# keya-dialog/LoCo-ASR

Hardware: AMD Instinct MI355X
Metric: audio frames/sec SpeechT5-base encoder, 30s×bs32 @1/2/4/8 GPU; embed L2 vs HF (higher is better)
Workload: dtype f16x3 (fp16 hi+lo operands, 3 MFMAs per product, fp32 accumulate); 1 GPU; SpeechT5-base speech encoder, synthetic 16 kHz 30 s clips, batch 32 per GPU (BASELINE.json configs[1]), random-init weights; batch_per_gpu=32, global_batch=32, frames_per_clip=1499, parallelism=dp1, collective=none

## Files before the change

### include/loco_asr.h

```cpp
#ifndef LOCO_ASR_H
#define LOCO_ASR_H

#include <stddef.h>
#include <stdint.h>

#ifdef __cplusplus
extern "C" {
#endif

#define LOCO_ABI_VERSION 1

enum {
    LOCO_OK = 0,
    LOCO_E_INVALID = -1,
    LOCO_E_STATE = -2,
    LOCO_E_WORKSPACE = -3,
    LOCO_E_HIP = -4,
    LOCO_E_RANGE = -5
};

typedef struct loco_config {
    int32_t struct_size;
    int32_t hidden;
    int32_t heads;
    int32_t ffn;
    int32_t layers;
    int32_t conv_dim;
    int32_t pos_conv_kernel;
    int32_t pos_conv_groups;
    int32_t rel_max;
    float ln_eps;
} loco_config;

typedef struct loco_encoder loco_encoder;

int loco_abi_version(void);
const char* loco_last_error(void);
void loco_default_config(loco_config* cfg);

loco_encoder* loco_create(const loco_config* cfg);
void loco_destroy(loco_encoder* enc);

int loco_set_weight(loco_encoder* enc, const char* key, const float* data, const int64_t* shape, int ndim);

int loco_missing_weights(const loco_encoder* enc, char* buf, size_t buflen);

int loco_finalize_weights(loco_encoder* enc, void* stream);

int64_t loco_output_frames(int64_t n_samples);

size_t loco_workspace_bytes(const loco_encoder* enc, int32_t B, int64_t L);

int loco_forward(loco_encoder* enc, const float* wav, const int32_t* attention_mask, int32_t B, int64_t L,
                 float* out, int32_t* out_frames, float* const* hidden_states, void* workspace,
                 size_t workspace_bytes, void* stream);

int loco_forward_status(loco_encoder* enc, char* buf, size_t buflen);
int loco_forward_range(const loco_encoder* enc, int32_t stage, float* amax, int32_t* layer, char* name, size_t namelen);
int loco_set_range_policy(loco_encoder* enc, int policy);
int loco_forward_checked(loco_encoder* enc, const float* wav, const int32_t* attention_mask, int32_t B, int64_t L,
                         float* out, int32_t* out_frames, float* const* hidden_states, void* workspace,
                         size_t workspace_bytes, void* stream, int32_t* used_fp32);

size_t loco_status_bytes(void);
int loco_forward_async(loco_encoder* enc, int precision, const float* wav, const int32_t* attention_mask, int32_t B, int64_t L,
                       float* out, int32_t* out_frames, float* const* hidden_states, void* workspace, size_t workspace_bytes,
                       void* stream, void* status);
int loco_status_check(const void* status, char* buf, size_t buflen);

int loco_max_pack_clips(void);
int loco_forward_packed(loco_encoder* enc, int precision, const float* wav, const int32_t* attention_mask, const int64_t* valid_len,
                        int32_t B, int64_t L, const int64_t* pad_len, float* out, int32_t* out_frames, float* const* hidden_states,
                        void* workspace, size_t workspace_bytes, void* stream, void* status);
int loco_status_range(const void* status, int32_t stage, float* amax, int32_t* layer, char* name, size_t namelen);

int loco_resample_design(int32_t sr_in, int32_t sr_out, int32_t* up, int32_t* down, int32_t* taps_per_phase, float* taps_host);
int64_t loco_resample_length(int64_t n_in, int32_t up, int32_t down);
int loco_op_resample(const float* x, int32_t B, int64_t n_in, int64_t x_stride, const float* taps_dev, int32_t up, int32_t down,
                     int32_t taps_per_phase, float* y, int64_t n_out, int64_t y_stride, void* stream);

const char* loco_flac_last_error(void);
int loco_flac_info(const void* data, size_t nbytes, int32_t* sample_rate, int32_t* channels, int32_t* bits_per_sample, int64_t* total_samples);
int loco_flac_decode(const void* data, size_t nbytes, float* mono, int32_t* pcm, int64_t capacity, int64_t* n_samples, int32_t verify_md5);

size_t loco_normalize_scratch_bytes(int32_t B);
int loco_op_normalize_waveform(const float* wav, const int32_t* attention_mask, int32_t B, int64_t L, float padding_value,
                               float* out, void* scratch, size_t scratch_bytes, void* stream);

size_t loco_text_workspace_bytes(const loco_encoder* enc, int32_t B, int32_t T);
int loco_text_max_positions(const loco_encoder* enc);
int loco_forward_text(loco_encoder* enc, const int32_t* input_ids, const int32_t* attention_mask, int32_t B, int32_t T,
                      float* out, int32_t* out_frames, float* const* hidden_states, void* workspace, size_t workspace_bytes,
                      void* stream);
int loco_forward_text_async(loco_encoder* enc, int precision, const int32_t* input_ids, const int32_t* attention_mask, int32_t B,
                            int32_t T, float* out, int32_t* out_frames, float* const* hidden_states, void* workspace,
                            size_t workspace_bytes, void* stream, void* status);

#define LOCO_PRECISION_MODES "0 f32, 1 f16x3, 2 f16x2"
const char* loco_precision_name(int mode);
int loco_set_precision(loco_encoder* enc, int mode);
int loco_get_precision(const loco_encoder* enc);

int loco_set_streams(loco_encoder* enc, int n);

int loco_set_taps(loco_encoder* enc, float* conv_stack, float* feature_projection, float* prenet);

int loco_set_attention_outputs(loco_encoder* enc, float* const* probs, int32_t n);

typedef struct loco_kernel_stat {
    char name[48];
    int64_t launches;
    double ms;
    double flops;
    double bytes;
} loco_kernel_stat;

int loco_set_profiling(loco_encoder* enc, int on);
int loco_set_profiling_filter(loco_encoder* enc, const char* bucket);
int loco_profile_reset(loco_encoder* enc);
int loco_profile_read(loco_encoder* enc, loco_kernel_stat* stats, int max_stats);


int loco_op_layernorm(const float* x, const float* gamma, const float* beta, float* y, int64_t rows, int32_t dim,
                      float eps, void* stream);

int loco_op_gemm(const float* A, int64_t lda, const float* W, int64_t ldw, const float* bias, const float* R, int64_t ldr,
                 float* C, int64_t ldc, int32_t M, int32_t N, int32_t K, int32_t epilogue, int32_t nb1, int32_t nb2,
                 int64_t sA1, int64_t sA2, int64_t sC1, int64_t sC2, void* stream);

size_t loco_conv0_scratch_bytes(int32_t B);
int loco_op_conv0_gn_gelu(const float* wav, int32_t B, int64_t L, const float* w, const float* gn_w, const float* gn_b,
                          float* out, void* scratch, void* stream);

int loco_op_frame_counts(const int32_t* mask, int32_t B, int64_t L, int32_t* frames, void* stream);

int loco_op_pos_conv(const float* h, const float* w_folded, const float* bias, const float* sin_table, const int32_t* frames,
                     float* out, int32_t B, int32_t T, void* stream);

int loco_op_attention(const float* qkv, const float* qp, const int32_t* frames, float* ctx, int32_t B, int32_t T,
                      void* stream);
int loco_op_attention_probs(const float* qkv, const float* qp, const int32_t* frames, float* probs, int32_t B, int32_t T,
                            void* stream);

int loco_op_split_f16(const float* x, void* hi, void* lo, int64_t n, void* stream);
int loco_op_gemm_f16x3(const void* Ahi, const void* Alo, int64_t lda, const void* Whi, const void* Wlo, int64_t ldw,
                       const float* bias, const float* R, int64_t ldr, float* C, void* Chi, void* Clo, int64_t ldc,
                       int32_t M, int32_t N, int32_t K, int32_t epilogue, int32_t nb1, int32_t nb2, int64_t sA1, int64_t sA2,
                       int64_t sC1, int64_t sC2, void* stream);

int loco_op_permute_conv_k(const float* w, float* out, int32_t N, int32_t taps, int32_t Cin, void* stream);
int loco_op_conv_gemm_f16x3(const void* Ahi, const void* Alo, int64_t lda, const void* Whi, const void* Wlo, float* C, void* Chi,
                            void* Clo, int32_t Tout, int32_t N, int32_t Cin, int32_t taps, int32_t epilogue, int32_t B, int64_t sA1,
                            void* stream);

size_t loco_gemm_splitk_bytes(void);
void loco_debug_reload_gemm_knobs(void);
int loco_op_gemm_f16x3_splitk(const void* Ahi, const void* Alo, int64_t lda, const void* Whi, const void* Wlo, int64_t ldw,
                              const float* bias, const float* R, int64_t ldr, float* C, void* Chi, void* Clo, int64_t ldc,
                              int32_t M, int32_t N, int32_t K, int32_t epilogue, void* splitk_ws, size_t splitk_bytes,
                              void* stream);

int loco_op_attention_f16x3(const void* qhi, const void* qlo, const void* khi, const void* klo, const void* vhi,
                            const void* vlo, const float* qp, const int32_t* frames, float* ctx, int32_t B, int32_t T,
                            void* stream);
int loco_op_attention_f16x3_pe(const void* qhi, const void* qlo, const void* khi, const void* klo, const void* vhi, const void* vlo,
                               const void* pe_hi, const void* pe_lo, float pe_scale, float* qp_scratch, const int32_t* frames,
                               float* ctx, int32_t B, int32_t T, void* stream);
int loco_op_attention_probs_f16x3(const void* qhi, const void* qlo, const void* khi, const void* klo, const float* qp,
                                  const int32_t* frames, float* probs, int32_t B, int32_t T, int32_t terms, void* stream);

typedef struct loco_head loco_head;
const char* loco_head_last_error(void);
loco_head* loco_head_create(int method);
void loco_head_destroy(loco_head* head);
int32_t loco_head_num_params(void);
int loco_head_set_params(loco_head* head, const float* flat);
int loco_head_get_params(const loco_head* head, float* flat);
size_t loco_head_workspace_bytes(int32_t B, int32_t T);
int loco_head_forward(loco_head* head, const float* x, int32_t B, int32_t T, float* logits, void* workspace,
                      size_t workspace_bytes, void* stream);
int loco_head_loss_grad(loco_head* head, const float* x, const float* target, int32_t B, int32_t T, float* loss,
                        float* logits, float* grads, void* workspace, size_t workspace_bytes, void* stream);
int loco_head_forward_ragged(loco_head* head, const float* store, const int64_t* offsets, const int32_t* lengths,
                             const int32_t* idx, int32_t B, int32_t T_pad, float* logits, void* workspace,
                             size_t workspace_bytes, void* stream);
int loco_head_loss_grad_ragged(loco_head* head, const float* store, const int64_t* offsets, const int32_t* lengths,
                               const float* targets, const int32_t* idx, int32_t B, int32_t T_pad, float* loss,
                               float* logits, float* grads, void* workspace, size_t workspace_bytes, void* stream);
int loco_head_adam_step(loco_head* head, const float* grads, float lr, float beta1, float beta2, float eps,
                        float weight_decay, void* stream);

int loco_has_decoder(const loco_encoder* enc);
int loco_decoder_max_batch(void);
size_t loco_decoder_workspace_bytes(const loco_encoder* enc, int32_t B, int32_t T_enc, int32_t S_max);
int loco_decoder_forward(loco_encoder* enc, const float* enc_out, const int32_t* enc_frames, int32_t B, int32_t T_enc,
                         const int32_t* decoder_input_ids, int32_t S, float* logits, float* const* hidden_states, void* workspace,
                         size_t workspace_bytes, void* stream);
int loco_decoder_begin(loco_encoder* enc, const float* enc_out, const int32_t* enc_frames, int32_t B, int32_t T_enc, int32_t S_max,
                       void* workspace, size_t workspace_bytes, void* stream);
int loco_decoder_step(loco_encoder* enc, int32_t B, int32_t T_enc, int32_t S_max, int32_t t, float* logits, void* workspace,
                      size_t workspace_bytes, void* stream);
int loco_decoder_read_tokens(const loco_encoder* enc, int32_t B, int32_t T_enc, int32_t S_max, int32_t* tokens, int32_t* lengths,
                             const void* workspace, size_t workspace_bytes, void* stream);
int loco_decoder_generate(loco_encoder* enc, const float* enc_out, const int32_t* enc_frames, int32_t B, int32_t T_enc, int32_t max_length,
                          int32_t* tokens_out, int32_t* lengths_out, int32_t* out_length, float* step_logits, void* workspace,
                          size_t workspace_bytes, void* stream);
int loco_op_skinny_gemm(const float* A, int64_t lda, const float* W, int64_t ldw, const float* bias, const float* R, int64_t ldr, float* C,
                        int64_t ldc, int32_t M, int32_t N, int32_t K, int32_t epilogue, void* stream);
size_t loco_decoder_attention_scratch_bytes(int32_t B, int32_t Sq, int32_t Tk);
int loco_op_decoder_attention(const float* q, const float* k, const float* v, const int32_t* key_counts, float* out, int32_t B, int32_t Sq,
                              int32_t Tk, int32_t causal, int32_t causal_offset, float scale, void* scratch, size_t scratch_bytes, void* stream);

#ifdef __cplusplus
}
#endif
#endif
```

### loco-asr_amd/_lib.py

```python
from __future__ import annotations

import ctypes as C
import os

_HERE = os.path.dirname(os.path.abspath(__file__))
LIB_PATH = os.environ.get("LOCO_ASR_LIB") or os.path.join(_HERE, "libloco_asr.so")
ABI_VERSION = 1


class LocoError(RuntimeError):
    """A C-ABI call returned a negative LOCO_E_* code."""


class LocoConfig(C.Structure):
    _fields_ = [("struct_size", C.c_int32), ("hidden", C.c_int32), ("heads", C.c_int32), ("ffn", C.c_int32),
                ("layers", C.c_int32), ("conv_dim", C.c_int32), ("pos_conv_kernel", C.c_int32),
                ("pos_conv_groups", C.c_int32), ("rel_max", C.c_int32), ("ln_eps", C.c_float)]


class KernelStat(C.Structure):
    _fields_ = [("name", C.c_char * 48), ("launches", C.c_int64), ("ms", C.c_double), ("flops", C.c_double),
                ("bytes", C.c_double)]


_vp, _i32, _i64, _sz, _f = C.c_void_p, C.c_int32, C.c_int64, C.c_size_t, C.c_float

SIGNATURES = {
    "loco_abi_version": (C.c_int, []),
    "loco_last_error": (C.c_char_p, []),
    "loco_default_config": (None, [C.POINTER(LocoConfig)]),
    "loco_create": (_vp, [C.POINTER(LocoConfig)]),
    "loco_destroy": (None, [_vp]),
    "loco_set_weight": (C.c_int, [_vp, C.c_char_p, _vp, C.POINTER(_i64), C.c_int]),
    "loco_missing_weights": (C.c_int, [_vp, C.c_char_p, _sz]),
    "loco_finalize_weights": (C.c_int, [_vp, _vp]),
    "loco_output_frames": (_i64, [_i64]),
    "loco_workspace_bytes": (_sz, [_vp, _i32, _i64]),
    "loco_forward": (C.c_int, [_vp, _vp, _vp, _i32, _i64, _vp, _vp, C.POINTER(_vp), _vp, _sz, _vp]),
    "loco_forward_status": (C.c_int, [_vp, C.c_char_p, _sz]),
    "loco_forward_range": (C.c_int, [_vp, _i32, C.POINTER(_f), C.POINTER(_i32), C.c_char_p, _sz]),
    "loco_set_range_policy": (C.c_int, [_vp, C.c_int]),
    "loco_forward_checked": (C.c_int, [_vp, _vp, _vp, _i32, _i64, _vp, _vp, C.POINTER(_vp), _vp, _sz, _vp, C.POINTER(_i32)]),
    "loco_status_bytes": (_sz, []),
    "loco_forward_async": (C.c_int, [_vp, C.c_int, _vp, _vp, _i32, _i64, _vp, _vp, C.POINTER(_vp), _vp, _sz, _vp, _vp]),
    "loco_max_pack_clips": (C.c_int, []),
    "loco_forward_packed": (C.c_int, [_vp, C.c_int, _vp, _vp, C.POINTER(_i64), _i32, _i64, C.POINTER(_i64), _vp, _vp, C.POINTER(_vp), _vp, _sz, _vp,
                                      _vp]),
    "loco_status_check": (C.c_int, [_vp, C.c_char_p, _sz]),
    "loco_status_range": (C.c_int, [_vp, _i32, C.POINTER(_f), C.POINTER(_i32), C.c_char_p, _sz]),
    "loco_flac_last_error": (C.c_char_p, []),
    "loco_flac_info": (C.c_int, [_vp, _sz, C.POINTER(_i32), C.POINTER(_i32), C.POINTER(_i32), C.POINTER(_i64)]),
    "loco_flac_decode": (C.c_int, [_vp, _sz, _vp, _vp, _i64, C.POINTER(_i64), _i32]),
    "loco_resample_design": (C.c_int, [_i32, _i32, C.POINTER(_i32), C.POINTER(_i32), C.POINTER(_i32), _vp]),
    "loco_resample_length": (_i64, [_i64, _i32, _i32]),
    "loco_op_resample": (C.c_int, [_vp, _i32, _i64, _i64, _vp, _i32, _i32, _i32, _vp, _i64, _i64, _vp]),
    "loco_normalize_scratch_bytes": (_sz, [_i32]),
    "loco_op_normalize_waveform": (C.c_int, [_vp, _vp, _i32, _i64, C.c_float, _vp, _vp, _sz, _vp]),
    "loco_text_workspace_bytes": (_sz, [_vp, _i32, _i32]),
    "loco_text_max_positions": (C.c_int, [_vp]),
    "loco_forward_text": (C.c_int, [_vp, _vp, _vp, _i32, _i32, _vp, _vp, C.POINTER(_vp), _vp, _sz, _vp]),
    "loco_precision_name": (C.c_char_p, [C.c_int]),
    "loco_forward_text_async": (C.c_int, [_vp, C.c_int, _vp, _vp, _i32, _i32, _vp, _vp, C.POINTER(_vp), _vp, _sz, _vp, _vp]),
    "loco_set_precision": (C.c_int, [_vp, C.c_int]),
    "loco_get_precision": (C.c_int, [_vp]),
    "loco_set_streams": (C.c_int, [_vp, C.c_int]),
    "loco_set_taps": (C.c_int, [_vp, _vp, _vp, _vp]),
    "loco_set_attention_outputs": (C.c_int, [_vp, _vp, _i32]),
    "loco_set_profiling": (C.c_int, [_vp, C.c_int]),
    "loco_set_profiling_filter": (C.c_int, [_vp, C.c_char_p]),
    "loco_profile_reset": (C.c_int, [_vp]),
    "loco_profile_read": (C.c_int, [_vp, C.POINTER(KernelStat), C.c_int]),
    "loco_op_layernorm": (C.c_int, [_vp, _vp, _vp, _vp, _i64, _i32, _f, _vp]),
    "loco_op_gemm": (C.c_int, [_vp, _i64, _vp, _i64, _vp, _vp, _i64, _vp, _i64, _i32, _i32, _i32, _i32, _i32, _i32,
                               _i64, _i64, _i64, _i64, _vp]),
    "loco_conv0_scratch_bytes": (_sz, [_i32]),
    "loco_op_conv0_gn_gelu": (C.c_int, [_vp, _i32, _i64, _vp, _vp, _vp, _vp, _vp, _vp]),
    "loco_op_frame_counts": (C.c_int, [_vp, _i32, _i64, _vp, _vp]),
    "loco_op_pos_conv": (C.c_int, [_vp, _vp, _vp, _vp, _vp, _vp, _i32, _i32, _vp]),
    "loco_op_attention": (C.c_int, [_vp, _vp, _vp, _vp, _i32, _i32, _vp]),
    "loco_op_attention_probs": (C.c_int, [_vp, _vp, _vp, _vp, _i32, _i32, _vp]),
    "loco_op_attention_probs_f16x3": (C.c_int, [_vp, _vp, _vp, _vp, _vp, _vp, _vp, _i32, _i32, _i32, _vp]),
    "loco_op_split_f16": (C.c_int, [_vp, _vp, _vp, _i64, _vp]),
    "loco_gemm_splitk_bytes": (_sz, []),
    "loco_debug_reload_gemm_knobs": (None, []),
    "loco_op_gemm_f16x3_splitk": (C.c_int, [_vp, _vp, _i64, _vp, _vp, _i64, _vp, _vp, _i64, _vp, _vp, _vp, _i64, _i32, _i32, _i32, _i32,
                                            _vp, _sz, _vp]),
    "loco_op_gemm_f16x3": (C.c_int, [_vp, _vp, _i64, _vp, _vp, _i64, _vp, _vp, _i64, _vp, _vp, _vp, _i64, _i32, _i32, _i32, _i32,
                                     _i32, _i32, _i64, _i64, _i64, _i64, _vp]),
    "loco_op_permute_conv_k": (C.c_int, [_vp, _vp, _i32, _i32, _i32, _vp]),
    "loco_op_conv_gemm_f16x3": (C.c_int, [_vp, _vp, _i64, _vp, _vp, _vp, _vp, _vp, _i32, _i32, _i32, _i32, _i32, _i32, _i64, _vp]),
    "loco_op_attention_f16x3": (C.c_int, [_vp, _vp, _vp, _vp, _vp, _vp, _vp, _vp, _vp, _i32, _i32, _vp]),
    "loco_op_attention_f16x3_pe": (C.c_int, [_vp, _vp, _vp, _vp, _vp, _vp, _vp, _vp, _f, _vp, _vp, _vp, _i32, _i32, _vp]),
    "loco_head_last_error": (C.c_char_p, []),
    "loco_head_create": (_vp, [C.c_int]),
    "loco_head_destroy": (None, [_vp]),
    "loco_head_num_params": (_i32, []),
    "loco_head_set_params": (C.c_int, [_vp, _vp]),
    "loco_head_get_params": (C.c_int, [_vp, _vp]),
    "loco_head_workspace_bytes": (_sz, [_i32, _i32]),
    "loco_head_forward": (C.c_int, [_vp, _vp, _i32, _i32, _vp, _vp, _sz, _vp]),
    "loco_head_loss_grad": (C.c_int, [_vp, _vp, _vp, _i32, _i32, _vp, _vp, _vp, _vp, _sz, _vp]),
    "loco_head_forward_ragged": (C.c_int, [_vp, _vp, _vp, _vp, _vp, _i32, _i32, _vp, _vp, _sz, _vp]),
    "loco_head_loss_grad_ragged": (C.c_int, [_vp, _vp, _vp, _vp, _vp, _vp, _i32, _i32, _vp, _vp, _vp, _vp, _sz, _vp]),
    "loco_head_adam_step": (C.c_int, [_vp, _vp, _f, _f, _f, _f, _f, _vp]),
    "loco_has_decoder": (C.c_int, [_vp]),
    "loco_decoder_max_batch": (C.c_int, []),
    "loco_decoder_workspace_bytes": (_sz, [_vp, _i32, _i32, _i32]),
    "loco_decoder_forward": (C.c_int, [_vp, _vp, _vp, _i32, _i32, _vp, _i32, _vp, C.POINTER(_vp), _vp, _sz, _vp]),
    "loco_decoder_begin": (C.c_int, [_vp, _vp, _vp, _i32, _i32, _i32, _vp, _sz, _vp]),
    "loco_decoder_step": (C.c_int, [_vp, _i32, _i32, _i32, _i32, _vp, _vp, _sz, _vp]),
    "loco_decoder_read_tokens": (C.c_int, [_vp, _i32, _i32, _i32, _vp, _vp, _vp, _sz, _vp]),
    "loco_decoder_generate": (C.c_int, [_vp, _vp, _vp, _i32, _i32, _i32, _vp, _vp, C.POINTER(_i32), _vp, _vp, _sz, _vp]),
    "loco_op_skinny_gemm": (C.c_int, [_vp, _i64, _vp, _i64, _vp, _vp, _i64, _vp, _i64, _i32, _i32, _i32, _i32, _vp]),
    "loco_decoder_attention_scratch_bytes": (_sz, [_i32, _i32, _i32]),
    "loco_op_decoder_attention": (C.c_int, [_vp, _vp, _vp, _vp, _vp, _i32, _i32, _i32, _i32, _i32, _f, _vp, _sz, _vp]),
}

_lib = None


def _check_foreign_build(path):
    import importlib.util
    spec = importlib.util.spec_from_file_location("loco_check_isa", os.path.join(_HERE, "csrc", "check_isa.py"))
    mod = importlib.util.module_from_spec(spec)
    spec.loader.exec_module(mod)
    try:
        _, _, bad = mod.check(path)
    except (OSError, RuntimeError) as e:
        import warnings
        warnings.warn(f"LOCO_ASR_LIB={path}: could not inspect the code objects ({e})")
        return
    if bad and os.environ.get("LOCO_ALLOW_BANNED_ISA") != "1":
        raise ImportError(f"LOCO_ASR_LIB={path}: {len(bad)} packed fp32 instructions cross-select their low lane (e.g. `{bad[0]}`): "
                          "results are unreliable beside the attention kernel (DESIGN.md 5); set LOCO_ALLOW_BANNED_ISA=1 only to "
                          "reproduce that hazard")


def load():
    global _lib
    if _lib is not None:
        return _lib
    if not os.path.exists(LIB_PATH):
        raise ImportError(
            f"{LIB_PATH} not found: the HIP library has not been built. Run `python -c 'import __graft_entry__ as g; "
            f"g.build()'` or `make -C {os.path.join(_HERE, 'csrc')}` (hipcc, --offload-arch=gfx950). There is no CPU fallback.")
    if os.environ.get("LOCO_ASR_LIB"):
        _check_foreign_build(LIB_PATH)
    lib = C.CDLL(LIB_PATH)
    for name, (res, args) in SIGNATURES.items():
        if os.environ.get("LOCO_ASR_LIB") and name.startswith("loco_op_") and not hasattr(lib, name):
            continue
        fn = getattr(lib, name)
        fn.restype = res
        fn.argtypes = args
    if lib.loco_abi_version() != ABI_VERSION:
        raise ImportError(f"{LIB_PATH}: ABI version {lib.loco_abi_version()} != {ABI_VERSION}; rebuild the library")
    _lib = lib
    return lib


def check(rc: int, what: str = ""):
    if rc < 0:
        msg = load().loco_last_error().decode(errors="replace")
        if rc == -1:
            raise ValueError(f"{what}: {msg}" if what else msg)
        raise LocoError(f"{what}: [{rc}] {msg}" if what else f"[{rc}] {msg}")
    return rc
```

### loco-asr_amd/csrc/gemm_f16x3.hip

```cpp
#include <cstdlib>

#include "loco_kernels.h"

#ifndef LOCO_GEMM_HACK
#define LOCO_GEMM_HACK 0
#endif

namespace loco {

typedef _Float16 h8 __attribute__((ext_vector_type(8)));
typedef _Float16 h4 __attribute__((ext_vector_type(4)));

template <int EPI, bool OUT_SPLIT>
__device__ __forceinline__ void split_gemm_store(const GemmSplitArgs& p, f32x4 v, long coff, int m, int n, float& amax, int z1 = 0,
                                                 int z2 = 0) {
    if (EPI == kEpiGelu) {
#pragma unroll
        for (int e = 0; e < 4; e += 2) { const f32x2_t g_ = gelu_erf2(f32x2_t{v[e], v[e + 1]}); v[e] = g_.x; v[e + 1] = g_.y; }
    }
    if (EPI == kEpiResidual) {
        const long ro = coff + (long)m * p.ldr + n;
        if (p.Rhi) {
            const h4 rh = *reinterpret_cast<const h4*>(p.Rhi + ro), rl = *reinterpret_cast<const h4*>(p.Rlo + ro);
#pragma unroll
            for (int e = 0; e < 4; ++e) v[e] += (float)rh[e] + (float)rl[e];
        } else {
            v += *reinterpret_cast<const f32x4*>(p.R + ro);
        }
    }
    if (EPI == kEpiPosConv) {
#pragma unroll
        for (int e = 0; e < 4; e += 2) { const f32x2_t g_ = gelu_erf2(f32x2_t{v[e], v[e + 1]}); v[e] = g_.x; v[e + 1] = g_.y; }
        int nvalid = p.frames ? p.frames[z1] : p.T;
        if (nvalid <= 0 || nvalid > p.T) nvalid = p.T;
        const int pos = m < nvalid ? m + 2 : 1;
        v += *reinterpret_cast<const f32x4*>(p.R + coff + (long)m * p.ldr + n);
        v += *reinterpret_cast<const f32x4*>(p.sin_table + (long)pos * kHidden + z2 * kPosCg + n);
        *reinterpret_cast<f32x4*>(p.C + coff + (long)m * p.ldc + n) = v;
        return;
    }
    if (!OUT_SPLIT && EPI != kEpiQkvScatter) {
        *reinterpret_cast<f32x4*>(p.C + coff + (long)m * p.ldc + n) = v;
        return;
    }
    typedef unsigned u32x2_t __attribute__((ext_vector_type(2)));
    amax = fmaxf(fmaxf(amax, fmaxf(fabsf(v[0]), fabsf(v[1]))), fmaxf(fabsf(v[2]), fabsf(v[3])));
    u32x2_t hu, lu;
    {
        unsigned h0, l0, h1, l1;
        split_f16_2pairs(v[0], v[1], v[2], v[3], h0, l0, h1, l1);
        hu = u32x2_t{h0, h1};
        lu = u32x2_t{l0, l1};
    }
    const h4 hi = __builtin_bit_cast(h4, hu), lo = __builtin_bit_cast(h4, lu);
    if (EPI == kEpiQkvScatter) {
        {
            const int third = n < kHidden ? 0 : (n < 2 * kHidden ? 1 : 2);
            const long o = third * p.qkv_stride + (long)m * kHidden + (n - third * kHidden);
            *reinterpret_cast<h4*>(p.Chi + o) = hi;
            *reinterpret_cast<h4*>(p.Clo + o) = lo;
        }
    } else {
        const long o = coff + (long)m * p.ldc + n;
        *reinterpret_cast<h4*>(p.Chi + o) = hi;
        *reinterpret_cast<h4*>(p.Clo + o) = lo;
    }
}

template <int EPI, bool OUT_SPLIT>
__device__ __forceinline__ void split_gemm_store16(const GemmSplitArgs& p, f32x4 (&v)[4], long coff, int m, int n, float& amax, int z1,
                                                   int z2) {
    constexpr bool wide_epi = EPI == kEpiNone || EPI == kEpiGelu || EPI == kEpiResidual || EPI == kEpiQkvScatter;
    if (!wide_epi || n + 16 > p.N) {
#pragma unroll
        for (int j = 0; j < 4; ++j)
            if (n + 4 * j < p.N) split_gemm_store<EPI, OUT_SPLIT>(p, v[j], coff, m, n + 4 * j, amax, z1, z2);
        return;
    }
    if (EPI == kEpiGelu) {
#pragma unroll
        for (int j = 0; j < 4; ++j)
#pragma unroll
            for (int e = 0; e < 4; e += 2) { const f32x2_t g_ = gelu_erf2(f32x2_t{v[j][e], v[j][e + 1]}); v[j][e] = g_.x; v[j][e + 1] = g_.y; }
    }
    if (EPI == kEpiResidual) {
        const long ro = coff + (long)m * p.ldr + n;
        if (p.Rhi) {
#pragma unroll
            for (int jj = 0; jj < 2; ++jj) {
                const h8 rh = *reinterpret_cast<const h8*>(p.Rhi + ro + 8 * jj), rl = *reinterpret_cast<const h8*>(p.Rlo + ro + 8 * jj);
#pragma unroll
                for (int e = 0; e < 8; ++e) v[2 * jj + (e >> 2)][e & 3] += (float)rh[e] + (float)rl[e];
            }
        } else {
#pragma unroll
            for (int j = 0; j < 4; ++j) v[j] += *reinterpret_cast<const f32x4*>(p.R + ro + 4 * j);
        }
    }
    if (!OUT_SPLIT && EPI != kEpiQkvScatter) {
        float* cp = p.C + coff + (long)m * p.ldc + n;
#pragma unroll
        for (int j = 0; j < 4; ++j)
            if (LOCO_GEMM_HACK != 4 || p.M <= 0) *reinterpret_cast<f32x4*>(cp + 4 * j) = v[j];
        return;
    }
    typedef unsigned u32x4_t __attribute__((ext_vector_type(4)));
    h8 hi[2], lo[2];
#pragma unroll
    for (int j = 0; j < 4; ++j) amax = fmaxf(fmaxf(amax, fmaxf(fabsf(v[j][0]), fabsf(v[j][1]))), fmaxf(fabsf(v[j][2]), fabsf(v[j][3])));
#pragma unroll
    for (int jj = 0; jj < 2; ++jj) {
        u32x4_t hu, lu;
        unsigned h0, l0, h1, l1;
        split_f16_2pairs(v[2 * jj][0], v[2 * jj][1], v[2 * jj][2], v[2 * jj][3], h0, l0, h1, l1);
        hu[0] = h0; hu[1] = h1; lu[0] = l0; lu[1] = l1;
        split_f16_2pairs(v[2 * jj + 1][0], v[2 * jj + 1][1], v[2 * jj + 1][2], v[2 * jj + 1][3], h0, l0, h1, l1);
        hu[2] = h0; hu[3] = h1; lu[2] = l0; lu[3] = l1;
        hi[jj] = __builtin_bit_cast(h8, hu);
        lo[jj] = __builtin_bit_cast(h8, lu);
    }
    _Float16 *dh, *dl;
    if (EPI == kEpiQkvScatter) {
        const int third = n < kHidden ? 0 : (n < 2 * kHidden ? 1 : 2);
        const long o = third * p.qkv_stride + (long)m * kHidden + (n - third * kHidden);
        dh = p.Chi + o;
        dl = p.Clo + o;
    } else {
        const long o = coff + (long)m * p.ldc + n;
        dh = p.Chi + o;
        dl = p.Clo + o;
    }
    if (LOCO_GEMM_HACK == 4 && p.M > 0) return;
    *reinterpret_cast<h8*>(dh) = hi[0];
    *reinterpret_cast<h8*>(dh + 8) = hi[1];
    *reinterpret_cast<h8*>(dl) = lo[0];
    *reinterpret_cast<h8*>(dl + 8) = lo[1];
}

constexpr int SBK = 32;

#ifdef LOCO_GEMM_STAMPS
__device__ unsigned long long* g_gemm_stamps = nullptr;
#define GEMM_STAMP(t) { __builtin_amdgcn_sched_barrier(0); asm volatile("s_memtime %0\n\ts_waitcnt lgkmcnt(0)" : "=s"(t) :: "memory"); __builtin_amdgcn_sched_barrier(0); }
#else
#define GEMM_STAMP(t) {}
#endif

typedef __attribute__((address_space(1))) const void* gptr_t;
typedef __attribute__((address_space(3))) void* lptr_t;
typedef __attribute__((address_space(3))) const h8* lds_h8p;

#if LOCO_GEMM_HACK == 1
#define DMA16(base_, voff_, ldsb_) asm volatile("" :: "s"(ldsb_), "v"(voff_), "s"(base_) : "memory")
#elif LOCO_GEMM_HACK == 6
#define DMA16(base_, voff_, ldsb_)                                                                                                  \
    if (wave < 4) asm volatile("s_mov_b32 m0, %0\n\ts_nop 0\n\tglobal_load_lds_dwordx4 %1, %2" :: "s"(ldsb_), "v"(voff_), "s"(base_) : "memory")
#else
#define DMA16(base_, voff_, ldsb_) \
    asm volatile("s_mov_b32 m0, %0\n\ts_nop 0\n\tglobal_load_lds_dwordx4 %1, %2" :: "s"(ldsb_), "v"(voff_), "s"(base_) : "memory")
#endif
#define VMCNT_LGKM0(n_)                                                                              \
    {                                                                                                \
        static_assert((n_) >= 0 && (n_) <= 63, "vmcnt is a 6-bit field");                            \
        asm volatile("s_waitcnt vmcnt(%0) lgkmcnt(0)" ::"n"(n_) : "memory");                         \
    }

template <int EPI, bool OUT_SPLIT, int WM, int WN, int AST, int WST, int NJ = 4, int WPS = 0, int TERMS = 3, bool PERSIST = false>
__global__ __launch_bounds__(64 * WM * WN, WPS ? WPS : (WM * WN) / 4) void gemm_f16x3_dma_kernel(GemmSplitArgs p, int tiles_m,
                                                                                                  int tiles_n, int nblk, int wg_step,
                                                                                                  int col_group) {
    constexpr int DBM = 64 * WM, DBN = 64 * WN, NW_ = WM * WN;
    constexpr int DPA = DBM * SBK, DPW = DBN * SBK;
    constexpr int ABUF = 2 * DPA, WBUF = 2 * DPW;
    constexpr int NDA = DBM / 16 / NW_;
    constexpr int NDW = (DBN / 16 + NW_ - 1) / NW_;
    constexpr int WPIECES = DBN / 16;
    constexpr int NA = 2 * NDA, NWP = (TERMS == 3 ? 2 : 1) * NDW;
    static_assert(NDA >= 1 && DBM % (16 * NW_) == 0, "tile too small for the wave count");
    static_assert((AST == WST && AST >= 2 && AST <= 5) || (AST == 3 && WST == 2), "ring depths: equal rings of 2-5 slots, or 3 A + 2 W");
    static_assert(WPIECES % NW_ == 0 || (WST == 2 && AST == 3) || AST == 2, "uneven W pieces: no wait may leave W DMAs in flight");
    static_assert(TERMS == 3 || TERMS == 2, "terms");
    static_assert((size_t)(AST * ABUF + WST * WBUF) * 2 <= 160 * 1024, "LDS");
    static_assert(2 * (DPA + 16 * 3 * SBK) < 65536 && 2 * (DPW + 16 * 3 * SBK) < 65536, "fragment offsets are ds_read immediates");
    constexpr bool PERMW = NJ == 4 && (OUT_SPLIT || EPI == kEpiQkvScatter);
    __shared__ __attribute__((aligned(16))) _Float16 lds[AST * ABUF + WST * WBUF];

    const int tid = threadIdx.x, lane = tid & 63;
    const int wave = __builtin_amdgcn_readfirstlane(tid >> 6);
    const int wm = wave / WN, wn = wave % WN;
    const int r16 = lane & 15, q4 = lane >> 4;
    const int drow = lane >> 2, dpos = lane & 3;
    const unsigned lds0 = (unsigned)(unsigned long)(lptr_t)lds;
    const int nk = p.K / SBK;

    const int xcd = blockIdx.x & 7;
    int tile_i = blockIdx.x >> 3;
    int run_start, run_len;
    {
        const int q = nblk >> 3, rr = nblk & 7;
        run_start = xcd < rr ? xcd * (q + 1) : rr * (q + 1) + (xcd - rr) * q;
        run_len = q + (xcd < rr ? 1 : 0);
    }
    struct Tile {
        const char *bAh, *bAl, *bWh, *bWl;
        unsigned va[NDA], vw[NDW];
        int m0, n0, z1, z2, kt0;
        long coff;
    };
    auto decode = [&](int i, Tile& t_) {
        const int t = run_start + i;
        const int per_z = tiles_m * tiles_n;
        const int z = t / per_z;
        const int tz = t - z * per_z;
        const int full = tiles_n / col_group;
        int g = tz / (tiles_m * col_group), rem, width;
        if (g < full) {
            rem = tz - g * tiles_m * col_group;
            width = col_group;
        } else {
            g = full;
            rem = tz - full * tiles_m * col_group;
            width = tiles_n - full * col_group;
        }
        const int mt = rem / width;
        const int nt = g * col_group + (rem - mt * width);
        t_.z1 = z / p.nb2;
        t_.z2 = z % p.nb2;
        t_.kt0 = t_.z2 * p.kt_per_z2;
        const int z1o = t_.z1 / p.z1_inner, z1i = t_.z1 - z1o * p.z1_inner;
        const long aoff = z1o * p.sA1 + z1i * p.sA1i + t_.z2 * p.sA2;
        const long woff = z1i * p.sW1i + t_.z2 * p.sW2;
        t_.coff = t_.z1 * p.sC1 + t_.z2 * p.sC2;
        t_.m0 = mt * DBM;
        t_.n0 = nt * DBN;
#pragma unroll
        for (int u = 0; u < NDA; ++u) {
            const int row = 16 * (NDA * wave + u) + drow;
            int ra = t_.m0 + row;
            ra = (ra < p.M ? ra : p.M - 1) - t_.m0;
            t_.va[u] = 2u * (unsigned)(ra * (int)p.lda + 8 * (dpos ^ (3 * ((row >> 2) & 1))));
        }
#pragma unroll
        for (int u = 0; u < NDW; ++u) {
            const int row = 16 * (NDW * wave + u) + drow;
            int rw = t_.n0 + row;
            rw = (rw < p.N ? rw : p.N - 1) - t_.n0;
            t_.vw[u] = 2u * (unsigned)(rw * (int)p.ldw + 8 * (dpos ^ (PERMW ? ((0x78 >> (2 * ((row >> 4) & 3))) & 3) : 3 * ((row >> 2) & 1))));
        }
        t_.bAh = reinterpret_cast<const char*>(p.Ahi + aoff + (long)t_.m0 * p.lda);
        t_.bAl = reinterpret_cast<const char*>(p.Alo + aoff + (long)t_.m0 * p.lda);
        t_.bWh = reinterpret_cast<const char*>(p.Whi + woff + (long)t_.n0 * p.ldw);
        t_.bWl = reinterpret_cast<const char*>(p.Wlo + woff + (long)t_.n0 * p.ldw);
    };
    Tile cur, nxt;
    decode(tile_i, cur);
    nxt = cur;

    const int ktaps = p.ktaps, kchan2 = 2 * (p.kchan ? p.kchan : p.K / (p.ktaps > 0 ? p.ktaps : 1));
    auto a_koff = [&](int t) -> long {
        const int q = t >> 1, half = t & 1;
        const int cbp = ktaps == 3 ? (int)(((unsigned)q * 0xAAABu) >> 17) : (ktaps == 2 ? q >> 1 : q);
        const int slot = q - cbp * ktaps;
        const int tap = ktaps == 3 ? ((0x18 >> (2 * slot)) & 3) : slot;
        const long off = (long)tap * kchan2 + (long)(2 * cbp + half) * (2 * SBK);
        return ktaps == 1 ? (long)t * (2 * SBK) : off;
    };
#define DMA_A(q_, T_, t_, sl_)                                                                                              \
    {                                                                                                                       \
        const int tt_ = (t_) < nk ? (t_) : nk - 1;                                                                          \
        const unsigned d_ = lds0 + 2u * (unsigned)((sl_) * ABUF + ((q_) & 1) * DPA + 16 * (NDA * wave + ((q_) >> 1)) * SBK); \
        DMA16((((q_) & 1) ? (T_).bAl : (T_).bAh) + a_koff((T_).kt0 + tt_), (T_).va[(q_) >> 1], d_);                         \
    }
#define DMA_W(q_, T_, t_, sl_)                                                                                              \
    {                                                                                                                       \
        const int tt_ = (t_) < nk ? (t_) : nk - 1;                                                                          \
        const int u_ = TERMS == 3 ? (q_) >> 1 : (q_);                                                                       \
        const int pl_ = TERMS == 3 ? (q_) & 1 : 0;                                                                          \
        if (WPIECES % NW_ == 0 || NDW * wave + u_ < WPIECES) {                                                              \
            const unsigned d_ = lds0 + 2u * (unsigned)(AST * ABUF + (sl_) * WBUF + pl_ * DPW + 16 * (NDW * wave + u_) * SBK); \
            DMA16((pl_ ? (T_).bWl : (T_).bWh) + (long)tt_ * (2 * SBK), (T_).vw[u_], d_);                                    \
        }                                                                                                                   \
    }

    [[maybe_unused]] unsigned long long st0 = 0, st1 = 0, st2 = 0, st3 = 0, st4 = 0, rt0 = 0, rt1 = 0;
#ifdef LOCO_GEMM_STAMPS
    asm volatile("s_memrealtime %0\n\ts_waitcnt lgkmcnt(0)" : "=s"(rt0) :: "memory");
#endif
    GEMM_STAMP(st0)

    const int swz = 3 * ((r16 >> 2) & 1);
    const int fa = (wm * 64 + r16) * SBK + 8 * (q4 ^ swz);
    const int fw = PERMW ? (wn * 64 + 16 * (r16 >> 2) + (r16 & 3)) * SBK + 8 * (q4 ^ ((0x78 >> (2 * (r16 >> 2))) & 3))
                         : (wn * 64 + r16) * SBK + 8 * (q4 ^ swz);
    unsigned a_ad = lds0 + 2u * (unsigned)fa;
    unsigned w_ad = lds0 + 2u * (unsigned)(AST * ABUF + fw);
#define LDS_H8(ad_, halves_) (*(lds_h8p)(unsigned long)((ad_) + 2u * (unsigned)(halves_)))
#define RD_A(i_, s_)                                                  \
    if (LOCO_GEMM_HACK != 2 || ((i_) & 1) == 0) {                     \
        ah[s_] = LDS_H8(a_ad, 16 * (i_) * SBK);                       \
        al[s_] = LDS_H8(a_ad, DPA + 16 * (i_) * SBK);                 \
    } else {                                                          \
        ah[s_] = ah[1 - (s_)];                                        \
        al[s_] = al[1 - (s_)];                                        \
    }
#define RD_W(j_)                                                                         \
    {                                                                                    \
        wh[j_] = LDS_H8(w_ad, (PERMW ? 4 : 16) * (j_) * SBK);                            \
        if (TERMS == 3) wl[j_] = LDS_H8(w_ad, DPW + (PERMW ? 4 : 16) * (j_) * SBK);      \
    }
#define MM(i_, s_, j_)                                                                                                    \
    {                                                                                                                     \
        if (TERMS == 3) acc16[i_][j_] = __builtin_amdgcn_mfma_f32_16x16x32_f16(wl[j_], ah[s_], acc16[i_][j_], 0, 0, 0);   \
        acc16[i_][j_] = __builtin_amdgcn_mfma_f32_16x16x32_f16(wh[j_], al[s_], acc16[i_][j_], 0, 0, 0);                   \
        acc16[i_][j_] = __builtin_amdgcn_mfma_f32_16x16x32_f16(wh[j_], ah[s_], acc16[i_][j_], 0, 0, 0);                   \
    }
#define SB() __builtin_amdgcn_sched_barrier(0);
    int sa = 0, sw = 0;
#define A_STEP() (unsigned)(sa + 1 == AST ? -(AST - 1) * 2 * ABUF : 2 * ABUF)
#define W_STEP() (unsigned)(sw + 1 == WST ? -(WST - 1) * 2 * WBUF : 2 * WBUF)

    constexpr int JH = (NJ + 1) / 2;
    constexpr int NG = (NJ + 1) / 2;
    constexpr int NBLK = 1 + NG;
    constexpr int NPC = NWP + NA;
    h8 ah[2], al[2], wh[NJ], wl[NJ];
    f32x4 acc16[4][NJ];
    constexpr int kPendLoop = AST == WST ? (AST - 2) * (NA + NWP) : NA;
    if (AST == WST) {
#pragma unroll
        for (int t = 0; t < AST; ++t) {
#pragma unroll
            for (int q = 0; q < NWP; ++q) DMA_W(q, cur, t, t)
#pragma unroll
            for (int q = 0; q < NA; ++q) DMA_A(q, cur, t, t)
        }
        VMCNT_LGKM0(WPIECES % NW_ == 0 ? (AST - 1) * (NA + NWP) : 0)
    } else {
#pragma unroll
        for (int t = 0; t < WST; ++t)
#pragma unroll
            for (int q = 0; q < NWP; ++q) DMA_W(q, cur, t, t)
#pragma unroll
        for (int t = 0; t < AST; ++t)
#pragma unroll
            for (int q = 0; q < NA; ++q) DMA_A(q, cur, t, t)
        VMCNT_LGKM0((AST - 1) * NA)
    }
    __builtin_amdgcn_s_barrier();
    GEMM_STAMP(st1)
#pragma unroll
    for (int j = 0; j < NJ; ++j) RD_W(j)
    RD_A(0, 0)
#define DMA_AFTER_BLOCK(b_)                                                                     \
    {                                                                                           \
        _Pragma("unroll") for (int q = 0; q < NPC; ++q)                                         \
            if (q * NBLK / NPC == (b_)) {                                                       \
                if (q < NWP) DMA_W(q < NWP ? q : 0, sel, tW, sw)                                \
                else DMA_A(q < NWP ? 0 : q - NWP, sel, tA, sa)                                  \
            }                                                                                   \
        SB()                                                                                    \
    }
    for (;;) {
        const bool has_next = PERSIST && wg_step > 0 && tile_i + wg_step < run_len;
        if (PERSIST && has_next) decode(tile_i + wg_step, nxt);
#pragma unroll
        for (int i = 0; i < 4; ++i)
#pragma unroll
            for (int j = 0; j < NJ; ++j) acc16[i][j] = f32x4{0.f, 0.f, 0.f, 0.f};
        for (int kt = 0; kt < nk; ++kt) {
            const unsigned a_step = A_STEP(), w_step = W_STEP();
            const bool a_cur = kt + AST < nk, w_cur = kt + WST < nk;
            const int tA = (a_cur || !PERSIST) ? kt + AST : kt + AST - nk, tW = (w_cur || !PERSIST) ? kt + WST : kt + WST - nk;
            Tile sel;
            if (PERSIST) {
                sel.kt0 = a_cur ? cur.kt0 : nxt.kt0;
                sel.bAh = a_cur ? cur.bAh : nxt.bAh;
                sel.bAl = a_cur ? cur.bAl : nxt.bAl;
                sel.bWh = w_cur ? cur.bWh : nxt.bWh;
                sel.bWl = w_cur ? cur.bWl : nxt.bWl;
#pragma unroll
                for (int u = 0; u < NDA; ++u) sel.va[u] = a_cur ? cur.va[u] : nxt.va[u];
#pragma unroll
                for (int u = 0; u < NDW; ++u) sel.vw[u] = w_cur ? cur.vw[u] : nxt.vw[u];
            } else {
                sel = cur;
            }
            SB()
            MM(0, 0, 0)
            if (NJ > 1) MM(0, 0, 1)
            asm volatile("" : "+v"(acc16[0][0]), "+v"(acc16[0][NJ > 1 ? 1 : 0]));
            SB()
            RD_A(1, 1)
            SB()
#pragma unroll
            for (int j = 2; j < NJ; ++j) MM(0, 0, j)
            SB()
            RD_A(2, 0)
            SB()
#pragma unroll
            for (int j = 0; j < NJ; ++j) MM(1, 1, j)
            SB()
            RD_A(3, 1)
            SB()
#pragma unroll
            for (int j = 0; j < JH; ++j) MM(2, 0, j)
            SB()
            VMCNT_LGKM0(kPendLoop)
            __builtin_amdgcn_s_barrier();
#pragma unroll
            for (int j = JH; j < NJ; ++j) MM(2, 0, j)
            SB()
            DMA_AFTER_BLOCK(0)
            a_ad += a_step;
            w_ad += w_step;
            RD_A(0, 0)
            SB()
#pragma unroll
            for (int g = 0; g < NG; ++g) {
#pragma unroll
                for (int j = 2 * g; j < 2 * g + 2 && j < NJ; ++j) MM(3, 1, j)
                SB()
                DMA_AFTER_BLOCK(1 + g)
#pragma unroll
                for (int j = 2 * g; j < 2 * g + 2 && j < NJ; ++j) RD_W(j)
                SB()
            }
            sa = sa + 1 == AST ? 0 : sa + 1;
            sw = sw + 1 == WST ? 0 : sw + 1;
            SB()
        }
        GEMM_STAMP(st2)

        {
            const int m0 = cur.m0, n0 = cur.n0, z1 = cur.z1, z2 = cur.z2;
            const long coff = cur.coff;
            const float osc = p.out_scale;
            float amax = 0.f;
            const unsigned seen = (OUT_SPLIT || EPI == kEpiQkvScatter) ? range_peek(p.range_slot) : 0u;
            if (PERMW) {
                const int n = n0 + wn * 64 + 16 * q4;
                if (n < p.N) {
#pragma unroll
                    for (int i = 0; i < 4; ++i) {
                        const int m = m0 + wm * 64 + 16 * i + r16;
                        if (m >= p.M) continue;
                        f32x4 v[4];
#pragma unroll
                        for (int j = 0; j < 4; ++j) {
                            v[j] = acc16[i][j < NJ ? j : 0] * osc;
                            if (p.bias && n + 4 * j < p.N) v[j] += *reinterpret_cast<const f32x4*>(p.bias + z2 * p.sBias2 + n + 4 * j);
                        }
                        split_gemm_store16<EPI, OUT_SPLIT>(p, v, coff, m, n, amax, z1, z2);
                    }
                }
                range_commit(p.range_slot, amax, seen);
            } else {
#pragma unroll
                for (int i = 0; i < 4; ++i) {
                    const int m = m0 + wm * 64 + 16 * i + r16;
                    if (m >= p.M) continue;
#pragma unroll
                    for (int j = 0; j < NJ; ++j) {
                        const int n = n0 + wn * 64 + 16 * j + 4 * q4;
                        if (n < p.N) {
                            f32x4 v = acc16[i][j] * osc;
                            if (p.bias) v += *reinterpret_cast<const f32x4*>(p.bias + z2 * p.sBias2 + n);
                            split_gemm_store<EPI, OUT_SPLIT>(p, v, coff, m, n, amax, z1, z2);
                        }
                    }
                }
                if (OUT_SPLIT || EPI == kEpiQkvScatter) range_commit(p.range_slot, amax, seen);
            }
        }
        if (!PERSIST || !has_next) break;
        cur = nxt;
        tile_i += wg_step;
    }
    asm volatile("s_waitcnt vmcnt(0)" ::: "memory");
#undef DMA_AFTER_BLOCK
#undef A_STEP
#undef W_STEP
#undef SB
#undef MM
#undef RD_W
#undef RD_A
#undef LDS_H8
#undef DMA_W
#undef DMA_A
#ifdef LOCO_GEMM_STAMPS
    {
        GEMM_STAMP(st3)
        asm volatile("s_waitcnt vmcnt(0)" ::: "memory");
        GEMM_STAMP(st4)
        asm volatile("s_memrealtime %0\n\ts_waitcnt lgkmcnt(0)" : "=s"(rt1) :: "memory");
        if (g_gemm_stamps && tid == 0) {
            unsigned hw;
            asm volatile("s_getreg_b32 %0, hwreg(HW_REG_XCC_ID)" : "=s"(hw));
            unsigned long long* o_ = g_gemm_stamps + 8l * blockIdx.x;
            o_[0] = st1 - st0; o_[1] = st2 - st1; o_[2] = 0; o_[3] = st3 - st2; o_[4] = st4 - st3; o_[5] = rt0; o_[6] = rt1;
            o_[7] = hw;
        }
    }
#endif
}
#undef VMCNT_LGKM0
#undef DMA16

constexpr int PCR_S = 24;
constexpr int PCR_WPL = kPosCg * SBK;
constexpr int PCR_WST = 3;
template <int NI> struct PcrGeom {
    static constexpr int BM = 8 * 16 * NI, ROWS = BM + kPosK;
    static constexpr int REG = ROWS * PCR_S, APL = 2 * REG;
    static_assert((REG * 2) % 256 == 0 && (ROWS * 3) % 64 == 0, "region = whole bank rows and whole DMA instructions");
    static_assert((2 * APL + PCR_WST * 2 * PCR_WPL) * 2 <= 160 * 1024, "LDS");
};
#define PCR_DMA16(base_, voff_, ldsb_) \
    asm volatile("s_mov_b32 m0, %0\n\ts_nop 0\n\tglobal_load_lds_dwordx4 %1, %2" :: "s"(ldsb_), "v"(voff_), "s"(base_) : "memory")

template <int TERMS, int NI>
__global__ __launch_bounds__(512, 2) void pos_conv_resident_kernel(GemmSplitArgs p) {
    constexpr int PCR_BM = PcrGeom<NI>::BM, PCR_ROWS = PcrGeom<NI>::ROWS, PCR_REG = PcrGeom<NI>::REG, PCR_APL = PcrGeom<NI>::APL;
    __shared__ __attribute__((aligned(16))) _Float16 lds[2 * PCR_APL + PCR_WST * 2 * PCR_WPL];
    const int tid = threadIdx.x, lane = tid & 63;
    const int wave = __builtin_amdgcn_readfirstlane(tid >> 6);
    const int r16 = lane & 15, q4 = lane >> 4;
    const int t0 = blockIdx.x * PCR_BM, g = blockIdx.y, b = blockIdx.z;
    const unsigned lds0 = (unsigned)(unsigned long)(lptr_t)lds;
    const int rows_total = p.M + kPosK;
    const char* const abase_h = reinterpret_cast<const char*>(p.Ahi + b * p.sA1 + g * p.sA2);
    const char* const abase_l = reinterpret_cast<const char*>(p.Alo + b * p.sA1 + g * p.sA2);
    const char* const wbase_h = reinterpret_cast<const char*>(p.Whi + g * p.sW2);
    const char* const wbase_l = reinterpret_cast<const char*>(p.Wlo + g * p.sW2);

    constexpr int kPiecesPerRegion = PCR_ROWS * 3, kInstrPerPlane = 2 * kPiecesPerRegion / 64;
    for (int n = wave; n < 2 * kInstrPerPlane; n += 8) {
        const int pl = n >= kInstrPerPlane, ni = pl ? n - kInstrPerPlane : n;
        const int P = 64 * ni + lane;
        const int par = P >= kPiecesPerRegion, Q = par ? P - kPiecesPerRegion : P;
        const int row = Q / 3, jj = Q - 3 * row;
        int grow = t0 + row;
        grow = grow < rows_total ? grow : rows_total - 1;
        const unsigned vo = (unsigned)grow * (2u * kPosCg) + 16u * (unsigned)(2 * jj + par);
        const unsigned d = lds0 + 2u * (unsigned)(pl * PCR_APL) + 1024u * (unsigned)ni;
        PCR_DMA16(pl ? abase_l : abase_h, vo, d);
    }
    const int wrow = 16 * (wave % 3) + (lane >> 2), wpos = lane & 3;
    const unsigned wvo = (unsigned)wrow * (unsigned)(2 * p.ldw) + 16u * (unsigned)(wpos ^ (3 * ((wrow >> 2) & 1)));
    const int nk = p.K / SBK;
#define PCR_DMA_W(kt_, slot_)                                                                                                   \
    if (wave < 6) {                                                                                                             \
        const int kk_ = (kt_) < nk ? (kt_) : nk - 1;                                                                            \
        const unsigned d_ = lds0 + 2u * (unsigned)(2 * PCR_APL + (slot_) * 2 * PCR_WPL + (wave / 3) * PCR_WPL + 16 * (wave % 3) * SBK); \
        PCR_DMA16((wave >= 3 ? wbase_l : wbase_h) + (long)kk_ * (2 * SBK), wvo, d_);                                             \
    }
    PCR_DMA_W(0, 0)
    PCR_DMA_W(1, 1)

    int aoff = (q4 & 1) * PCR_REG + (16 * NI * wave + r16) * PCR_S + 8 * (q4 >> 1);
    const int woff = r16 * SBK + 8 * (q4 ^ (3 * ((r16 >> 2) & 1)));
    f32x4 acc[NI][3];
#pragma unroll
    for (int i = 0; i < NI; ++i)
#pragma unroll
        for (int j = 0; j < 3; ++j) acc[i][j] = f32x4{0.f, 0.f, 0.f, 0.f};

    int slot = 0;
    for (int kt = 0; kt < nk; ++kt) {
        if (kt == 0 && wave >= 6) asm volatile("s_waitcnt vmcnt(0)" ::: "memory");
        else asm volatile("s_waitcnt vmcnt(1)" ::: "memory");
        __builtin_amdgcn_s_barrier();
        asm volatile("" ::: "memory");
        {
            const int s2 = slot + 2 >= PCR_WST ? slot + 2 - PCR_WST : slot + 2;
            PCR_DMA_W(kt + 2, s2)
        }
        const _Float16* wb = lds + 2 * PCR_APL + slot * 2 * PCR_WPL;
        h8 wh[3], wl[3];
#pragma unroll
        for (int j = 0; j < 3; ++j) {
            wh[j] = *reinterpret_cast<const h8*>(wb + 16 * j * SBK + woff);
            if (TERMS == 3) wl[j] = *reinterpret_cast<const h8*>(wb + PCR_WPL + 16 * j * SBK + woff);
        }
#pragma unroll
        for (int i = 0; i < NI; ++i) {
            const h8 ah = *reinterpret_cast<const h8*>(lds + aoff + 16 * i * PCR_S);
            const h8 al = *reinterpret_cast<const h8*>(lds + PCR_APL + aoff + 16 * i * PCR_S);
#pragma unroll
            for (int j = 0; j < 3; ++j) {
                if (TERMS == 3) acc[i][j] = __builtin_amdgcn_mfma_f32_16x16x32_f16(wl[j], ah, acc[i][j], 0, 0, 0);
                acc[i][j] = __builtin_amdgcn_mfma_f32_16x16x32_f16(wh[j], al, acc[i][j], 0, 0, 0);
                acc[i][j] = __builtin_amdgcn_mfma_f32_16x16x32_f16(wh[j], ah, acc[i][j], 0, 0, 0);
            }
        }
        aoff += 16;
        slot = slot + 1 == PCR_WST ? 0 : slot + 1;
    }
    asm volatile("s_waitcnt vmcnt(0)" ::: "memory");
#undef PCR_DMA_W

    const long coff = b * p.sC1 + g * p.sC2;
    float amax = 0.f;
#pragma unroll
    for (int i = 0; i < NI; ++i) {
        const int m = t0 + 16 * NI * wave + 16 * i + r16;
        if (m >= p.M) continue;
#pragma unroll
        for (int j = 0; j < 3; ++j) {
            const int n = 16 * j + 4 * q4;
            f32x4 v = acc[i][j] * p.out_scale;
            if (p.bias) v += *reinterpret_cast<const f32x4*>(p.bias + g * p.sBias2 + n);
            split_gemm_store<kEpiPosConv, false>(p, v, coff, m, n, amax, b, g);
        }
    }
}
#undef PCR_DMA16

template <int EPI, bool OUT_SPLIT>
__global__ __launch_bounds__(256) void splitk_reduce_kernel(GemmSplitArgs p, int ks) {
    const long n4 = (long)p.M * (p.N / 4);
    float amax = 0.f;
    const unsigned seen = (OUT_SPLIT || EPI == kEpiQkvScatter) ? range_peek(p.range_slot) : 0u;
    for (long i = (long)blockIdx.x * 256 + threadIdx.x; i < n4; i += (long)gridDim.x * 256) {
        const int m = (int)(i / (p.N / 4));
        const int n = 4 * (int)(i - (long)m * (p.N / 4));
        const float* part = p.splitk_ws + (long)m * p.N + n;
        f32x4 v = *reinterpret_cast<const f32x4*>(part);
        for (int k = 1; k < ks; ++k) v += *reinterpret_cast<const f32x4*>(part + (long)k * p.M * p.N);
        v *= p.out_scale;
        if (p.bias) v += *reinterpret_cast<const f32x4*>(p.bias + n);
        split_gemm_store<EPI, OUT_SPLIT>(p, v, 0, m, n, amax);
    }
    if (OUT_SPLIT || EPI == kEpiQkvScatter) range_commit_block(p.range_slot, amax, seen);
}

__global__ __launch_bounds__(256) void splitk_reduce_qkv_kernel(GemmSplitArgs p, int ks) {
    const int m0 = blockIdx.x * 64, n0 = blockIdx.y * 64;
    const int tid = threadIdx.x;
    const int c4 = tid & 15, r0 = tid >> 4;
    float amax = 0.f;
    const unsigned seen = range_peek(p.range_slot);
    const int n = n0 + 4 * c4;
    const f32x4 bias = p.bias ? *reinterpret_cast<const f32x4*>(p.bias + n) : f32x4{0.f, 0.f, 0.f, 0.f};
    const int third = n0 < kHidden ? 0 : (n0 < 2 * kHidden ? 1 : 2);
    _Float16* const dh = p.Chi + third * p.qkv_stride;
    _Float16* const dl = p.Clo + third * p.qkv_stride;
#pragma unroll
    for (int rr = 0; rr < 4; ++rr) {
        const int ml = r0 + 16 * rr, m = m0 + ml;
        if (m >= p.M) continue;
        const float* part = p.splitk_ws + (long)m * p.N + n;
        f32x4 v = *reinterpret_cast<const f32x4*>(part);
        for (int k = 1; k < ks; ++k) v += *reinterpret_cast<const f32x4*>(part + (long)k * p.M * p.N);
        v = v * p.out_scale + bias;
        amax = fmaxf(fmaxf(amax, fmaxf(fabsf(v[0]), fabsf(v[1]))), fmaxf(fabsf(v[2]), fabsf(v[3])));
        unsigned h0, l0, h1, l1;
        split_f16_2pairs(v[0], v[1], v[2], v[3], h0, l0, h1, l1);
        typedef unsigned u32x2_t __attribute__((ext_vector_type(2)));
        const long o = (long)m * kHidden + (n - third * kHidden);
        *reinterpret_cast<u32x2_t*>(dh + o) = u32x2_t{h0, h1};
        *reinterpret_cast<u32x2_t*>(dl + o) = u32x2_t{l0, l1};
    }
    range_commit_block(p.range_slot, amax, seen);
}

__global__ __launch_bounds__(256) void splitk_reduce_posconv_kernel(GemmSplitArgs p, int ks) {
    constexpr int n4s = kPosCg / 4;
    const long total = (long)p.nb1 * p.nb2 * p.M * n4s;
    float amax = 0.f;
    for (long i = (long)blockIdx.x * 256 + threadIdx.x; i < total; i += (long)gridDim.x * 256) {
        const int n = 4 * (int)(i % n4s);
        long rest = i / n4s;
        const int m = (int)(rest % p.M);
        rest /= p.M;
        const int g = (int)(rest % p.nb2), b = (int)(rest / p.nb2);
        const long gstride = (long)p.M * kPosCg, sstride = (long)p.nb2 * gstride;
        const float* part = p.splitk_ws + ((long)b * ks * p.nb2 + g) * gstride + (long)m * kPosCg + n;
        f32x4 v = *reinterpret_cast<const f32x4*>(part);
        for (int k = 1; k < ks; ++k) v += *reinterpret_cast<const f32x4*>(part + k * sstride);
        v *= p.out_scale;
        if (p.bias) v += *reinterpret_cast<const f32x4*>(p.bias + g * p.sBias2 + n);
        split_gemm_store<kEpiPosConv, false>(p, v, b * p.sC1 + g * p.sC2, m, n, amax, b, g);
    }
}

struct GemmKnobs {
    int tile = 0, narrow = 0;
    bool nopersist = false, nocolgroup = false, no192 = false, nosplitk = false, posconv_generic = false;
    int posconv_ni = 0;
};
static GemmKnobs read_gemm_knobs() {
    GemmKnobs k;
    const char* v;
    if ((v = getenv("LOCO_GEMM_TILE"))) k.tile = atoi(v);
    if ((v = getenv("LOCO_GEMM_TILE_NARROW"))) k.narrow = atoi(v);
    k.nopersist = getenv("LOCO_GEMM_NOPERSIST") != nullptr;
    k.nocolgroup = getenv("LOCO_GEMM_NOCOLGROUP") != nullptr;
    k.no192 = getenv("LOCO_GEMM_NO192") != nullptr;
    k.posconv_generic = getenv("LOCO_POSCONV_GENERIC") != nullptr;
    if ((v = getenv("LOCO_POSCONV_NI"))) k.posconv_ni = (atoi(v) == 2 || atoi(v) == 4) ? atoi(v) : 0;
    k.nosplitk = getenv("LOCO_GEMM_NOSPLITK") != nullptr;
    return k;
}
static GemmKnobs& gemm_knobs() {
    static GemmKnobs k = read_gemm_knobs();
    return k;
}
void reload_gemm_knobs() { gemm_knobs() = read_gemm_knobs(); }

template <int WM, int WN, int AST, int WST, int WPS, int TERMS = 3>
static hipError_t launch_tile(const GemmSplitArgs& a, hipStream_t s) {
    constexpr int bm = 64 * WM, bn = 64 * WN;
    const int tm = (a.M + bm - 1) / bm, tn = (a.N + bn - 1) / bn;
    const long nb = (long)tm * tn * a.nb1 * a.nb2;
    if (nb <= 0 || nb > 0x7fffffffL) return hipErrorInvalidValue;
    const bool sp = a.Chi != nullptr;
    constexpr bool kPersist = WM * WN <= 12;
    constexpr int slots = 256 * (WPS ? (4 * WPS) / (WM * WN) : 1);
    const bool persist = kPersist && nb > slots && a.K / SBK >= AST && !gemm_knobs().nopersist;
    const unsigned grid = persist ? (unsigned)slots : (unsigned)nb;
    const int wg_step = persist ? slots / 8 : 0;
    const int ngroups = (tn + 5) / 6;
    const int col_group = gemm_knobs().nocolgroup ? tn : (tn + ngroups - 1) / ngroups;
#define TILE_LAUNCH(EPI)                                                                                                              \
    if (sp) hipLaunchKernelGGL((gemm_f16x3_dma_kernel<EPI, true, WM, WN, AST, WST, 4, WPS, TERMS, kPersist>), dim3(grid), dim3(64 * WM * WN), 0, \
                               s, a, tm, tn, (int)nb, wg_step, col_group);                                                            \
    else hipLaunchKernelGGL((gemm_f16x3_dma_kernel<EPI, false, WM, WN, AST, WST, 4, WPS, TERMS, kPersist>), dim3(grid), dim3(64 * WM * WN), 0,  \
                            s, a, tm, tn, (int)nb, wg_step, col_group);
    switch (a.epilogue) {
        case kEpiNone: TILE_LAUNCH(kEpiNone) break;
        case kEpiGelu: TILE_LAUNCH(kEpiGelu) break;
        case kEpiResidual: TILE_LAUNCH(kEpiResidual) break;
        case kEpiQkvScatter: TILE_LAUNCH(kEpiQkvScatter) break;
        default: return hipErrorInvalidValue;
    }
#undef TILE_LAUNCH
    return hipGetLastError();
}

hipError_t launch_gemm_split(const GemmSplitArgs& a, hipStream_t s) {
    if (a.M <= 0 || a.N <= 0 || a.K <= 0 || a.K % SBK != 0) return hipErrorInvalidValue;
    if ((a.lda | a.ldw | a.sA1 | a.sA2) & 7) return hipErrorInvalidValue;
    if ((a.N | a.ldc | a.sC1 | a.sC2) & 3) return hipErrorInvalidValue;
    if (a.epilogue == kEpiResidual && ((!a.R && !(a.Rhi && a.Rlo)) || (a.ldr & (a.Rhi ? 7 : 3)))) return hipErrorInvalidValue;
    const bool split = a.Chi != nullptr;
    if (split ? (a.Clo == nullptr) : (a.C == nullptr)) return hipErrorInvalidValue;
    if (a.epilogue == kEpiQkvScatter &&
        (!split || a.N != kQkv || a.nb1 * a.nb2 != 1 || a.qkv_stride < (long)a.M * kHidden))
        return hipErrorInvalidValue;
    if (a.epilogue == kEpiPosConv) {
        if (a.N != kPosCg || !a.C || !a.R || !a.sin_table || a.T <= 0 || split) return hipErrorInvalidValue;
        const int tm = (a.M + 511) / 512;
        const long nb = (long)tm * a.nb1 * a.nb2;
        if (nb <= 0 || nb > 0x7fffffffL) return hipErrorInvalidValue;
        if (a.splitk_ws && nb <= 64 && a.z1_inner == 1 && !gemm_knobs().nosplitk) {
            const int ks = 8;
            if (a.K % (ks * SBK) == 0 && (size_t)ks * a.nb1 * a.nb2 * a.M * kPosCg * sizeof(float) <= kSplitKBytes) {
                GemmSplitArgs b = a;
                const int kslice = a.K / ks;
                b.splitk_ws = nullptr;
                b.bias = nullptr; b.R = nullptr; b.out_scale = 1.0f; b.sin_table = nullptr; b.frames = nullptr;
                b.C = a.splitk_ws; b.ldc = kPosCg;
                b.nb1 = a.nb1 * ks; b.z1_inner = ks;
                b.sA1i = kslice; b.sW1i = kslice;
                b.sC1 = (long)a.nb2 * a.M * kPosCg; b.sC2 = (long)a.M * kPosCg;
                b.K = kslice;
                b.epilogue = kEpiNone;
                const long nbp = (long)tm * b.nb1 * b.nb2;
                if (a.terms == 2)
                    hipLaunchKernelGGL((gemm_f16x3_dma_kernel<kEpiNone, false, 8, 1, 2, 2, 3, 0, 2>), dim3((unsigned)nbp), dim3(512), 0, s, b, tm, 1,
                                       (int)nbp, 0, 1);
                else
                    hipLaunchKernelGGL((gemm_f16x3_dma_kernel<kEpiNone, false, 8, 1, 2, 2, 3>), dim3((unsigned)nbp), dim3(512), 0, s, b, tm, 1,
                                       (int)nbp, 0, 1);
                hipError_t err = hipGetLastError();
                if (err != hipSuccess) return err;
                const long n4 = (long)a.nb1 * a.nb2 * a.M * (kPosCg / 4);
                const unsigned blocks = (unsigned)((n4 + 255) / 256 < 1024 ? (n4 + 255) / 256 : 1024);
                hipLaunchKernelGGL(splitk_reduce_posconv_kernel, dim3(blocks), dim3(256), 0, s, a, ks);
                return hipGetLastError();
            }
        }
        const bool resident = !gemm_knobs().posconv_generic && a.z1_inner == 1 && a.lda == kPosCg && a.K == kPosK * kPosCg && a.nb2 == kPosGroups &&
                              a.nb1 <= 65535 && a.sA2 == (long)(a.M + kPosK) * kPosCg && ((2 * a.ldw) & 15) == 0;
        if (resident) {
            constexpr double kSmallTile = 0.62;
            const int t512 = (a.M + 511) / 512, t256 = (a.M + 255) / 256;
            int ni = (t256 * kSmallTile < t512) ? 2 : 4;
            if (gemm_knobs().posconv_ni) ni = gemm_knobs().posconv_ni;
            const dim3 grid((unsigned)(ni == 2 ? t256 : t512), kPosGroups, (unsigned)a.nb1);
            if (ni == 2) {
                if (a.terms == 2) hipLaunchKernelGGL((pos_conv_resident_kernel<2, 2>), grid, dim3(512), 0, s, a);
                else hipLaunchKernelGGL((pos_conv_resident_kernel<3, 2>), grid, dim3(512), 0, s, a);
            } else {
                if (a.terms == 2) hipLaunchKernelGGL((pos_conv_resident_kernel<2, 4>), grid, dim3(512), 0, s, a);
                else hipLaunchKernelGGL((pos_conv_resident_kernel<3, 4>), grid, dim3(512), 0, s, a);
            }
            return hipGetLastError();
        }
        if (a.terms == 2)
            hipLaunchKernelGGL((gemm_f16x3_dma_kernel<kEpiPosConv, false, 8, 1, 2, 2, 3, 0, 2>), dim3((unsigned)nb), dim3(512), 0, s, a, tm, 1,
                               (int)nb, 0, 1);
        else
            hipLaunchKernelGGL((gemm_f16x3_dma_kernel<kEpiPosConv, false, 8, 1, 2, 2, 3>), dim3((unsigned)nb), dim3(512), 0, s, a, tm, 1,
                               (int)nb, 0, 1);
        return hipGetLastError();
    }
    if (a.ktaps < 1 || a.ktaps > 3 || (!a.kchan && a.ktaps > 1 && a.K % (a.ktaps * 2 * SBK) != 0) || a.K / SBK >= 32768) return hipErrorInvalidValue;
    if (a.splitk_ws && a.nb1 * a.nb2 == 1 && a.M <= kSplitKMaxM && !gemm_knobs().nosplitk) {
        const int bm = a.M >= 1024 ? 256 : 128;
        const int tm = (a.M + bm - 1) / bm, tn = (a.N + 127) / 128;
        int ks = 256 / (tm * tn);
        if (ks > a.K / 256) ks = a.K / 256;
        while (ks > 1 && a.K % (ks * SBK) != 0) --ks;
        if (ks >= 2) {
            GemmSplitArgs b = a;
            const int kslice = a.K / ks;
            b.splitk_ws = nullptr;
            b.bias = nullptr; b.R = nullptr; b.Chi = nullptr; b.Clo = nullptr; b.out_scale = 1.0f; b.range_slot = nullptr;
            b.C = a.splitk_ws; b.ldc = a.N;
            b.nb1 = 1; b.nb2 = ks; b.sA1 = 0; b.sC1 = 0;
            b.sA2 = kslice; b.sW2 = kslice; b.sC2 = (long)a.M * a.N; b.sBias2 = 0;
            if (a.ktaps > 1) {
                b.sA2 = 0;
                b.kt_per_z2 = kslice / SBK;
                b.kchan = a.kchan ? a.kchan : a.K / a.ktaps;
            }
            b.K = kslice;
            b.epilogue = kEpiNone;
            hipError_t err = launch_gemm_split(b, s);
            if (err != hipSuccess) return err;
            const long n4 = (long)a.M * (a.N / 4);
            const unsigned blocks = (unsigned)((n4 + 255) / 256 < 1024 ? (n4 + 255) / 256 : 1024);
#define RED_LAUNCH(EPI)                                                                                                  \
            if (split || EPI == kEpiQkvScatter) hipLaunchKernelGGL((splitk_reduce_kernel<EPI, true>), dim3(blocks), dim3(256), 0, s, a, ks); \
            else hipLaunchKernelGGL((splitk_reduce_kernel<EPI, false>), dim3(blocks), dim3(256), 0, s, a, ks);
            switch (a.epilogue) {
                case kEpiNone: RED_LAUNCH(kEpiNone) break;
                case kEpiGelu: RED_LAUNCH(kEpiGelu) break;
                case kEpiResidual: RED_LAUNCH(kEpiResidual) break;
                case kEpiQkvScatter:
                    hipLaunchKernelGGL(splitk_reduce_qkv_kernel, dim3((unsigned)((a.M + 63) / 64), kQkv / 64), dim3(256), 0, s, a, ks);
                    break;
                default: return hipErrorInvalidValue;
            }
#undef RED_LAUNCH
            return hipGetLastError();
        }
    }
    int tile = gemm_knobs().tile;
    if (tile == 0) {
        const long rows_total = (long)a.M * a.nb1 * a.nb2;
        if (rows_total >= 1024 && a.K <= 128) {
            tile = 4;
        } else if (rows_total >= 1024) {
            struct Form { int id, bm, bn; double eff; bool n256; };
            static const Form kForms[] = {{1, 256, 256, 1.00, true}, {6, 192, 256, 0.91, true}, {2, 256, 128, 0.80, false}, {5, 128, 128, 0.55, false}};
            double best = 0.0;
            for (const Form& f : kForms) {
                if (f.n256 && a.N % 256 != 0) continue;
                if (f.id == 6 && gemm_knobs().no192) continue;
                const double tiles = (double)((a.M + f.bm - 1) / f.bm) * ((a.N + f.bn - 1) / f.bn) * a.nb1 * a.nb2;
                const double rounds = a.co_scheduled ? tiles / 256.0 : (double)(((long)tiles + 255) / 256);
                const double cost = rounds * f.bm * f.bn / f.eff;
                if (tile == 0 || cost < best) { tile = f.id; best = cost; }
            }
            if (tile == 2 && gemm_knobs().narrow) tile = gemm_knobs().narrow;
        } else {
            tile = 5;
        }
    }
    if (a.terms == 2) {
        switch (tile) {
            case 1: return launch_tile<4, 4, 3, 2, 0, 2>(a, s);
            case 2: return launch_tile<4, 2, 3, 3, 0, 2>(a, s);
            case 4: return launch_tile<2, 2, 2, 2, 2, 2>(a, s);
            case 6: return launch_tile<3, 4, 3, 2, 0, 2>(a, s);
            case 3:
            case 5: return launch_tile<2, 2, 3, 3, 0, 2>(a, s);
            default: return hipErrorInvalidValue;
        }
    }
    switch (tile) {
        case 1: return launch_tile<4, 4, 3, 2, 0>(a, s);
        case 2: return launch_tile<4, 2, 3, 3, 0>(a, s);
        case 3: return launch_tile<3, 2, 2, 2, 3>(a, s);
        case 4: return launch_tile<2, 2, 2, 2, 2>(a, s);
        case 5: return launch_tile<2, 2, 3, 3, 0>(a, s);
        case 8: return launch_tile<2, 2, 5, 5, 0>(a, s);
        case 6: return launch_tile<3, 4, 3, 2, 0>(a, s);
        case 7: return launch_tile<4, 4, 2, 2, 0>(a, s);
        default: return hipErrorInvalidValue;
    }
}

__global__ void split_f16_kernel(const float* __restrict__ x, _Float16* __restrict__ hi, _Float16* __restrict__ lo, long n4, float scale) {
    for (long i = (long)blockIdx.x * blockDim.x + threadIdx.x; i < n4; i += (long)gridDim.x * blockDim.x) {
        const f32x4 v = reinterpret_cast<const f32x4*>(x)[i] * scale;
        h4 a, b;
#pragma unroll
        for (int e = 0; e < 4; ++e) {
            a[e] = (_Float16)v[e];
            b[e] = (_Float16)(v[e] - (float)a[e]);
        }
        reinterpret_cast<h4*>(hi)[i] = a;
        reinterpret_cast<h4*>(lo)[i] = b;
    }
}

__global__ void group_major_split_kernel(const float* __restrict__ x, _Float16* __restrict__ hi, _Float16* __restrict__ lo, int T,
                                         long total4, float* __restrict__ range_slot, const int32_t* __restrict__ rows_clip) {
    const int rows = T + kPosK;
    float amax = 0.f;
    const unsigned seen = range_peek(range_slot);
    for (long i = (long)blockIdx.x * blockDim.x + threadIdx.x; i < total4; i += (long)gridDim.x * blockDim.x) {
        const int c4 = (int)(i % (kPosCg / 4));
        long rest = i / (kPosCg / 4);
        const int row = (int)(rest % rows);
        rest /= rows;
        const int g = (int)(rest % kPosGroups);
        const int b = (int)(rest / kPosGroups);
        const int t = row - kPosK / 2;
        f32x4 v = {0.f, 0.f, 0.f, 0.f};
        if (t >= 0 && t < (rows_clip ? rows_clip[b] : T)) v = *reinterpret_cast<const f32x4*>(x + ((long)b * T + t) * kHidden + g * kPosCg + 4 * c4);
        h4 a, c;
#pragma unroll
        for (int e = 0; e < 4; ++e) {
            amax = fmaxf(amax, fabsf(v[e]));
            a[e] = (_Float16)v[e];
            c[e] = (_Float16)(v[e] - (float)a[e]);
        }
        reinterpret_cast<h4*>(hi)[i] = a;
        reinterpret_cast<h4*>(lo)[i] = c;
    }
    range_commit_block(range_slot, amax, seen);
}

hipError_t launch_group_major_split(const float* x, void* hi, void* lo, int B, int T, hipStream_t s, float* range_slot,
                                    const int32_t* rows_clip) {
    if (B <= 0 || T <= 0) return hipErrorInvalidValue;
    const long total4 = (long)B * kPosGroups * (T + kPosK) * (kPosCg / 4);
    hipLaunchKernelGGL(group_major_split_kernel, dim3(2048), dim3(256), 0, s, x, (_Float16*)hi, (_Float16*)lo, T, total4, range_slot, rows_clip);
    return hipGetLastError();
}

__global__ void pos_w_for_gemm_kernel(const float* __restrict__ wf, float* __restrict__ out) {
    const long total = (long)kHidden * kPosCg * kPosK;
    for (long idx = (long)blockIdx.x * blockDim.x + threadIdx.x; idx < total; idx += (long)gridDim.x * blockDim.x) {
        const int i = (int)(idx % kPosCg);
        long rest = idx / kPosCg;
        const int tap = (int)(rest % kPosK);
        rest /= kPosK;
        const int o = (int)(rest % kPosCg);
        const int g = (int)(rest / kPosCg);
        out[idx] = wf[(((long)g * kPosK + tap) * kPosCg + o) * kPosCg + i];
    }
}

hipError_t launch_pos_w_for_gemm(const float* wf, float* out, hipStream_t s) {
    hipLaunchKernelGGL(pos_w_for_gemm_kernel, dim3(1024), dim3(256), 0, s, wf, out);
    return hipGetLastError();
}

hipError_t launch_split_f16(const float* x, void* hi, void* lo, long n, hipStream_t s, float scale) {
    if (n <= 0 || (n & 3)) return hipErrorInvalidValue;
    hipLaunchKernelGGL(split_f16_kernel, dim3(2048), dim3(256), 0, s, x, (_Float16*)hi, (_Float16*)lo, n / 4, scale);
    return hipGetLastError();
}

}

#ifdef LOCO_GEMM_STAMPS
extern "C" int loco_debug_set_gemm_stamps(void* buf) {
    return (int)hipMemcpyToSymbol(HIP_SYMBOL(loco::g_gemm_stamps), &buf, sizeof(buf));
}
#endif
```

### loco-asr_amd/csrc/loco_api.hip

```cpp
#include <hip/hip_runtime.h>

#include <atomic>
#include <cmath>
#include <cstdarg>
#include <cstdio>
#include <cstring>
#include <map>
#include <mutex>
#include <string>
#include <utility>
#include <vector>

#include "../../include/loco_asr.h"
#include "loco_kernels.h"

using namespace loco;

namespace {

thread_local std::string g_err;

int fail(int code, const char* fmt, ...) {
    char buf[512];
    va_list ap;
// ... 268 lines not shown
std::string canonical_key(const char* key) {
    std::string k(key);
    const std::string a = "pos_conv_embed.conv.weight_g", b = "pos_conv_embed.conv.weight_v";
    size_t pos;
    if ((pos = k.find(a)) != std::string::npos && pos + a.size() == k.size())
        k.replace(pos, a.size(), "pos_conv_embed.conv.parametrizations.weight.original0");
    else if ((pos = k.find(b)) != std::string::npos && pos + b.size() == k.size())
        k.replace(pos, b.size(), "pos_conv_embed.conv.parametrizations.weight.original1");
    return k;
}

const float* W(const loco_encoder* e, const std::string& k) { return e->raw.at(k); }
WB weight_bias(const loco_encoder* e, const std::string& prefix) { return {W(e, prefix + "weight"), W(e, prefix + "bias")}; }

size_t align_up(size_t n) { return (n + 255) & ~size_t(255); }

struct Plan {
    int B;
    long L;
    long Tc[7];
    long T, M;
    size_t off_frames, off_clip, off_c0scratch, off_a, off_b, off_x0, off_x1, off_tmp, off_ctx, off_qkv, off_qp, off_ffn, off_xs0, off_xs1,
        off_splitk, total;
    bool splitk;
};

void carve_plan(const loco_encoder* e, Plan& p);

bool make_plan(const loco_encoder* e, int B, long L, Plan& p) {
    p.B = B;
    p.L = L;
    long n = L;
    for (int i = 0; i < 7; ++i) {
        n = conv_out_len(n, kConvK[i], kConvS[i]);
        p.Tc[i] = n;
    }
    if (B <= 0 || n <= 0) return false;
    p.T = n;
    p.M = (long)B * n;
    carve_plan(e, p);
    return true;
}

bool make_plan_tokens(const loco_encoder* e, int B, long T, Plan& p) {
    p.B = B;
    p.L = 0;
    for (int i = 0; i < 7; ++i) p.Tc[i] = 0;
    if (B <= 0 || T <= 0) return false;
    p.T = T;
    p.M = (long)B * T;
    carve_plan(e, p);
    return true;
}

void carve_plan(const loco_encoder* e, Plan& p) {
    const int B = p.B;
    const size_t f = sizeof(float);
    size_t o = 0;
    auto take = [&](size_t bytes) {
        size_t at = o;
        o += align_up(bytes);
        return at;
    };
    p.off_frames = take((size_t)B * sizeof(int32_t));
    p.off_clip = take((size_t)3 * B * sizeof(int32_t));
    p.off_c0scratch = take(conv0_scratch_bytes(B));
    p.off_a = take((size_t)B * p.Tc[0] * kConvDim * f);
    p.off_b = take((size_t)B * p.Tc[1] * kConvDim * f);
    p.off_x0 = take((size_t)p.M * kHidden * f);
    p.off_x1 = take((size_t)p.M * kHidden * f);
    p.off_tmp = take((size_t)p.M * kHidden * f);
    p.off_ctx = take((size_t)p.M * kHidden * f);
    p.off_qkv = take((size_t)3 * p.M * kHidden * f);
    p.off_qp = take((size_t)p.M * kHeads * kRelN * f);
    const size_t ffn_elems = (size_t)p.M * e->cfg.ffn, posg_elems = (size_t)B * (p.T + kPosK) * kHidden;
    p.off_ffn = take((ffn_elems > posg_elems ? ffn_elems : posg_elems) * f);
    p.off_xs0 = take((size_t)p.M * kHidden * f);
    p.off_xs1 = take((size_t)p.M * kHidden * f);
    p.splitk = p.M <= kSplitKMaxM;
    p.off_splitk = take(p.splitk ? kSplitKBytes : 0);
    p.total = o;
}

struct Bracket {
    loco_encoder* e;
    hipStream_t s;
    ProfRec* rec = nullptr;
    Bracket(loco_encoder* enc, hipStream_t st, int kid, double flops, double bytes) : e(enc), s(st) {
        if (!e->profiling || (e->profile_only >= 0 && e->profile_only != kid)) return;
        if (e->recs_used == e->recs.size()) {
            ProfRec r{};
            if (hipEventCreate(&r.a) != hipSuccess || hipEventCreate(&r.b) != hipSuccess) return;
            e->recs.push_back(r);
        }
        rec = &e->recs[e->recs_used++];
        rec->kid = kid;
        rec->flops = flops;
        rec->bytes = bytes;
        (void)hipEventRecord(rec->a, s);
    }
    ~Bracket() {
        if (rec) (void)hipEventRecord(rec->b, s);
    }
};

double gemm_flops(int M, int N, int K, int nb1, int nb2) { return 2.0 * M * (double)N * K * ((double)nb1 * nb2); }
double gemm_bytes(int M, int N, int K, int nb1, int nb2, int epi) {
    const double nb = (double)nb1 * nb2;
    return 4.0 * (nb * ((double)M * K + (double)M * N * (epi == kEpiResidual ? 2 : 1)) + (double)N * K);
}

int run_gemm(loco_encoder* e, hipStream_t s, const float* A, long lda, const float* Wt, long ldw, const float* bias,
             const float* R, long ldr, float* C, long ldc, int M, int N, int K, int epi, int nb1 = 1, int nb2 = 1,
             long sA1 = 0, long sA2 = 0, long sC1 = 0, long sC2 = 0) {
    GemmArgs a{A, Wt, bias, R, C, M, N, K, lda, ldw, ldc, ldr, nb1, nb2, sA1, sA2, sC1, sC2, epi};
    Bracket br(e, s, K_GEMM, gemm_flops(M, N, K, nb1, nb2), gemm_bytes(M, N, K, nb1, nb2, epi));
    HIP_TRY(launch_gemm(a, s));
    return LOCO_OK;
}

int run_ln(loco_encoder* e, hipStream_t s, const float* x, const float* g, const float* b, float* y, long rows, int dim,
           _Float16* yhi = nullptr, _Float16* ylo = nullptr, float* nonfinite_slot = nullptr) {
    Bracket br(e, s, K_LN, 8.0 * rows * dim, (y && yhi ? 12.0 : 8.0) * rows * dim);
    HIP_TRY(launch_layernorm(x, g, b, y, rows, dim, e->cfg.ln_eps, s, yhi, ylo, nonfinite_slot));
    return LOCO_OK;
}

GemmSplitArgs split_args(int M, int N, int K, int epilogue) {
    GemmSplitArgs a{};
    a.M = M; a.N = N; a.K = K;
    a.lda = a.ldw = K;
    a.ldc = N;
    a.epilogue = epilogue;
    a.nb1 = a.nb2 = 1;
    return a;
}

int run_gemm_split(loco_encoder* e, const Call& c, hipStream_t s, GemmSplitArgs a, const SplitW& w, int kid, double flops, double bytes) {
    a.Whi = w.hi;
    a.Wlo = w.lo;
    a.out_scale = w.inv_scale;
    a.terms = c.precision == 2 ? 2 : 3;
    a.co_scheduled = c.dual && a.epilogue != kEpiPosConv;
    a.splitk_ws = c.splitk;
    Bracket br(e, s, kid, flops, bytes);
    HIP_TRY(launch_gemm_split(a, s));
    return LOCO_OK;
}
int run_gemm_split(loco_encoder* e, const Call& c, hipStream_t s, const GemmSplitArgs& a, const SplitW& w) {
    return run_gemm_split(e, c, s, a, w, K_GEMM_SPLIT, gemm_flops(a.M, a.N, a.K, a.nb1, a.nb2),
                          gemm_bytes(a.M, a.N, a.K, a.nb1, a.nb2, a.epilogue));
}

int absmax_host(loco_encoder* e, const float* src, size_t n, hipStream_t s, float& out) {
    HIP_TRY(hipMemsetAsync(e->absmax_dev, 0, sizeof(float), s));
    HIP_TRY(launch_absmax(src, (long)n, e->absmax_dev, s));
    HIP_TRY(hipMemcpyAsync(&out, e->absmax_dev, sizeof(float), hipMemcpyDeviceToHost, s));
    HIP_TRY(hipStreamSynchronize(s));
    return LOCO_OK;
}

int make_split(loco_encoder* e, SplitW& w, const float* src, size_t n, hipStream_t s) {
    if (!w.hi) HIP_TRY(hipMalloc(&w.hi, n * sizeof(_Float16)));
    if (!w.lo) HIP_TRY(hipMalloc(&w.lo, n * sizeof(_Float16)));
    float amax = 0.f;
    if (int rc = absmax_host(e, src, n, s, amax)) return rc;
    int k = 0;
    if (amax > 0.f && amax < INFINITY) {
        int ex = 0;
        (void)frexpf(amax, &ex);
        k = 14 - ex;
        k = k > 100 ? 100 : (k < -100 ? -100 : k);
    }
    w.inv_scale = ldexpf(1.0f, -k);
    HIP_TRY(launch_split_f16(src, w.hi, w.lo, (long)n, s, ldexpf(1.0f, k)));
    return LOCO_OK;
}

constexpr float kRangeHi = 65504.0f;
constexpr float kRangeLo = 0.015625f;

int static_range_check(loco_encoder* e, const std::string& ln_prefix, int dim, hipStream_t s) {
    float g = 0.f, b = 0.f;
    int rc = absmax_host(e, W(e, ln_prefix + "weight"), (size_t)dim, s, g);
    if (!rc) rc = absmax_host(e, W(e, ln_prefix + "bias"), (size_t)dim, s, b);
    if (rc) return rc;
    const float hi = sqrtf((float)dim) * g + b, lo = fmaxf(g, b);
    if (e->range_static.empty() && (!(hi < kRangeHi) || lo < kRangeLo)) {
        char msg[320];
        snprintf(msg, sizeof msg, "activation range: the output of '%s*' (max|weight| = %.6g, max|bias| = %.6g) is %s the range precision mode "
                 "f16x3 represents to fp32 class (%g <= max|x| < %g)", ln_prefix.c_str(), (double)g, (double)b,
                 !(hi < kRangeHi) ? "not bounded inside" : "below", (double)kRangeLo, (double)kRangeHi);
        e->range_static = msg;
    }
    return LOCO_OK;
}

int dbg_check(loco_encoder* e, hipStream_t s, const char* stage, int layer, const void* p, size_t n, bool half, long row_len) {
    if (!e->debug_nonfinite || !p) return LOCO_OK;
    unsigned long long h[2] = {0, ~0ull};
    HIP_TRY(hipMemcpyAsync(e->debug_counter, h, sizeof h, hipMemcpyHostToDevice, s));
    HIP_TRY(launch_count_nonfinite(p, (long)n, half, e->debug_counter, s));
    HIP_TRY(hipMemcpyAsync(h, e->debug_counter, sizeof h, hipMemcpyDeviceToHost, s));
    HIP_TRY(hipStreamSynchronize(s));
    if (h[0])
        fprintf(stderr, "[loco debug] non-finite values: %llu of %zu elements written by '%s' (layer %d); first at element %llu = row %llu, column %llu\n",
                h[0], n, stage, layer, h[1], row_len ? h[1] / row_len : 0ull, row_len ? h[1] % row_len : 0ull);
    return LOCO_OK;
}
void dbg_planes(loco_encoder* e, hipStream_t s, const char* stage, int layer, const _Float16* hi, const _Float16* lo, size_t n,
                long row_len) {
    if (!e->debug_nonfinite) return;
    char name[96];
    snprintf(name, sizeof name, stage, "hi");
    dbg_check(e, s, name, layer, hi, n, true, row_len);
    snprintf(name, sizeof name, stage, "lo");
    dbg_check(e, s, name, layer, lo, n, true, row_len);
}

int run_copy(loco_encoder* e, hipStream_t s, float* dst, const float* src, size_t n) {
    Bracket br(e, s, K_COPY, 0.0, 8.0 * n);
    HIP_TRY(hipMemcpyAsync(dst, src, n * sizeof(float), hipMemcpyDeviceToDevice, s));
    return LOCO_OK;
}

int ensure_sin_rows(loco_encoder* e, int rows, hipStream_t s, const float** tab) {
    if (e->sin_rows.load(std::memory_order_acquire) >= rows) {
        *tab = e->sin_tab.load(std::memory_order_acquire);
        return LOCO_OK;
    }
    std::lock_guard<std::mutex> lock(e->sin_mu);
    if (e->sin_rows.load(std::memory_order_relaxed) >= rows) {
        *tab = e->sin_tab.load(std::memory_order_relaxed);
        return LOCO_OK;
    }
    int want = rows < 4002 ? 4002 : rows + 2;
    float* nt = nullptr;
    HIP_TRY(hipMalloc(&nt, (size_t)want * kHidden * sizeof(float)));
    hipError_t err = launch_sinusoid_table(nt, want, s);
    if (err == hipSuccess) err = hipStreamSynchronize(s);
    if (err != hipSuccess) {
        (void)hipFree(nt);
        return fail(LOCO_E_HIP, "sinusoid table: %s", hipGetErrorString(err));
    }
    if (float* old = e->sin_tab.load(std::memory_order_relaxed)) e->retired.push_back(old);
    e->sin_tab.store(nt, std::memory_order_release);
    e->sin_rows.store(want, std::memory_order_release);
    *tab = nt;
    e->sin_user = false;
    return LOCO_OK;
}


struct Bufs {
    int32_t* frames;
    const int32_t* frames_or_null;
    float *bufA, *bufB, *x0, *x1, *tmp, *ctx, *qkv, *qp, *ffn;
    _Float16 *xs0, *xs1;
    char* c0scratch;
    const int32_t* t0_clip = nullptr;
    const int32_t* rows_clip = nullptr;
    const float* sin_tab = nullptr;
};

Bufs carve_bufs(Call& c, const Plan& p, char* ws, int32_t* out_frames) {
    auto f32 = [ws](size_t off) { return reinterpret_cast<float*>(ws + off); };
    c.splitk = p.splitk ? f32(p.off_splitk) : nullptr;
    c.nslot = 0;
    return {out_frames ? out_frames : reinterpret_cast<int32_t*>(ws + p.off_frames), nullptr, f32(p.off_a), f32(p.off_b), f32(p.off_x0),
            f32(p.off_x1), f32(p.off_tmp), f32(p.off_ctx), f32(p.off_qkv), f32(p.off_qp), f32(p.off_ffn),
            reinterpret_cast<_Float16*>(ws + p.off_xs0), reinterpret_cast<_Float16*>(ws + p.off_xs1), ws + p.off_c0scratch};
}

int run_conv0(loco_encoder* e, hipStream_t s, const Plan& p, const float* wav, const Bufs& bf, float* y, _Float16* yhi, _Float16* ylo,
              float* range_slot) {
    const double outb = 4.0 * p.B * (double)p.Tc[0] * kConvDim;
    Bracket br(e, s, K_CONV0, 2.0 * 10 * p.B * (double)p.Tc[0] * kConvDim, outb + 8.0 * p.B * (double)p.L);
    HIP_TRY(launch_conv0_gn_gelu(wav, p.B, p.L, e->conv_w[0], e->stem.conv0_norm.w, e->stem.conv0_norm.b, y, bf.c0scratch, e->cfg.ln_eps, s,
                                 yhi, ylo, range_slot, bf.t0_clip));
    return LOCO_OK;
}

void planes(float* base, size_t n, _Float16*& hi, _Float16*& lo) {
    hi = reinterpret_cast<_Float16*>(base);
    lo = hi + n;
}

int prenet_f32(loco_encoder* e, const Plan& p, const float* wav, const Bufs& bf, hipStream_t s) {
    const int B = p.B;
    const long M = p.M;
    const StemW& sw = e->stem;
    int rc;
    if ((rc = run_conv0(e, s, p, wav, bf, bf.bufA, nullptr, nullptr, nullptr))) return rc;
    float* cin = bf.bufA;
    float* cout = bf.bufB;
    for (int i = 1; i < 7; ++i) {
        const long Tin = p.Tc[i - 1], Tout = p.Tc[i];
        rc = run_gemm(e, s, cin, (long)kConvS[i] * kConvDim, e->conv_w[i], (long)kConvK[i] * kConvDim, nullptr, nullptr, 0,
                      cout, kConvDim, (int)Tout, kConvDim, kConvK[i] * kConvDim, kEpiGelu, B, 1, Tin * kConvDim, 0,
                      Tout * kConvDim, 0);
        if (rc) return rc;
        std::swap(cin, cout);
    }
    float* feats = cin;
    if (e->tap_conv && (rc = run_copy(e, s, e->tap_conv, feats, (size_t)M * kConvDim))) return rc;

// ... 17 lines not shown
    const double tt = (double)B * kHeads * T * (double)T;
    Bracket br(e, s, K_ATTN_PROBS, 2.0 * 2.0 * tt * kHeadDim, 4.0 * tt);
    HIP_TRY(launch_attention_probs(qkv, qhi, qlo, khi, klo, qp, frames, e->attn_probs[l], B, T, 3, s));
    return LOCO_OK;
}

int encoder_f32(loco_encoder* e, const Plan& p, float* out, float* const* hidden_states, const Bufs& bf, hipStream_t s) {
    const int B = p.B;
    const int T = (int)p.T;
    const long M = p.M;
    int rc;
    float *x0 = bf.x0, *x1 = bf.x1, *tmp = bf.tmp, *ctx = bf.ctx, *qkv = bf.qkv, *qp = bf.qp, *ffn = bf.ffn;
    if ((rc = run_ln(e, s, x0, e->stem.layer_norm.w, e->stem.layer_norm.b, x0, M, kHidden))) return rc;
    const int nl = e->cfg.layers;
    for (int l = 0; l < nl; ++l) {
        if (hidden_states && hidden_states[l] && (rc = run_copy(e, s, hidden_states[l], x0, (size_t)M * kHidden))) return rc;
        const LayerW& lw = e->layers[l];
        if ((rc = run_gemm(e, s, x0, kHidden, lw.wqkv, kHidden, lw.bqkv, nullptr, 0, qkv, kQkv, (int)M, kQkv, kHidden, kEpiNone)))
            return rc;
        if ((rc = run_gemm(e, s, qkv, kQkv, e->stem.pe_k, kHeadDim, nullptr, nullptr, 0, qp, kRelN, T, kRelN, kHeadDim, kEpiNone, B,
                           kHeads, (long)T * kQkv, kHeadDim, (long)kHeads * T * kRelN, (long)T * kRelN)))
            return rc;
        {
            const double tt = (double)T * T;
            Bracket br(e, s, K_ATTN, 4.0 * B * kHeads * tt * kHeadDim, 4.0 * (M * (double)(kQkv + kHidden) + M * (double)kHeads * kRelN));
            HIP_TRY(launch_attention(qkv, qp, bf.frames_or_null, ctx, B, T, s));
        }
        if ((rc = run_attention_probs(e, s, qkv, nullptr, nullptr, nullptr, nullptr, qp, bf.frames_or_null, l, B, T))) return rc;
        if ((rc = run_gemm(e, s, ctx, kHidden, lw.out_proj.w, kHidden, lw.out_proj.b, x0, kHidden, tmp, kHidden, (int)M, kHidden, kHidden,
                           kEpiResidual)))
            return rc;
        if ((rc = run_ln(e, s, tmp, lw.layer_norm.w, lw.layer_norm.b, x1, M, kHidden))) return rc;
        if ((rc = run_gemm(e, s, x1, kHidden, lw.ffn_in.w, kHidden, lw.ffn_in.b, nullptr, 0, ffn, e->cfg.ffn, (int)M, e->cfg.ffn, kHidden,
                           kEpiGelu)))
            return rc;
        if ((rc = run_gemm(e, s, ffn, e->cfg.ffn, lw.ffn_out.w, e->cfg.ffn, lw.ffn_out.b, x1, kHidden, tmp, kHidden, (int)M, kHidden,
                           e->cfg.ffn, kEpiResidual)))
            return rc;
        float* dst = (l == nl - 1) ? out : x0;
        if ((rc = run_ln(e, s, tmp, lw.final_layer_norm.w, lw.final_layer_norm.b, dst, M, kHidden))) return rc;
    }
    if (nl == 0 && (rc = run_copy(e, s, out, x0, (size_t)M * kHidden))) return rc;
    if (hidden_states && hidden_states[nl] && (rc = run_copy(e, s, hidden_states[nl], out, (size_t)M * kHidden))) return rc;
    return LOCO_OK;
}

int prenet_f16x3(loco_encoder* e, Call& c, const Plan& p, const float* wav, const Bufs& bf, hipStream_t s) {
    const int B = p.B;
    const int T = (int)p.T;
    const long M = p.M;
    const StemW& sw = e->stem;
    int rc;
    static const char* const kConvNames[7] = {"feature_encoder.conv_layers.0 (GroupNorm + GELU)", "feature_encoder.conv_layers.1",
                                              "feature_encoder.conv_layers.2", "feature_encoder.conv_layers.3",
                                              "feature_encoder.conv_layers.4", "feature_encoder.conv_layers.5",
                                              "feature_encoder.conv_layers.6"};
    _Float16 *ihi, *ilo, *ohi, *olo;
    planes(bf.bufA, (size_t)B * p.Tc[0] * kConvDim, ihi, ilo);
    if ((rc = run_conv0(e, s, p, wav, bf, nullptr, ihi, ilo, c.slot(kConvNames[0])))) return rc;
    float* cin = bf.bufA;
    float* cout = bf.bufB;
    for (int i = 1; i < 7; ++i) {
        const long Tin = p.Tc[i - 1], Tout = p.Tc[i];
        planes(cin, (size_t)B * Tin * kConvDim, ihi, ilo);
        planes(cout, (size_t)B * Tout * kConvDim, ohi, olo);
        GemmSplitArgs a = split_args(Tout, kConvDim, kConvK[i] * kConvDim, kEpiGelu);
        a.Ahi = ihi; a.Alo = ilo; a.lda = (long)kConvS[i] * kConvDim; a.ktaps = kConvK[i];
        a.nb1 = B; a.sA1 = Tin * kConvDim; a.sC1 = Tout * kConvDim;
        if (i == 6) {
            a.C = cout;
        } else {
            a.Chi = ohi; a.Clo = olo;
            a.range_slot = c.slot(kConvNames[i]);
        }
        if ((rc = run_gemm_split(e, c, s, a, e->conv_s[i]))) return rc;
        std::swap(cin, cout);
    }
    float* feats = cin;
    if (e->tap_conv && (rc = run_copy(e, s, e->tap_conv, feats, (size_t)M * kConvDim))) return rc;

    planes(cout, (size_t)M * kConvDim, ohi, olo);
    if ((rc = run_ln(e, s, feats, sw.proj_norm.w, sw.proj_norm.b, nullptr, M, kConvDim, ohi, olo))) return rc;
    GemmSplitArgs a = split_args(M, kHidden, kConvDim, kEpiNone);
    a.Ahi = ohi; a.Alo = olo; a.bias = sw.proj.b; a.C = bf.x1;
    if ((rc = run_gemm_split(e, c, s, a, e->proj_s))) return rc;
    if (e->tap_proj && (rc = run_copy(e, s, e->tap_proj, bf.x1, (size_t)M * kHidden))) return rc;

    _Float16* ghi = reinterpret_cast<_Float16*>(bf.ffn);
    _Float16* glo = ghi + (size_t)B * kPosGroups * (T + kPosK) * kPosCg;
    {
        Bracket br(e, s, K_COPY, 0.0, 8.0 * M * kHidden);
        HIP_TRY(launch_group_major_split(bf.x1, ghi, glo, B, T, s, c.slot("feature_projection (input of pos_conv_embed)"), bf.rows_clip));
    }
    a = split_args(T, kPosCg, kPosK * kPosCg, kEpiPosConv);
    a.Ahi = ghi; a.Alo = glo; a.bias = sw.pos_b; a.R = bf.x1; a.C = bf.x0;
    a.lda = kPosCg; a.ldc = kHidden; a.ldr = kHidden;
    a.nb1 = B; a.nb2 = kPosGroups;
    a.sA1 = (long)kPosGroups * (T + kPosK) * kPosCg; a.sA2 = (long)(T + kPosK) * kPosCg;
    a.sC1 = (long)T * kHidden; a.sC2 = kPosCg;
    a.sW2 = (long)kPosCg * kPosK * kPosCg; a.sBias2 = kPosCg;
    a.sin_table = bf.sin_tab; a.frames = bf.frames_or_null; a.T = T;
    if ((rc = run_gemm_split(e, c, s, a, e->posg_s, K_POSCONV_SPLIT, 2.0 * M * (double)kHidden * kPosCg * kPosK, 8.0 * M * kHidden)))
        return rc;
    if (e->tap_prenet && (rc = run_copy(e, s, e->tap_prenet, bf.x0, (size_t)M * kHidden))) return rc;
    return LOCO_OK;
}

int encoder_f16x3(loco_encoder* e, Call& c, const Plan& p, float* out, float* const* hidden_states, const Bufs& bf, hipStream_t s) {
    const int B = p.B;
    const int T = (int)p.T;
    const long M = p.M;
    const int F = e->cfg.ffn;
    const size_t MH = (size_t)M * kHidden;
    int rc;
    float *x0 = bf.x0, *tmp = bf.tmp;
    _Float16* qshi = reinterpret_cast<_Float16*>(bf.qkv);
    _Float16* qslo = qshi + MH;
    _Float16* const kshi = qslo + MH;
    _Float16* const kslo = kshi + MH;
    _Float16* const vshi = kslo + MH;
    _Float16* const vslo = vshi + MH;
    _Float16 *x0hi = bf.xs0, *x0lo = bf.xs0 + MH;
    _Float16 *x1hi = bf.xs1, *x1lo = bf.xs1 + MH;
    _Float16 *chi, *clo, *fhi, *flo;
    planes(bf.ctx, MH, chi, clo);
    planes(bf.ffn, (size_t)M * F, fhi, flo);
    const int nl = e->cfg.layers;
    float* x0f = (hidden_states || nl == 0) ? x0 : nullptr;
    if ((rc = run_ln(e, s, x0, e->stem.layer_norm.w, e->stem.layer_norm.b, x0f, M, kHidden, x0hi, x0lo))) return rc;
    for (int l = 0; l < nl; ++l) {
        if (hidden_states && hidden_states[l] && (rc = run_copy(e, s, hidden_states[l], x0, MH))) return rc;
        const LayerW& lw = e->layers[l];
        GemmSplitArgs a = split_args(M, kQkv, kHidden, kEpiQkvScatter);
        a.Ahi = x0hi; a.Alo = x0lo; a.bias = lw.bqkv;
        a.Chi = qshi; a.Clo = qslo; a.ldc = kHidden; a.qkv_stride = (long)2 * M * kHidden; a.T = T;
        a.range_slot = c.slot("attention q|k|v projections", l);
        if ((rc = run_gemm_split(e, c, s, a, lw.sqkv))) return rc;
        dbg_planes(e, s, "x0 planes %s (layer input)", l, x0hi, x0lo, MH, kHidden);
        dbg_planes(e, s, "q planes %s", l, qshi, qslo, MH, kHidden);
        dbg_planes(e, s, "k planes %s", l, kshi, kslo, MH, kHidden);
        dbg_planes(e, s, "v planes %s", l, vshi, vslo, MH, kHidden);
        {
            const double tt = (double)T * T;
            Bracket br(e, s, K_ATTN_SPLIT, 4.0 * B * kHeads * tt * kHeadDim + 2.0 * M * (double)kHeads * kRelN * kHeadDim,
                       4.0 * (M * (double)(kQkv + kHidden)));
            HIP_TRY(launch_attention_f16x3(qshi, qslo, kshi, kslo, vshi, vslo, bf.qp, bf.frames_or_null, chi, clo, nullptr, B, T,
                                           s, e->pe_s.hi, e->pe_s.lo, e->pe_s.inv_scale));
        }
        if ((rc = run_attention_probs(e, s, nullptr, qshi, qslo, kshi, kslo, bf.qp, bf.frames_or_null, l, B, T))) return rc;
        dbg_planes(e, s, "attention context planes %s", l, chi, clo, MH, kHidden);
        a = split_args(M, kHidden, kHidden, kEpiResidual);
        a.Ahi = chi; a.Alo = clo; a.bias = lw.out_proj.b;
        a.Rhi = x0hi; a.Rlo = x0lo; a.ldr = kHidden; a.C = tmp;
        if ((rc = run_gemm_split(e, c, s, a, lw.so))) return rc;
        dbg_check(e, s, "out_proj + residual (fp32)", l, tmp, MH, false, kHidden);
        if ((rc = run_ln(e, s, tmp, lw.layer_norm.w, lw.layer_norm.b, nullptr, M, kHidden, x1hi, x1lo))) return rc;
        dbg_planes(e, s, "layer_norm planes %s", l, x1hi, x1lo, MH, kHidden);
        a = split_args(M, F, kHidden, kEpiGelu);
        a.Ahi = x1hi; a.Alo = x1lo; a.bias = lw.ffn_in.b;
        a.Chi = fhi; a.Clo = flo; a.range_slot = c.slot("feed_forward intermediate (GELU)", l);
        if ((rc = run_gemm_split(e, c, s, a, lw.s1))) return rc;
        dbg_planes(e, s, "feed_forward intermediate planes %s", l, fhi, flo, (size_t)M * F, F);
        a = split_args(M, kHidden, F, kEpiResidual);
        a.Ahi = fhi; a.Alo = flo; a.bias = lw.ffn_out.b;
        a.Rhi = x1hi; a.Rlo = x1lo; a.ldr = kHidden; a.C = tmp;
        if ((rc = run_gemm_split(e, c, s, a, lw.s2))) return rc;
        dbg_check(e, s, "feed_forward output + residual (fp32)", l, tmp, MH, false, kHidden);
        const bool last = l == nl - 1;
        if ((rc = run_ln(e, s, tmp, lw.final_layer_norm.w, lw.final_layer_norm.b, last ? out : (hidden_states ? x0 : nullptr), M, kHidden,
                         last ? nullptr : x0hi, last ? nullptr : x0lo,
                         last && c.range_dev ? c.range_dev + (size_t)kRangeShards * kFiniteStage : nullptr)))
            return rc;
    }
    if (nl == 0 && (rc = run_copy(e, s, out, x0, MH))) return rc;
    if (hidden_states && hidden_states[nl] && (rc = run_copy(e, s, hidden_states[nl], out, MH))) return rc;
    if (c.st) c.st->used = c.nslot;
    return LOCO_OK;
}

int encoder_stack(loco_encoder* e, Call& c, const Plan& p, float* out, float* const* hidden_states, const Bufs& bf, hipStream_t s) {
    return c.precision >= 1 ? encoder_f16x3(e, c, p, out, hidden_states, bf, s) : encoder_f32(e, p, out, hidden_states, bf, s);
}

int range_begin(loco_encoder* e, Call& c, hipStream_t s) {
    StatusBlock* st = c.st;
    st->magic = kStatusMagic;
    st->precision = c.precision;
    st->used = 0;
    st->msg[0] = 0;
    if (c.precision >= 1 && !e->range_static.empty()) snprintf(st->msg, sizeof st->msg, "%s", e->range_static.c_str());
    if (c.precision >= 1) HIP_TRY(hipMemsetAsync(c.range_dev, 0, sizeof(float) * kRangeMaxStages * kRangeShards, s));
    return LOCO_OK;
}
int range_end(const Call& c, hipStream_t s) {
    if (c.precision >= 1 && c.st->used > 0)
        HIP_TRY(hipMemcpyAsync(c.st->words, c.range_dev, sizeof(float) * kRangeShards * kRangeMaxStages, hipMemcpyDeviceToHost, s));
    return LOCO_OK;
}

template <class Half>
int enqueue(loco_encoder* e, int precision, StatusBlock* st, void* workspace, hipStream_t s, bool dual, const Half& half) {
    Call c;
    c.precision = precision;
    c.st = st;
    c.range_dev = reinterpret_cast<float*>(workspace);
    char* ws = reinterpret_cast<char*>(workspace) + kStatusDevBytes;
    int rc = range_begin(e, c, s);
    if (rc) return rc;
    if (!dual) {
        rc = half(c, 0, ws, s);
        return rc ? rc : range_end(c, s);
    }

    std::lock_guard<std::mutex> lock(e->side_mu);
    if (!e->side) {
        HIP_TRY(hipStreamCreateWithFlags(&e->side, hipStreamNonBlocking));
        HIP_TRY(hipEventCreateWithFlags(&e->ev_fork, hipEventDisableTiming));
        HIP_TRY(hipEventCreateWithFlags(&e->ev_join, hipEventDisableTiming));
    }
    HIP_TRY(hipEventRecord(e->ev_fork, s));
    HIP_TRY(hipStreamWaitEvent(e->side, e->ev_fork, 0));
    c.dual = true;
    rc = half(c, 0, ws, s);
    if (!rc) rc = half(c, 1, ws, e->side);
    c.dual = false;
    const hipError_t j1 = hipEventRecord(e->ev_join, e->side);
    const hipError_t j2 = j1 == hipSuccess ? hipStreamWaitEvent(s, e->ev_join, 0) : j1;
    if (j2 != hipSuccess) {
        (void)hipStreamSynchronize(e->side);
        if (!rc) return fail(LOCO_E_HIP, "loco_forward: joining the second stream failed: %s", hipGetErrorString(j2));
    }
    return rc ? rc : range_end(c, s);
}

template <class Run>
int with_status(const loco_encoder* e, const char* fn, int precision, void* status, const Run& run) {
    if (precision != -1 && !loco_precision_name(precision))
        return fail(LOCO_E_INVALID, "%s: precision must be -1 (the handle's mode) or one of " LOCO_PRECISION_MODES, fn);
    if (reinterpret_cast<uintptr_t>(status) & 7) return fail(LOCO_E_INVALID, "%s: the status block must be 8-byte aligned", fn);
    StatusBlock* st = reinterpret_cast<StatusBlock*>(status);
    st->magic = 0;
    const int rc = run(precision < 0 ? e->precision : precision, st);
    if (rc) st->magic = 0;
    return rc;
}

}

extern "C" {

int loco_abi_version(void) { return LOCO_ABI_VERSION; }

const char* loco_last_error(void) { return g_err.c_str(); }

void loco_default_config(loco_config* c) {
    if (!c) return;
    c->struct_size = (int32_t)sizeof(loco_config);
    c->hidden = kHidden;
    c->heads = kHeads;
    c->ffn = kFfn;
    c->layers = 12;
    c->conv_dim = kConvDim;
    c->pos_conv_kernel = kPosK;
    c->pos_conv_groups = kPosGroups;
    c->rel_max = kRelMax;
    c->ln_eps = 1e-5f;
}

loco_encoder* loco_create(const loco_config* cfg) {
    loco_config c;
    loco_default_config(&c);
    if (cfg) {
        if (cfg->struct_size != (int32_t)sizeof(loco_config)) {
            fail(LOCO_E_INVALID, "loco_config.struct_size %d != %zu", cfg->struct_size, sizeof(loco_config));
            return nullptr;
        }
        c = *cfg;
    }
    if (c.hidden != kHidden || c.heads != kHeads || c.ffn != kFfn || c.conv_dim != kConvDim ||
        c.pos_conv_kernel != kPosK || c.pos_conv_groups != kPosGroups || c.rel_max != kRelMax || c.layers < 0 ||
        c.layers > 64) {
        fail(LOCO_E_INVALID, "unsupported configuration: kernels are specialised for SpeechT5-base (768/12/3072/512/128/16/160)");
        return nullptr;
    }
    int dev = 0;
    if (hipGetDevice(&dev) != hipSuccess) {
        fail(LOCO_E_HIP, "hipGetDevice failed: no usable HIP device");
        return nullptr;
    }
    loco_encoder* e = new loco_encoder();
    e->cfg = c;
    e->device = dev;
    if (hipHostMalloc(reinterpret_cast<void**>(&e->own), sizeof(StatusBlock), hipHostMallocDefault) != hipSuccess ||
        hipMalloc(&e->absmax_dev, sizeof(float)) != hipSuccess) {
        fail(LOCO_E_HIP, "loco_create: could not allocate the range-status block");
        if (e->own) (void)hipHostFree(e->own);
        delete e;
        return nullptr;
    }
    memset(e->own, 0, sizeof(StatusBlock));
    e->own->magic = kStatusMagic;
    if (const char* dbg = getenv("LOCO_DEBUG_NONFINITE")) {
        e->debug_nonfinite = dbg[0] == '1' && hipMalloc(&e->debug_counter, 2 * sizeof(unsigned long long)) == hipSuccess;
    }
    e->layers.resize(c.layers);
    build_expected(e);
    for (int i = 0; i < K_COUNT; ++i) {
        memset(&e->stats[i], 0, sizeof(loco_kernel_stat));
        snprintf(e->stats[i].name, sizeof e->stats[i].name, "%s", kKernelNames[i]);
    }
    return e;
}

void loco_destroy(loco_encoder* e) {
    if (!e) return;
    for (auto& kv : e->raw) (void)hipFree(kv.second);
    for (int i = 1; i < 7; ++i) (void)hipFree(e->conv_w[i]);
    (void)hipFree(e->pos_w);
    auto free_split = [](SplitW& w) {
        (void)hipFree(w.hi);
        (void)hipFree(w.lo);
    };
    for (int i = 1; i < 7; ++i) free_split(e->conv_s[i]);
    free_split(e->proj_s);
// ... 661 lines not shown

static int drain_records(loco_encoder* e) {
    for (size_t i = 0; i < e->recs_used; ++i) {
        ProfRec& r = e->recs[i];
        HIP_TRY(hipEventSynchronize(r.b));
        float ms = 0.f;
        HIP_TRY(hipEventElapsedTime(&ms, r.a, r.b));
        loco_kernel_stat& st = e->stats[r.kid];
        st.launches += 1;
        st.ms += ms;
        st.flops += r.flops;
        st.bytes += r.bytes;
    }
    e->recs_used = 0;
    return LOCO_OK;
}

int loco_profile_reset(loco_encoder* e) {
    if (!e) return fail(LOCO_E_INVALID, "null encoder");
    int rc = drain_records(e);
    if (rc) return rc;
    for (int i = 0; i < K_COUNT; ++i) {
        e->stats[i].launches = 0;
        e->stats[i].ms = e->stats[i].flops = e->stats[i].bytes = 0.0;
    }
    return LOCO_OK;
}

int loco_profile_read(loco_encoder* e, loco_kernel_stat* stats, int max_stats) {
    if (!e || !stats) return fail(LOCO_E_INVALID, "null argument");
    int rc = drain_records(e);
    if (rc) return rc;
    int n = 0;
    for (int i = 0; i < K_COUNT && n < max_stats; ++i)
        if (e->stats[i].launches) stats[n++] = e->stats[i];
    return n;
}

int loco_op_layernorm(const float* x, const float* gamma, const float* beta, float* y, int64_t rows, int32_t dim, float eps,
                      void* stream) {
    if (!x || !gamma || !beta || !y) return fail(LOCO_E_INVALID, "loco_op_layernorm: null argument");
    if (dim != 512 && dim != 768) return fail(LOCO_E_INVALID, "loco_op_layernorm: dim %d not in {512,768}", dim);
    HIP_TRY(launch_layernorm(x, gamma, beta, y, rows, dim, eps, (hipStream_t)stream));
    return LOCO_OK;
}

int loco_op_gemm(const float* A, int64_t lda, const float* Wt, int64_t ldw, const float* bias, const float* R, int64_t ldr,
                 float* C, int64_t ldc, int32_t M, int32_t N, int32_t K, int32_t epilogue, int32_t nb1, int32_t nb2,
                 int64_t sA1, int64_t sA2, int64_t sC1, int64_t sC2, void* stream) {
    if (!A || !Wt || !C) return fail(LOCO_E_INVALID, "loco_op_gemm: null argument");
    if (K % 32 || (lda | ldw) & 3) return fail(LOCO_E_INVALID, "loco_op_gemm: K %% 32 and lda/ldw %% 4 must be 0");
    if (nb1 < 1 || nb2 < 1) return fail(LOCO_E_INVALID, "loco_op_gemm: batch counts must be >= 1");
    GemmArgs a{A, Wt, bias, R, C, M, N, K, lda, ldw, ldc, ldr, nb1, nb2, sA1, sA2, sC1, sC2, epilogue};
    HIP_TRY(launch_gemm(a, (hipStream_t)stream));
    return LOCO_OK;
}

size_t loco_conv0_scratch_bytes(int32_t B) { return conv0_scratch_bytes(B); }

int loco_op_conv0_gn_gelu(const float* wav, int32_t B, int64_t L, const float* w, const float* gn_w, const float* gn_b,
                          float* out, void* scratch, void* stream) {
    if (!wav || !w || !gn_w || !gn_b || !out || !scratch) return fail(LOCO_E_INVALID, "loco_op_conv0_gn_gelu: null argument");
    if (L < 10) return fail(LOCO_E_INVALID, "loco_op_conv0_gn_gelu: L < 10");
    HIP_TRY(launch_conv0_gn_gelu(wav, B, L, w, gn_w, gn_b, out, scratch, 1e-5f, (hipStream_t)stream));
    return LOCO_OK;
}

int loco_op_frame_counts(const int32_t* mask, int32_t B, int64_t L, int32_t* frames, void* stream) {
    if (!frames || B <= 0) return fail(LOCO_E_INVALID, "loco_op_frame_counts: invalid argument");
    HIP_TRY(launch_frame_counts(mask, B, L, frames, (hipStream_t)stream));
    return LOCO_OK;
}

int loco_op_pos_conv(const float* h, const float* w_folded, const float* bias, const float* sin_table, const int32_t* frames,
                     float* out, int32_t B, int32_t T, void* stream) {
    if (!h || !w_folded || !bias || !sin_table || !out) return fail(LOCO_E_INVALID, "loco_op_pos_conv: null argument");
    HIP_TRY(launch_pos_conv(h, w_folded, bias, sin_table, frames, out, B, T, (hipStream_t)stream));
    return LOCO_OK;
}


size_t loco_normalize_scratch_bytes(int32_t B) { return B > 0 ? normalize_scratch_bytes(B) : 0; }

int loco_op_normalize_waveform(const float* wav, const int32_t* attention_mask, int32_t B, int64_t L, float padding_value, float* out,
                               void* scratch, size_t scratch_bytes, void* stream) {
    if (!wav || !out || !scratch || B <= 0 || L <= 0) return fail(LOCO_E_INVALID, "loco_op_normalize_waveform: null/invalid argument");
    if (scratch_bytes < normalize_scratch_bytes(B) || (reinterpret_cast<uintptr_t>(scratch) & 7))
        return fail(LOCO_E_WORKSPACE, "loco_op_normalize_waveform: scratch %zu < %zu bytes (or not 8-byte aligned)", scratch_bytes,
                    normalize_scratch_bytes(B));
    HIP_TRY(launch_normalize_waveform(wav, attention_mask, B, L, padding_value, out, scratch, (hipStream_t)stream));
    return LOCO_OK;
}

int loco_resample_design(int32_t sr_in, int32_t sr_out, int32_t* up, int32_t* down, int32_t* taps_per_phase, float* taps_host) {
    if (!up || !down || !taps_per_phase) return fail(LOCO_E_INVALID, "loco_resample_design: null argument");
    int L = 0, M = 0, K = 0;
    const int rc = resample_design(sr_in, sr_out, &L, &M, &K, taps_host);
    if (rc) return fail(LOCO_E_INVALID, "loco_resample_design: unsupported rates %d -> %d Hz", sr_in, sr_out);
    *up = L; *down = M; *taps_per_phase = K;
    return LOCO_OK;
}

int64_t loco_resample_length(int64_t n_in, int32_t up, int32_t down) {
    if (n_in <= 0 || up <= 0 || down <= 0) return 0;
    return (n_in * up + down - 1) / down;
}

int loco_op_resample(const float* x, int32_t B, int64_t n_in, int64_t x_stride, const float* taps_dev, int32_t up, int32_t down,
                     int32_t taps_per_phase, float* y, int64_t n_out, int64_t y_stride, void* stream) {
    if (!x || !taps_dev || !y) return fail(LOCO_E_INVALID, "loco_op_resample: null argument");
    if (B <= 0 || n_in <= 0 || n_out <= 0 || n_out > loco_resample_length(n_in, up, down) || x_stride < n_in || y_stride < n_out ||
        (reinterpret_cast<uintptr_t>(taps_dev) & 15))
        return fail(LOCO_E_INVALID, "loco_op_resample: invalid shape (n_out must be <= ceil(n_in * up / down); taps 16-byte aligned)");
    HIP_TRY(launch_resample(x, B, n_in, x_stride, taps_dev, up, down, taps_per_phase, y, n_out, y_stride, (hipStream_t)stream));
    return LOCO_OK;
}

int loco_op_split_f16(const float* x, void* hi, void* lo, int64_t n, void* stream) {
    if (!x || !hi || !lo || n <= 0 || (n & 3)) return fail(LOCO_E_INVALID, "loco_op_split_f16: invalid argument");
    HIP_TRY(launch_split_f16(x, hi, lo, n, (hipStream_t)stream));
    return LOCO_OK;
}

int loco_op_gemm_f16x3(const void* Ahi, const void* Alo, int64_t lda, const void* Whi, const void* Wlo, int64_t ldw,
                       const float* bias, const float* R, int64_t ldr, float* C, void* Chi, void* Clo, int64_t ldc, int32_t M,
                       int32_t N, int32_t K, int32_t epilogue, int32_t nb1, int32_t nb2, int64_t sA1, int64_t sA2, int64_t sC1,
                       int64_t sC2, void* stream) {
    if (!Ahi || !Alo || !Whi || !Wlo || (!C && !Chi)) return fail(LOCO_E_INVALID, "loco_op_gemm_f16x3: null argument");
    if (K % 32 || (lda | ldw) & 7) return fail(LOCO_E_INVALID, "loco_op_gemm_f16x3: K %% 32 and lda/ldw %% 8 must be 0");
    GemmSplitArgs a{(const _Float16*)Ahi, (const _Float16*)Alo, (const _Float16*)Whi, (const _Float16*)Wlo, bias, R, C,
                    (_Float16*)Chi, (_Float16*)Clo, M, N, K, lda, ldw, ldc, ldr, nb1, nb2, sA1, sA2, sC1, sC2, epilogue};
    HIP_TRY(launch_gemm_split(a, (hipStream_t)stream));
    return LOCO_OK;
}

int loco_op_permute_conv_k(const float* w, float* out, int32_t N, int32_t taps, int32_t C, void* stream) {
    if (!w || !out) return fail(LOCO_E_INVALID, "loco_op_permute_conv_k: null argument");
    HIP_TRY(launch_permute_conv_k(w, out, N, taps, C, (hipStream_t)stream));
    return LOCO_OK;
}

int loco_op_conv_gemm_f16x3(const void* Ahi, const void* Alo, int64_t lda, const void* Whi, const void* Wlo, float* C, void* Chi, void* Clo,
                            int32_t Tout, int32_t N, int32_t Cin, int32_t taps, int32_t epilogue, int32_t B, int64_t sA1, void* stream) {
    if (!Ahi || !Alo || !Whi || !Wlo || (!C && !Chi)) return fail(LOCO_E_INVALID, "loco_op_conv_gemm_f16x3: null argument");
    if (taps < 1 || taps > 3 || Cin % 64 || lda & 7) return fail(LOCO_E_INVALID, "loco_op_conv_gemm_f16x3: taps in 1..3, Cin %% 64 and lda %% 8");
    const int K = taps * Cin;
    GemmSplitArgs a{(const _Float16*)Ahi, (const _Float16*)Alo, (const _Float16*)Whi, (const _Float16*)Wlo, nullptr, nullptr, C,
                    (_Float16*)Chi, (_Float16*)Clo, Tout, N, K, lda, K, N, 0, B, 1, sA1, 0, (int64_t)Tout * N, 0, epilogue};
    a.ktaps = taps;
    HIP_TRY(launch_gemm_split(a, (hipStream_t)stream));
    return LOCO_OK;
}

size_t loco_gemm_splitk_bytes(void) { return kSplitKBytes; }

void loco_debug_reload_gemm_knobs(void) {
    reload_gemm_knobs();
    reload_attention_knobs();
}

int loco_op_gemm_f16x3_splitk(const void* Ahi, const void* Alo, int64_t lda, const void* Whi, const void* Wlo, int64_t ldw,
                              const float* bias, const float* R, int64_t ldr, float* C, void* Chi, void* Clo, int64_t ldc, int32_t M,
                              int32_t N, int32_t K, int32_t epilogue, void* splitk_ws, size_t splitk_bytes, void* stream) {
    if (!Ahi || !Alo || !Whi || !Wlo || (!C && !Chi) || !splitk_ws) return fail(LOCO_E_INVALID, "loco_op_gemm_f16x3_splitk: null argument");
    if (K % 32 || (lda | ldw) & 7) return fail(LOCO_E_INVALID, "loco_op_gemm_f16x3_splitk: K %% 32 and lda/ldw %% 8 must be 0");
    if (splitk_bytes < kSplitKBytes) return fail(LOCO_E_WORKSPACE, "loco_op_gemm_f16x3_splitk: workspace %zu < %zu bytes", splitk_bytes, kSplitKBytes);
    GemmSplitArgs a{(const _Float16*)Ahi, (const _Float16*)Alo, (const _Float16*)Whi, (const _Float16*)Wlo, bias, R, C,
                    (_Float16*)Chi, (_Float16*)Clo, M, N, K, lda, ldw, ldc, ldr, 1, 1, 0, 0, 0, 0, epilogue};
    a.splitk_ws = reinterpret_cast<float*>(splitk_ws);
    HIP_TRY(launch_gemm_split(a, (hipStream_t)stream));
    return LOCO_OK;
}

int loco_op_attention_f16x3(const void* qhi, const void* qlo, const void* khi, const void* klo, const void* vhi, const void* vlo,
                            const float* qp, const int32_t* frames, float* ctx, int32_t B, int32_t T, void* stream) {
    if (!qhi || !qlo || !khi || !klo || !vhi || !vlo || !qp || !ctx) return fail(LOCO_E_INVALID, "loco_op_attention_f16x3: null argument");
    HIP_TRY(launch_attention_f16x3((const _Float16*)qhi, (const _Float16*)qlo, (const _Float16*)khi, (const _Float16*)klo,
                                   (const _Float16*)vhi, (const _Float16*)vlo, qp, frames, nullptr, nullptr, ctx, B, T,
                                   (hipStream_t)stream));
    return LOCO_OK;
}

int loco_op_attention_f16x3_pe(const void* qhi, const void* qlo, const void* khi, const void* klo, const void* vhi, const void* vlo,
                               const void* pe_hi, const void* pe_lo, float pe_scale, float* qp_scratch, const int32_t* frames, float* ctx,
                               int32_t B, int32_t T, void* stream) {
    if (!qhi || !qlo || !khi || !klo || !vhi || !vlo || !pe_hi || !pe_lo || !qp_scratch || !ctx)
        return fail(LOCO_E_INVALID, "loco_op_attention_f16x3_pe: null argument");
    HIP_TRY(launch_attention_f16x3((const _Float16*)qhi, (const _Float16*)qlo, (const _Float16*)khi, (const _Float16*)klo,
                                   (const _Float16*)vhi, (const _Float16*)vlo, qp_scratch, frames, nullptr, nullptr, ctx, B, T,
                                   (hipStream_t)stream, (const _Float16*)pe_hi, (const _Float16*)pe_lo, pe_scale));
    return LOCO_OK;
}

int loco_op_attention_probs(const float* qkv, const float* qp, const int32_t* frames, float* probs, int32_t B, int32_t T, void* stream) {
    if (!qkv || !qp || !probs) return fail(LOCO_E_INVALID, "loco_op_attention_probs: null argument");
    HIP_TRY(launch_attention_probs(qkv, nullptr, nullptr, nullptr, nullptr, qp, frames, probs, B, T, 3, (hipStream_t)stream));
    return LOCO_OK;
}

int loco_op_attention_probs_f16x3(const void* qhi, const void* qlo, const void* khi, const void* klo, const float* qp, const int32_t* frames,
                                  float* probs, int32_t B, int32_t T, int32_t terms, void* stream) {
    if (!qhi || !qlo || !khi || !klo || !qp || !probs) return fail(LOCO_E_INVALID, "loco_op_attention_probs_f16x3: null argument");
    if (terms != 2 && terms != 3) return fail(LOCO_E_INVALID, "loco_op_attention_probs_f16x3: terms must be 2 or 3");
    HIP_TRY(launch_attention_probs(nullptr, (const _Float16*)qhi, (const _Float16*)qlo, (const _Float16*)khi, (const _Float16*)klo, qp,
                                   frames, probs, B, T, terms, (hipStream_t)stream));
    return LOCO_OK;
}

int loco_op_attention(const float* qkv, const float* qp, const int32_t* frames, float* ctx, int32_t B, int32_t T, void* stream) {
    if (!qkv || !qp || !ctx) return fail(LOCO_E_INVALID, "loco_op_attention: null argument");
    HIP_TRY(launch_attention(qkv, qp, frames, ctx, B, T, (hipStream_t)stream));
    return LOCO_OK;
}

}

namespace {

struct DecPlan {
    int B, T, S, L;
    size_t off_state, off_lengths, off_frames, off_tokens, off_nonpad, off_finished, off_cross, off_self, off_x0, off_x1, off_tmp, off_q,
        off_ctx, off_ffn, off_logits, off_attn, total;
};

void make_dec_plan(int layers, int B, int T, int S, DecPlan& p) {
    p.B = B, p.T = T, p.S = S, p.L = layers;
    const size_t f = sizeof(float), rows = (size_t)B * S;
    size_t o = 0;
    auto take = [&](size_t bytes) {
        size_t at = o;
        o += align_up(bytes);
        return at;
    };
    p.off_state = take(4 * sizeof(int32_t));
    p.off_lengths = take((size_t)B * sizeof(int32_t));
    p.off_frames = take((size_t)B * sizeof(int32_t));
    p.off_tokens = take(rows * sizeof(int32_t));
    p.off_nonpad = take(rows * sizeof(int32_t));
    p.off_finished = take(rows * sizeof(int32_t));
    p.off_cross = take((size_t)B * T * p.L * 2 * kHidden * f);
    p.off_self = take((size_t)p.L * rows * 2 * kHidden * f);
    p.off_x0 = take(rows * kHidden * f);
    p.off_x1 = take(rows * kHidden * f);
    p.off_tmp = take(rows * kHidden * f);
    p.off_q = take(rows * kHidden * f);
    p.off_ctx = take(rows * kHidden * f);
    p.off_ffn = take(rows * kFfn * f);
    p.off_logits = take((size_t)B * 128 * f);
    size_t attn = dec_attention_scratch_bytes(B, S, T);
    for (size_t v : {dec_attention_scratch_bytes(B, S, S), dec_attention_scratch_bytes(B, 1, T), dec_attention_scratch_bytes(B, 1, S)})
        attn = v > attn ? v : attn;
    p.off_attn = take(attn);
    p.total = o;
}

int dec_check(const loco_encoder* e, const char* fn, int B, int T, int S, const void* ws, size_t bytes, DecPlan& p) {
    if (!e) return fail(LOCO_E_INVALID, "%s: null encoder", fn);
    if (!e->finalized || !e->dec.ready)
        return fail(LOCO_E_STATE, "%s: the handle has no decoder weights (decoder.prenet.*, decoder.wrapped_decoder.*, text_decoder_postnet.*) or "
                                  "loco_finalize_weights has not run", fn);
    if (B <= 0 || T <= 0 || S <= 0) return fail(LOCO_E_INVALID, "%s: B, T_enc and the sequence length must be positive", fn);
    if (S > kDecMaxPositions) return fail(LOCO_E_INVALID, "%s: %d positions exceed max_text_positions = %d", fn, S, kDecMaxPositions);
    if (!ws) return fail(LOCO_E_INVALID, "%s: null workspace", fn);
    make_dec_plan(e->dec.layers, B, T, S, p);
    if (bytes < p.total) return fail(LOCO_E_WORKSPACE, "%s: workspace %zu < %zu bytes", fn, bytes, p.total);
    return LOCO_OK;
}

int run_skinny(hipStream_t s, const float* A, const WB& w, const float* R, float* C, int M, int N, int K, int epi) {
    HIP_TRY(launch_skinny_gemm(A, K, w.w, K, w.b, R, N, C, N, nullptr, 0, N, M, N, K, epi, s));
    return LOCO_OK;
}

int dec_cross_kv(loco_encoder* e, const DecPlan& p, char* ws, const float* enc_out, hipStream_t s) {
    const int N = p.L * 2 * kHidden;
    return run_gemm(e, s, enc_out, kHidden, e->dec.wckv, kHidden, e->dec.bckv, nullptr, 0, reinterpret_cast<float*>(ws + p.off_cross), N,
                    p.B * p.T, N, kHidden, kEpiNone);
}

int dec_attention(hipStream_t s, const float* q, long ldq, long sq, const float* kv, long ldk, long sk, const int32_t* kcount, float* out,
                  int B, int Sq, int Tk, int causal, float* scratch) {
    HIP_TRY(launch_dec_attention(q, ldq, sq, kv, ldk, sk, kv + kHidden, ldk, sk, kcount, out, kHidden, (long)Sq * kHidden, B, Sq, Tk, causal, 0,
                                 1.0f, scratch, s));
    return LOCO_OK;
}

#define DEC_TRY(expr)           \
    do {                        \
        const int rc_ = (expr); \
        if (rc_) return rc_;    \
    } while (0)

int dec_step(loco_encoder* e, const DecPlan& p, char* ws, int t, float* logits_out, hipStream_t s) {
    const DecoderW& d = e->dec;
    const int B = p.B;
    auto F = [&](size_t off) { return reinterpret_cast<float*>(ws + off); };
    auto I = [&](size_t off) { return reinterpret_cast<int32_t*>(ws + off); };
    float *x0 = F(p.off_x0), *x1 = F(p.off_x1), *tmp = F(p.off_tmp), *q = F(p.off_q), *ctx = F(p.off_ctx), *ffn = F(p.off_ffn), *scr = F(p.off_attn);
    float* logits = logits_out ? logits_out : F(p.off_logits);
    const long ld_cross = (long)p.L * 2 * kHidden, ld_self = 2 * kHidden;
    HIP_TRY(launch_dec_embed_step(I(p.off_tokens), p.S, t, d.embed, d.vocab, d.pos_tab, d.pos_rows, I(p.off_nonpad), x0, B, s));
    for (int l = 0; l < p.L; ++l) {
        const DecLayerW& lw = d.L[l];
        float* cache = F(p.off_self) + (size_t)l * B * p.S * ld_self;
        HIP_TRY(launch_skinny_gemm(x0, kHidden, lw.wqkv, kHidden, lw.bqkv, nullptr, 0, q, kHidden, cache + (size_t)t * ld_self, (long)p.S * ld_self,
                                   kHidden, B, kQkv, kHidden, kEpiNone, s));
// ... 174 lines not shown
```

### loco-asr_amd/csrc/loco_kernels.h

```cpp
#pragma once
#include <hip/hip_runtime.h>
#include <stdint.h>

namespace loco {

typedef float f32x4 __attribute__((ext_vector_type(4)));
typedef float f32x16 __attribute__((ext_vector_type(16)));

constexpr int kHidden = 768;
constexpr int kHeads = 12;
constexpr int kHeadDim = 64;
constexpr int kFfn = 3072;
constexpr int kConvDim = 512;
constexpr int kPosK = 128;
constexpr int kPosGroups = 16;
constexpr int kPosCg = 48;
constexpr int kRelMax = 160;
constexpr int kRelN = 320;
constexpr int kQkv = 3 * kHidden;

constexpr size_t kSplitKBytes = (size_t)256 * 256 * 128 * sizeof(float);
constexpr int kSplitKMaxM = 8192;

enum Epilogue { kEpiNone = 0, kEpiGelu = 1, kEpiResidual = 2, kEpiQkvScatter = 3, kEpiPosConv = 4 };

struct GemmArgs {
    const float* A;
    const float* W;
    const float* bias;
    const float* R;
    float* C;
    int M, N, K;
    long lda, ldw, ldc, ldr;
    int nb1, nb2;
    long sA1, sA2, sC1, sC2;
    int epilogue;
};

struct GemmSplitArgs {
    const _Float16* Ahi;
    const _Float16* Alo;
    const _Float16* Whi;
    const _Float16* Wlo;
    const float* bias;
    const float* R;
    float* C;
    _Float16* Chi;
    _Float16* Clo;
    int M, N, K;
    long lda, ldw, ldc, ldr;
    int nb1, nb2;
    long sA1, sA2, sC1, sC2;
    int epilogue;
    const _Float16* Rhi = nullptr;
    const _Float16* Rlo = nullptr;
    float* splitk_ws = nullptr;
    long qkv_stride = 0;
    int T = 0;
    float out_scale = 1.0f;
    int terms = 3;
    bool co_scheduled = false;
    int ktaps = 1;
    int kchan = 0;
    int kt_per_z2 = 0;
    float* range_slot = nullptr;
    long sW2 = 0;
    int z1_inner = 1;
    long sA1i = 0, sW1i = 0;
    long sBias2 = 0;
    const float* sin_table = nullptr;
    const int32_t* frames = nullptr;
};
hipError_t launch_group_major_split(const float* x, void* hi, void* lo, int B, int T, hipStream_t s, float* range_slot = nullptr,
                                    const int32_t* rows_clip = nullptr);
hipError_t launch_pos_w_for_gemm(const float* wf, float* out, hipStream_t s);
hipError_t launch_attention_f16x3(const _Float16* qhi, const _Float16* qlo, const _Float16* khi, const _Float16* klo,
                                  const _Float16* vhi, const _Float16* vlo, const float* qp, const int32_t* frames,
                                  _Float16* ctx_hi, _Float16* ctx_lo, float* ctx, int B, int T, hipStream_t s,
                                  const _Float16* pe_hi = nullptr, const _Float16* pe_lo = nullptr, float pe_scale = 1.0f);
hipError_t launch_gemm_split(const GemmSplitArgs& a, hipStream_t s);
void reload_gemm_knobs();
void reload_attention_knobs();
hipError_t launch_split_f16(const float* x, void* hi, void* lo, long n, hipStream_t s, float scale = 1.0f);
hipError_t launch_absmax(const float* x, long n, float* out, hipStream_t s);

hipError_t launch_count_nonfinite(const void* x, long n, bool half, unsigned long long* out, hipStream_t s);

constexpr int kRangeShards = 8;
constexpr int kRangeMaxStages = 96;
constexpr int kFiniteStage = kRangeMaxStages - 1;
__device__ __forceinline__ unsigned range_peek(const float* slot) {
    if (!slot) return 0xffffffffu;
    return __hip_atomic_load(reinterpret_cast<const unsigned*>(slot) + (blockIdx.x & (kRangeShards - 1)), __ATOMIC_RELAXED,
                             __HIP_MEMORY_SCOPE_AGENT);
}
__device__ __forceinline__ float wave_max_nonneg(float v) {
#define LOCO_DPP_MAX(ctrl) \
    v = fmaxf(v, __builtin_bit_cast(float, __builtin_amdgcn_update_dpp(0, __builtin_bit_cast(int, v), ctrl, 0xf, 0xf, true)))
    LOCO_DPP_MAX(0xB1);
    LOCO_DPP_MAX(0x4E);
    LOCO_DPP_MAX(0x141);
    LOCO_DPP_MAX(0x140);
#undef LOCO_DPP_MAX
    const int b = __builtin_bit_cast(int, v);
    const float r0 = __builtin_bit_cast(float, __builtin_amdgcn_readlane(b, 0)), r1 = __builtin_bit_cast(float, __builtin_amdgcn_readlane(b, 16));
    const float r2 = __builtin_bit_cast(float, __builtin_amdgcn_readlane(b, 32)), r3 = __builtin_bit_cast(float, __builtin_amdgcn_readlane(b, 48));
    return fmaxf(fmaxf(r0, r1), fmaxf(r2, r3));
}
__device__ __forceinline__ void range_commit(float* slot, float amax, unsigned seen) {
    if (!slot) return;
    const unsigned bits = __float_as_uint(wave_max_nonneg(amax));
    if ((threadIdx.x & 63) == 0 && bits > seen)
        atomicMax(reinterpret_cast<unsigned*>(slot) + (blockIdx.x & (kRangeShards - 1)), bits);
}

__device__ __forceinline__ void range_commit_block(float* slot, float amax, unsigned seen) {
    if (!slot) return;
    __shared__ float wmax[16];
    const float w = wave_max_nonneg(amax);
    if ((threadIdx.x & 63) == 0) wmax[threadIdx.x >> 6] = w;
    __syncthreads();
    if (threadIdx.x == 0) {
        float m = wmax[0];
        for (unsigned i = 1; i < (blockDim.x + 63) / 64; ++i) m = fmaxf(m, wmax[i]);
        const unsigned bits = __float_as_uint(m);
        if (bits > seen) atomicMax(reinterpret_cast<unsigned*>(slot) + (blockIdx.x & (kRangeShards - 1)), bits);
    }
}


__device__ __forceinline__ float gelu_erf(float x) {
    constexpr float kSMax = 5.79827547f;
    const float s = fminf(fabsf(x), kSMax);
    float q = 2.171883651e-08f;
    q = fmaf(q, s, -6.759613029e-07f);
    q = fmaf(q, s, 9.013814633e-06f);
    q = fmaf(q, s, -6.522983313e-05f);
    q = fmaf(q, s, 2.421164681e-04f);
    q = fmaf(q, s, 7.379760791e-05f);
    q = fmaf(q, s, -7.028903347e-03f);
    q = fmaf(q, s, 5.248807371e-02f);
    q = fmaf(q, s, 4.592096508e-01f);
    q = fmaf(q, s, 1.151104808e+00f);
    const float h = 0.5f * __builtin_amdgcn_exp2f(-(q * s));
    return x >= 0.f ? x * (1.0f - h) : (x < -kSMax ? -kSMax : x) * h;
}

__device__ __forceinline__ void split_f16_2pairs(float a0, float a1, float b0, float b1, unsigned& hia, unsigned& loa, unsigned& hib,
                                                 unsigned& lob) {
    typedef _Float16 h2_ __attribute__((ext_vector_type(2)));
    asm volatile("" : "+v"(a0), "+v"(a1), "+v"(b0), "+v"(b1));
    const h2_ ha = {(_Float16)a0, (_Float16)a1}, hb = {(_Float16)b0, (_Float16)b1};
    hia = __builtin_bit_cast(unsigned, ha);
    hib = __builtin_bit_cast(unsigned, hb);
    asm("v_fma_mixlo_f16 %0, %2, 1.0, -%6 op_sel_hi:[0,0,1]\n\t"
        "v_fma_mixlo_f16 %1, %4, 1.0, -%7 op_sel_hi:[0,0,1]\n\t"
        "v_fma_mixhi_f16 %0, %3, 1.0, -%6 op_sel:[0,0,1] op_sel_hi:[0,0,1]\n\t"
        "v_fma_mixhi_f16 %1, %5, 1.0, -%7 op_sel:[0,0,1] op_sel_hi:[0,0,1]"
        : "=&v"(loa), "=&v"(lob)
        : "v"(a0), "v"(a1), "v"(b0), "v"(b1), "v"(hia), "v"(hib));
}

typedef float f32x2_t __attribute__((ext_vector_type(2)));
__device__ __forceinline__ f32x2_t gelu_erf2(f32x2_t x) {
    constexpr float kSMax = 5.79827547f;
    const f32x2_t s = {fminf(fabsf(x.x), kSMax), fminf(fabsf(x.y), kSMax)};
#define LOCO_Q2(c) (f32x2_t){(c), (c)}
    f32x2_t q = LOCO_Q2(2.171883651e-08f);
    q = __builtin_elementwise_fma(q, s, LOCO_Q2(-6.759613029e-07f));
    q = __builtin_elementwise_fma(q, s, LOCO_Q2(9.013814633e-06f));
    q = __builtin_elementwise_fma(q, s, LOCO_Q2(-6.522983313e-05f));
    q = __builtin_elementwise_fma(q, s, LOCO_Q2(2.421164681e-04f));
    q = __builtin_elementwise_fma(q, s, LOCO_Q2(7.379760791e-05f));
    q = __builtin_elementwise_fma(q, s, LOCO_Q2(-7.028903347e-03f));
    q = __builtin_elementwise_fma(q, s, LOCO_Q2(5.248807371e-02f));
    q = __builtin_elementwise_fma(q, s, LOCO_Q2(4.592096508e-01f));
    q = __builtin_elementwise_fma(q, s, LOCO_Q2(1.151104808e+00f));
#undef LOCO_Q2
    const f32x2_t u = q * s;
    const f32x2_t h = {0.5f * __builtin_amdgcn_exp2f(-u.x), 0.5f * __builtin_amdgcn_exp2f(-u.y)};
    f32x2_t r;
    r.x = x.x >= 0.f ? x.x * (1.0f - h.x) : (x.x < -kSMax ? -kSMax : x.x) * h.x;
    r.y = x.y >= 0.f ? x.y * (1.0f - h.y) : (x.y < -kSMax ? -kSMax : x.y) * h.y;
    return r;
}

hipError_t launch_gemm(const GemmArgs& a, hipStream_t s);
hipError_t launch_layernorm(const float* x, const float* g, const float* b, float* y, long rows, int dim, float eps,
                            hipStream_t s, void* yhi = nullptr, void* ylo = nullptr, float* nonfinite_slot = nullptr);

constexpr int kConv0Parts = 64;
constexpr int kConv0Moments = 65;
size_t conv0_scratch_bytes(int B);
hipError_t launch_conv0_gn_gelu(const float* wav, int B, long L, const float* w, const float* gn_w, const float* gn_b,
                                float* out, void* scratch, float eps, hipStream_t s, void* out_hi = nullptr,
                                void* out_lo = nullptr, float* range_slot = nullptr, const int32_t* t0_clip = nullptr);
hipError_t launch_frame_counts(const int32_t* mask, int B, long L, int32_t* frames, hipStream_t s);
size_t normalize_scratch_bytes(int B);
hipError_t launch_normalize_waveform(const float* wav, const int32_t* mask, int B, long L, float pad, float* out, void* scratch,
                                     hipStream_t s);
hipError_t launch_token_counts(const int32_t* mask, int B, int T, int32_t* frames, hipStream_t s);
hipError_t launch_text_prenet(const int32_t* ids, const float* embed, int vocab, const float* alpha, const float* pe, int B, int T,
                              float* out, hipStream_t s);
hipError_t launch_text_pe_table(float* pe, int rows, hipStream_t s);
hipError_t launch_pos_conv(const float* h, const float* wf, const float* bias, const float* sin_table,
                           const int32_t* frames, float* out, int B, int T, hipStream_t s, const int32_t* rows_clip = nullptr);
hipError_t launch_attention(const float* qkv, const float* qp, const int32_t* frames, float* ctx, int B, int T,
                            hipStream_t s, void* ctx_hi = nullptr, void* ctx_lo = nullptr);
hipError_t launch_attention_probs(const float* qkv, const _Float16* qhi, const _Float16* qlo, const _Float16* khi, const _Float16* klo,
                                  const float* qp, const int32_t* frames, float* probs, int B, int T, int terms, hipStream_t s);

hipError_t launch_relayout_conv_weight(const float* w, float* out, int N, int C, int k, hipStream_t s);
hipError_t launch_fold_pos_conv(const float* g, const float* v, float* out, hipStream_t s);
hipError_t launch_scale_copy(const float* src, float* dst, long n, float scale, hipStream_t s);
hipError_t launch_permute_conv_k(const float* src, float* dst, int N, int taps, int C, hipStream_t s);
hipError_t launch_sinusoid_table(float* tab, int rows, hipStream_t s);

int resample_design(int sr_in, int sr_out, int* L_out, int* M_out, int* K_out, float* taps);
hipError_t launch_resample(const float* x, int B, long n_in, long x_stride, const float* taps, int L, int M, int K, float* y, long n_out,
                           long y_stride, hipStream_t s);

constexpr int kSkinnyMaxM = 64;
constexpr int kDecAttnMaxSplit = 64;
hipError_t launch_skinny_gemm(const float* A, long lda, const float* W, long ldw, const float* bias, const float* R, long ldr, float* C,
                              long ldc, float* C2, long ldc2, int nsplit, int M, int N, int K, int epilogue, hipStream_t s);
int skinny_gemm_slices(int N, int K);
int dec_attention_splits(int B, int Sq, int Tk);
size_t dec_attention_scratch_bytes(int B, int Sq, int Tk);
hipError_t launch_dec_attention(const float* q, long ldq, long sq, const float* k, long ldk, long sk, const float* v, long ldv, long sv,
                                const int32_t* kcount, float* out, long ldo, long so, int B, int Sq, int Tk, int causal, int causal_offset,
                                float scale, float* scratch, hipStream_t s);
hipError_t launch_dec_embed(const int32_t* ids, long ld_ids, const float* embed, int vocab, const float* table, int table_rows, float* x,
                            int B, int S, int32_t* positions, hipStream_t s);
hipError_t launch_dec_embed_step(const int32_t* tokens, int S_max, int t, const float* embed, int vocab, const float* table, int table_rows,
                                 int32_t* nonpad, float* x, int B, hipStream_t s);
hipError_t launch_dec_select(const float* logits, int vocab, int B, int32_t* tokens, int S_max, int t, int32_t* finished, int32_t* lengths,
                             int32_t* state, int eos, int pad, hipStream_t s);
hipError_t launch_dec_begin(int32_t* tokens, int B, int S_max, int start, int pad, int32_t* lengths, int32_t* state, hipStream_t s);

inline long conv_out_len(long n, int k, int s) { return n < k ? 0 : (n - k) / s + 1; }

}
```

### loco-asr_amd/csrc/norm_misc.hip

```cpp
#include "loco_kernels.h"

namespace loco {

__device__ __forceinline__ float wave_sum(float v) {
#pragma unroll
    for (int o = 32; o > 0; o >>= 1) v += __shfl_xor(v, o, 64);
    return v;
}

typedef _Float16 h4_t __attribute__((ext_vector_type(4)));

template <int NV4, bool SPLIT>
__global__ __launch_bounds__(256) void layernorm_kernel(const float* __restrict__ x, const float* __restrict__ g,
                                                        const float* __restrict__ b, float* __restrict__ y,
                                                        _Float16* __restrict__ yhi, _Float16* __restrict__ ylo, long rows,
                                                        float eps, float* __restrict__ nonfinite_slot) {
    constexpr int D = NV4 * 256;
    const int lane = threadIdx.x & 63;
    const long row = (long)blockIdx.x * 4 + (threadIdx.x >> 6);
    if (row >= rows) return;
    const float4* xr = reinterpret_cast<const float4*>(x + row * D);
    float4 v[NV4];
    float s = 0.f;
#pragma unroll
    for (int i = 0; i < NV4; ++i) {
        v[i] = xr[lane + 64 * i];
        s += (v[i].x + v[i].y) + (v[i].z + v[i].w);
    }
    const float mean = wave_sum(s) * (1.0f / D);
    float q = 0.f;
#pragma unroll
    for (int i = 0; i < NV4; ++i) {
        v[i].x -= mean; v[i].y -= mean; v[i].z -= mean; v[i].w -= mean;
        q += (v[i].x * v[i].x + v[i].y * v[i].y) + (v[i].z * v[i].z + v[i].w * v[i].w);
    }
    const float rstd = 1.0f / sqrtf(wave_sum(q) * (1.0f / D) + eps);
    if (nonfinite_slot && lane == 0 && !(rstd > 0.f)) atomicMax(reinterpret_cast<unsigned*>(nonfinite_slot) + (blockIdx.x & 7), 0x7f800000u);
#pragma unroll
    for (int i = 0; i < NV4; ++i) {
        const float4 gg = reinterpret_cast<const float4*>(g)[lane + 64 * i];
        const float4 bb = reinterpret_cast<const float4*>(b)[lane + 64 * i];
        float o[4];
        o[0] = v[i].x * rstd * gg.x + bb.x;
        o[1] = v[i].y * rstd * gg.y + bb.y;
        o[2] = v[i].z * rstd * gg.z + bb.z;
        o[3] = v[i].w * rstd * gg.w + bb.w;
        if (y) reinterpret_cast<float4*>(y + row * D)[lane + 64 * i] = make_float4(o[0], o[1], o[2], o[3]);
        if (SPLIT) {
            typedef unsigned u32x2_t __attribute__((ext_vector_type(2)));
            unsigned h0, l0, h1, l1;
            split_f16_2pairs(o[0], o[1], o[2], o[3], h0, l0, h1, l1);
            reinterpret_cast<u32x2_t*>(yhi + row * D)[lane + 64 * i] = u32x2_t{h0, h1};
            reinterpret_cast<u32x2_t*>(ylo + row * D)[lane + 64 * i] = u32x2_t{l0, l1};
        }
    }
}

hipError_t launch_layernorm(const float* x, const float* g, const float* b, float* y, long rows, int dim, float eps,
                            hipStream_t s, void* yhi, void* ylo, float* nonfinite_slot) {
    if (rows <= 0 || (!y && !yhi) || ((yhi == nullptr) != (ylo == nullptr))) return hipErrorInvalidValue;
    const unsigned grid = (unsigned)((rows + 3) / 4);
    _Float16* hi = (_Float16*)yhi;
    _Float16* lo = (_Float16*)ylo;
    if (dim == 768 && !hi)
        hipLaunchKernelGGL((layernorm_kernel<3, false>), dim3(grid), dim3(256), 0, s, x, g, b, y, hi, lo, rows, eps, nonfinite_slot);
    else if (dim == 768)
        hipLaunchKernelGGL((layernorm_kernel<3, true>), dim3(grid), dim3(256), 0, s, x, g, b, y, hi, lo, rows, eps, nonfinite_slot);
    else if (dim == 512 && !hi)
        hipLaunchKernelGGL((layernorm_kernel<2, false>), dim3(grid), dim3(256), 0, s, x, g, b, y, hi, lo, rows, eps, nonfinite_slot);
    else if (dim == 512)
        hipLaunchKernelGGL((layernorm_kernel<2, true>), dim3(grid), dim3(256), 0, s, x, g, b, y, hi, lo, rows, eps, nonfinite_slot);
    else
        return hipErrorInvalidValue;
    return hipGetLastError();
}

__global__ __launch_bounds__(256) void mask_count_kernel(const int32_t* __restrict__ mask, long L, int32_t* __restrict__ frames) {
    __shared__ int part[4];
    const int b = blockIdx.y;
    const int32_t* m = mask + (long)b * L;
    const long per = (((L + gridDim.x - 1) / gridDim.x) + 3) & ~3L;
    const long i0 = (long)blockIdx.x * per;
    long i1 = i0 + per;
    i1 = i1 < L ? i1 : L;
    i1 = i1 < i0 ? i0 : i1;
    int n = 0;
    if ((reinterpret_cast<uintptr_t>(m) & 15) == 0) {
        const long v1 = i0 + ((i1 - i0) & ~3L);
        for (long i = i0 + 4 * threadIdx.x; i < v1; i += 1024) {
            const int4 v = *reinterpret_cast<const int4*>(m + i);
            n += (v.x + v.y) + (v.z + v.w);
        }
        for (long i = v1 + threadIdx.x; i < i1; i += 256) n += m[i];
    } else {
        for (long i = i0 + threadIdx.x; i < i1; i += 256) n += m[i];
    }
#pragma unroll
    for (int o = 32; o > 0; o >>= 1) n += __shfl_xor(n, o, 64);
    if ((threadIdx.x & 63) == 0) part[threadIdx.x >> 6] = n;
    __syncthreads();
    if (threadIdx.x == 0) atomicAdd(&frames[b], (part[0] + part[1]) + (part[2] + part[3]));
}

__global__ void frames_from_counts_kernel(int32_t* __restrict__ frames, int B, long L, int have_mask) {
    const int b = blockIdx.x * blockDim.x + threadIdx.x;
    if (b >= B) return;
    long n = have_mask ? (long)frames[b] : L;
    const int ks[7] = {10, 3, 3, 3, 3, 2, 2}, ss[7] = {5, 2, 2, 2, 2, 2, 2};
    for (int i = 0; i < 7; ++i) {
        const long d = n - ks[i];
        n = (d >= 0 ? d / ss[i] : -((-d + ss[i] - 1) / ss[i])) + 1;
    }
    frames[b] = (int32_t)n;
}

hipError_t launch_frame_counts(const int32_t* mask, int B, long L, int32_t* frames, hipStream_t s) {
    if (B <= 0 || B > 65535) return hipErrorInvalidValue;
    if (mask) {
        hipError_t e = hipMemsetAsync(frames, 0, (size_t)B * sizeof(int32_t), s);
        if (e != hipSuccess) return e;
        long parts = (L + 65535) / 65536;
        parts = parts < 1 ? 1 : (parts > 256 ? 256 : parts);
        hipLaunchKernelGGL(mask_count_kernel, dim3((unsigned)parts, B), dim3(256), 0, s, mask, L, frames);
    }
    hipLaunchKernelGGL(frames_from_counts_kernel, dim3((B + 63) / 64), dim3(64), 0, s, frames, B, L, mask ? 1 : 0);
    return hipGetLastError();
}

constexpr int kNormParts = 128;

__global__ __launch_bounds__(256) void wav_moments_kernel(const float* __restrict__ x, long L, const int32_t* __restrict__ counts,
                                                          double* __restrict__ part) {
    const int b = blockIdx.y;
    const long n = counts ? counts[b] : L;
    const long chunk = ((n + kNormParts - 1) / kNormParts + 3) & ~3L;
    long i0 = (long)blockIdx.x * chunk, i1 = i0 + chunk;
    i1 = i1 < n ? i1 : n;
    const float* xb = x + (long)b * L;
    double s = 0.0, q = 0.0;
    for (long i = i0 + threadIdx.x; i < i1; i += 256) {
        const double v = xb[i];
        s += v;
        q += v * v;
    }
    __shared__ double sh[2][256];
    sh[0][threadIdx.x] = s;
    sh[1][threadIdx.x] = q;
    __syncthreads();
    for (int w = 128; w > 0; w >>= 1) {
        if ((int)threadIdx.x < w) {
            sh[0][threadIdx.x] += sh[0][threadIdx.x + w];
            sh[1][threadIdx.x] += sh[1][threadIdx.x + w];
        }
        __syncthreads();
    }
    if (threadIdx.x == 0) {
        part[((long)b * kNormParts + blockIdx.x) * 2] = sh[0][0];
        part[((long)b * kNormParts + blockIdx.x) * 2 + 1] = sh[1][0];
    }
}

__global__ void wav_norm_coeffs_kernel(const double* __restrict__ part, const int32_t* __restrict__ counts, long L, int B,
                                       float* __restrict__ coef) {
    const int b = blockIdx.x * blockDim.x + threadIdx.x;
    if (b >= B) return;
    const long n = counts ? counts[b] : L;
    double s = 0.0, q = 0.0;
    for (int p = 0; p < kNormParts; ++p) {
        s += part[((long)b * kNormParts + p) * 2];
        q += part[((long)b * kNormParts + p) * 2 + 1];
    }
    const double mean = n > 0 ? s / (double)n : 0.0;
    double var = n > 0 ? q / (double)n - mean * mean : 0.0;
    var = var > 0.0 ? var : 0.0;
    coef[2 * b] = (float)mean;
    coef[2 * b + 1] = (float)(1.0 / sqrt(var + 1e-7));
}

__global__ __launch_bounds__(256) void wav_norm_apply_kernel(const float* __restrict__ x, long L, const int32_t* __restrict__ counts,
                                                             const float* __restrict__ coef, float pad, float* __restrict__ out) {
    const int b = blockIdx.y;
    const long n = counts ? counts[b] : L;
    const float mean = coef[2 * b], rstd = coef[2 * b + 1];
    const float* xb = x + (long)b * L;
    float* ob = out + (long)b * L;
    for (long i = (long)blockIdx.x * 256 + threadIdx.x; i < L; i += (long)gridDim.x * 256)
        ob[i] = i < n ? (xb[i] - mean) * rstd : pad;
}

size_t normalize_scratch_bytes(int B) { return ((size_t)B * (kNormParts * 2 * sizeof(double) + 2 * sizeof(float) + sizeof(int32_t)) + 255) & ~size_t(255); }

hipError_t launch_normalize_waveform(const float* wav, const int32_t* mask, int B, long L, float pad, float* out, void* scratch,
                                     hipStream_t s) {
    if (B <= 0 || B > 65535 || L <= 0) return hipErrorInvalidValue;
    double* part = reinterpret_cast<double*>(scratch);
    float* coef = reinterpret_cast<float*>(part + (size_t)B * kNormParts * 2);
    int32_t* counts = nullptr;
    if (mask) {
        counts = reinterpret_cast<int32_t*>(coef + (size_t)2 * B);
        hipError_t e = hipMemsetAsync(counts, 0, (size_t)B * sizeof(int32_t), s);
        if (e != hipSuccess) return e;
        long parts = (L + 65535) / 65536;
        parts = parts < 1 ? 1 : (parts > 256 ? 256 : parts);
        hipLaunchKernelGGL(mask_count_kernel, dim3((unsigned)parts, B), dim3(256), 0, s, mask, L, counts);
    }
    hipLaunchKernelGGL(wav_moments_kernel, dim3(kNormParts, B), dim3(256), 0, s, wav, L, counts, part);
    hipLaunchKernelGGL(wav_norm_coeffs_kernel, dim3((B + 63) / 64), dim3(64), 0, s, part, counts, L, B, coef);
    long blocks = (L + 255) / 256;
// ... 199 lines not shown
```

Before: 975,300 frames/s.

## Fuse post-residual LayerNorm into the persistent GEMM via row-block walk

Adds an LNTAIL mode to the persistent f16x3 GEMM. Each workgroup owns a row block and walks every column tile of the 768-wide output, then runs LayerNorm on those completed rows in-kernel, writing the fp32 output and/or the fp16 hi/lo split. This removes the separate LayerNorm launch and its re-read of C after residual GEMMs. In exchange, the tile scheduling becomes row-major per workgroup, which may hurt load balance and L2 reuse of weights. The tile-cost model gains a form 9 that is chosen only when enough row blocks exist.

```diff
diff --git a/include/loco_asr.h b/include/loco_asr.h
--- a/include/loco_asr.h
+++ b/include/loco_asr.h
@@ -147,6 +147,11 @@
                        const float* bias, const float* R, int64_t ldr, float* C, void* Chi, void* Clo, int64_t ldc,
                        int32_t M, int32_t N, int32_t K, int32_t epilogue, int32_t nb1, int32_t nb2, int64_t sA1, int64_t sA2,
                        int64_t sC1, int64_t sC2, void* stream);
+
+int loco_op_gemm_f16x3_ln(const void* Ahi, const void* Alo, const void* Whi, const void* Wlo, const float* bias, const void* Rhi,
+                          const void* Rlo, float* C, const float* gamma, const float* beta, float eps, float* y, void* yhi, void* ylo,
+                          int32_t M, int32_t K, int32_t* fused, void* stream);
+int loco_debug_gemm_tile_form(int32_t M, int32_t N, int32_t K, int32_t epilogue, int32_t with_layernorm, int32_t co_scheduled);
 
 int loco_op_permute_conv_k(const float* w, float* out, int32_t N, int32_t taps, int32_t Cin, void* stream);
 int loco_op_conv_gemm_f16x3(const void* Ahi, const void* Alo, int64_t lda, const void* Whi, const void* Wlo, float* C, void* Chi,
diff --git a/loco-asr_amd/_lib.py b/loco-asr_amd/_lib.py
--- a/loco-asr_amd/_lib.py
+++ b/loco-asr_amd/_lib.py
@@ -87,6 +87,8 @@
                                             _vp, _sz, _vp]),
     "loco_op_gemm_f16x3": (C.c_int, [_vp, _vp, _i64, _vp, _vp, _i64, _vp, _vp, _i64, _vp, _vp, _vp, _i64, _i32, _i32, _i32, _i32,
                                      _i32, _i32, _i64, _i64, _i64, _i64, _vp]),
+    "loco_op_gemm_f16x3_ln": (C.c_int, [_vp, _vp, _vp, _vp, _vp, _vp, _vp, _vp, _vp, _vp, _f, _vp, _vp, _vp, _i32, _i32, _vp, _vp]),
+    "loco_debug_gemm_tile_form": (C.c_int, [_i32, _i32, _i32, _i32, _i32, _i32]),
     "loco_op_permute_conv_k": (C.c_int, [_vp, _vp, _i32, _i32, _i32, _vp]),
     "loco_op_conv_gemm_f16x3": (C.c_int, [_vp, _vp, _i64, _vp, _vp, _vp, _vp, _vp, _i32, _i32, _i32, _i32, _i32, _i32, _i64, _vp]),
     "loco_op_attention_f16x3": (C.c_int, [_vp, _vp, _vp, _vp, _vp, _vp, _vp, _vp, _vp, _i32, _i32, _vp]),
diff --git a/loco-asr_amd/csrc/gemm_f16x3.hip b/loco-asr_amd/csrc/gemm_f16x3.hip
--- a/loco-asr_amd/csrc/gemm_f16x3.hip
+++ b/loco-asr_amd/csrc/gemm_f16x3.hip
@@ -165,7 +165,8 @@
         asm volatile("s_waitcnt vmcnt(%0) lgkmcnt(0)" ::"n"(n_) : "memory");                         \
     }
 
-template <int EPI, bool OUT_SPLIT, int WM, int WN, int AST, int WST, int NJ = 4, int WPS = 0, int TERMS = 3, bool PERSIST = false>
+template <int EPI, bool OUT_SPLIT, int WM, int WN, int AST, int WST, int NJ = 4, int WPS = 0, int TERMS = 3, bool PERSIST = false,
+          bool LNTAIL = false>
 __global__ __launch_bounds__(64 * WM * WN, WPS ? WPS : (WM * WN) / 4) void gemm_f16x3_dma_kernel(GemmSplitArgs p, int tiles_m,
                                                                                                   int tiles_n, int nblk, int wg_step,
                                                                                                   int col_group) {
@@ -175,6 +176,7 @@
     constexpr int NDA = DBM / 16 / NW_;
     constexpr int NDW = (DBN / 16 + NW_ - 1) / NW_;
     constexpr int WPIECES = DBN / 16;
+    static_assert(!LNTAIL || (PERSIST && EPI == kEpiResidual && !OUT_SPLIT && NJ == 4), "the LayerNorm tail belongs to the persistent residual form");
     constexpr int NA = 2 * NDA, NWP = (TERMS == 3 ? 2 : 1) * NDW;
     static_assert(NDA >= 1 && DBM % (16 * NW_) == 0, "tile too small for the wave count");
     static_assert((AST == WST && AST >= 2 && AST <= 5) || (AST == 3 && WST == 2), "ring depths: equal rings of 2-5 slots, or 3 A + 2 W");
@@ -201,29 +203,38 @@
         run_start = xcd < rr ? xcd * (q + 1) : rr * (q + 1) + (xcd - rr) * q;
         run_len = q + (xcd < rr ? 1 : 0);
     }
+    if (LNTAIL && tile_i >= run_len) return;
+    int nt_cur = 0;
     struct Tile {
         const char *bAh, *bAl, *bWh, *bWl;
         unsigned va[NDA], vw[NDW];
         int m0, n0, z1, z2, kt0;
         long coff;
     };
-    auto decode = [&](int i, Tile& t_) {
-        const int t = run_start + i;
-        const int per_z = tiles_m * tiles_n;
-        const int z = t / per_z;
-        const int tz = t - z * per_z;
-        const int full = tiles_n / col_group;
-        int g = tz / (tiles_m * col_group), rem, width;
-        if (g < full) {
-            rem = tz - g * tiles_m * col_group;
-            width = col_group;
+    auto decode = [&](int i, int ntw, Tile& t_) {
+        int z, mt, nt;
+        if (LNTAIL) {
+            z = 0;
+            mt = run_start + i;
+            nt = ntw;
         } else {
-            g = full;
-            rem = tz - full * tiles_m * col_group;
-            width = tiles_n - full * col_group;
-        }
-        const int mt = rem / width;
-        const int nt = g * col_group + (rem - mt * width);
+            const int t = run_start + i;
+            const int per_z = tiles_m * tiles_n;
+            z = t / per_z;
+            const int tz = t - z * per_z;
+            const int full = tiles_n / col_group;
+            int g = tz / (tiles_m * col_group), rem, width;
+            if (g < full) {
+                rem = tz - g * tiles_m * col_group;
+                width = col_group;
+            } else {
+                g = full;
+                rem = tz - full * tiles_m * col_group;
+                width = tiles_n - full * col_group;
+            }
+            mt = rem / width;
+            nt = g * col_group + (rem - mt * width);
+        }
         t_.z1 = z / p.nb2;
         t_.z2 = z % p.nb2;
         t_.kt0 = t_.z2 * p.kt_per_z2;
@@ -253,7 +264,7 @@
         t_.bWl = reinterpret_cast<const char*>(p.Wlo + woff + (long)t_.n0 * p.ldw);
     };
     Tile cur, nxt;
-    decode(tile_i, cur);
+    decode(tile_i, 0, cur);
     nxt = cur;
 
     const int ktaps = p.ktaps, kchan2 = 2 * (p.kchan ? p.kchan : p.K / (p.ktaps > 0 ? p.ktaps : 1));
@@ -361,8 +372,9 @@
         SB()                                                                                    \
     }
     for (;;) {
-        const bool has_next = PERSIST && wg_step > 0 && tile_i + wg_step < run_len;
-        if (PERSIST && has_next) decode(tile_i + wg_step, nxt);
+        const bool more_cols = LNTAIL && nt_cur + 1 < tiles_n;
+        const bool has_next = PERSIST && wg_step > 0 && (more_cols || tile_i + wg_step < run_len);
+        if (PERSIST && has_next) decode(more_cols ? tile_i : tile_i + wg_step, more_cols ? nt_cur + 1 : 0, nxt);
 #pragma unroll
         for (int i = 0; i < 4; ++i)
 #pragma unroll
@@ -472,9 +484,25 @@
                 if (OUT_SPLIT || EPI == kEpiQkvScatter) range_commit(p.range_slot, amax, seen);
             }
         }
+        if (LNTAIL && !more_cols) {
+            asm volatile("s_waitcnt vmcnt(0)" ::: "memory");
+            __threadfence_block();
+            __builtin_amdgcn_s_barrier();
+            const int nrows = p.M - cur.m0 < DBM ? p.M - cur.m0 : DBM;
+            const float* x = p.C + cur.coff;
+            for (int r = wave; r < nrows; r += NW_) {
+                if (p.ln_hi) layernorm_row<kHidden / 256, true>(x, p.ln_gamma, p.ln_beta, p.ln_y, p.ln_hi, p.ln_lo, (long)cur.m0 + r, lane, p.ln_eps, p.ln_nonfinite);
+                else layernorm_row<kHidden / 256, false>(x, p.ln_gamma, p.ln_beta, p.ln_y, nullptr, nullptr, (long)cur.m0 + r, lane, p.ln_eps, p.ln_nonfinite);
+            }
+        }
         if (!PERSIST || !has_next) break;
         cur = nxt;
-        tile_i += wg_step;
+        if (LNTAIL && more_cols) {
+            ++nt_cur;
+        } else {
+            nt_cur = 0;
+            tile_i += wg_step;
+        }
     }
     asm volatile("s_waitcnt vmcnt(0)" ::: "memory");
 #undef DMA_AFTER_BLOCK
@@ -686,7 +714,7 @@
 
 struct GemmKnobs {
     int tile = 0, narrow = 0;
-    bool nopersist = false, nocolgroup = false, no192 = false, nosplitk = false, posconv_generic = false;
+    bool nopersist = false, nocolgroup = false, no192 = false, nosplitk = false, posconv_generic = false, nolnfuse = false;
     int posconv_ni = 0;
 };
 static GemmKnobs read_gemm_knobs() {
@@ -697,6 +725,7 @@
     k.nopersist = getenv("LOCO_GEMM_NOPERSIST") != nullptr;
     k.nocolgroup = getenv("LOCO_GEMM_NOCOLGROUP") != nullptr;
     k.no192 = getenv("LOCO_GEMM_NO192") != nullptr;
+    k.nolnfuse = getenv("LOCO_GEMM_NOLNFUSE") != nullptr;
     k.posconv_generic = getenv("LOCO_POSCONV_GENERIC") != nullptr;
     if ((v = getenv("LOCO_POSCONV_NI"))) k.posconv_ni = (atoi(v) == 2 || atoi(v) == 4) ? atoi(v) : 0;
     k.nosplitk = getenv("LOCO_GEMM_NOSPLITK") != nullptr;
@@ -708,7 +737,7 @@
 }
 void reload_gemm_knobs() { gemm_knobs() = read_gemm_knobs(); }
 
-template <int WM, int WN, int AST, int WST, int WPS, int TERMS = 3>
+template <int WM, int WN, int AST, int WST, int WPS, int TERMS = 3, bool LNT = false>
 static hipError_t launch_tile(const GemmSplitArgs& a, hipStream_t s) {
     constexpr int bm = 64 * WM, bn = 64 * WN;
     const int tm = (a.M + bm - 1) / bm, tn = (a.N + bn - 1) / bn;
@@ -722,6 +751,13 @@
     const int wg_step = persist ? slots / 8 : 0;
     const int ngroups = (tn + 5) / 6;
     const int col_group = gemm_knobs().nocolgroup ? tn : (tn + ngroups - 1) / ngroups;
+    if constexpr (LNT) {
+        static_assert(kPersist && WPS == 0, "the row-block walk is a mode of the one-per-CU persistent form");
+        if (a.epilogue != kEpiResidual || sp || a.nb1 * a.nb2 != 1 || tn * bn != a.N || a.K / SBK < AST) return hipErrorInvalidValue;
+        hipLaunchKernelGGL((gemm_f16x3_dma_kernel<kEpiResidual, false, WM, WN, AST, WST, 4, WPS, TERMS, true, true>), dim3(slots),
+                           dim3(64 * WM * WN), 0, s, a, tm, tn, tm, slots / 8, tn);
+        return hipGetLastError();
+    }
 #define TILE_LAUNCH(EPI)                                                                                                              \
     if (sp) hipLaunchKernelGGL((gemm_f16x3_dma_kernel<EPI, true, WM, WN, AST, WST, 4, WPS, TERMS, kPersist>), dim3(grid), dim3(64 * WM * WN), 0, \
                                s, a, tm, tn, (int)nb, wg_step, col_group);                                                            \
@@ -738,7 +774,46 @@
     return hipGetLastError();
 }
 
-hipError_t launch_gemm_split(const GemmSplitArgs& a, hipStream_t s) {
+static bool ln_fusable(const GemmSplitArgs& a) {
+    if (!a.ln_gamma || !a.ln_beta || (!a.ln_y && !a.ln_hi) || ((a.ln_hi == nullptr) != (a.ln_lo == nullptr))) return false;
+    if (a.epilogue != kEpiResidual || a.Chi || !a.C || a.N != kHidden || a.ldc != kHidden || a.nb1 * a.nb2 != 1 || a.ktaps != 1) return false;
+    if (a.co_scheduled || gemm_knobs().nolnfuse || gemm_knobs().nopersist || a.K / SBK < 3) return false;
+    return (long)((a.M + 191) / 192) * (kHidden / 256) > 256;
+}
+constexpr double kEffLnFused = 0.92;
+
+static int choose_tile(const GemmSplitArgs& a) {
+    int tile = gemm_knobs().tile;
+    if (tile == 9 && !ln_fusable(a)) tile = 6;
+    if (tile == 0) {
+        const long rows_total = (long)a.M * a.nb1 * a.nb2;
+        if (rows_total >= 1024 && a.K <= 128) {
+            tile = 4;
+        } else if (rows_total >= 1024) {
+            struct Form { int id, bm, bn; double eff; bool n256; };
+            static const Form kForms[] = {{1, 256, 256, 1.00, true}, {6, 192, 256, 0.91, true}, {9, 192, 256, kEffLnFused, true},
+                                          {2, 256, 128, 0.80, false}, {5, 128, 128, 0.55, false}};
+            double best = 0.0;
+            for (const Form& f : kForms) {
+                if (f.n256 && a.N % 256 != 0) continue;
+                if ((f.id == 6 || f.id == 9) && gemm_knobs().no192) continue;
+                if (f.id == 9 && !ln_fusable(a)) continue;
+                const double tiles = (double)((a.M + f.bm - 1) / f.bm) * ((a.N + f.bn - 1) / f.bn) * a.nb1 * a.nb2;
+                const double rounds = f.id == 9 ? (double)(((a.M + f.bm - 1) / f.bm + 255) / 256) * (a.N / f.bn)
+                                                : (a.co_scheduled ? tiles / 256.0 : (double)(((long)tiles + 255) / 256));
+                const double cost = rounds * f.bm * f.bn / f.eff;
+                if (tile == 0 || cost < best) { tile = f.id; best = cost; }
+            }
+            if (tile == 2 && gemm_knobs().narrow) tile = gemm_knobs().narrow;
+        } else {
+            tile = 5;
+        }
+    }
+    return tile;
+}
+
+hipError_t launch_gemm_split(const GemmSplitArgs& a, hipStream_t s, bool* ln_fused) {
+    if (ln_fused) *ln_fused = false;
     if (a.M <= 0 || a.N <= 0 || a.K <= 0 || a.K % SBK != 0) return hipErrorInvalidValue;
     if ((a.lda | a.ldw | a.sA1 | a.sA2) & 7) return hipErrorInvalidValue;
     if ((a.N | a.ldc | a.sC1 | a.sC2) & 3) return hipErrorInvalidValue;
@@ -848,34 +923,15 @@
             return hipGetLastError();
         }
     }
-    int tile = gemm_knobs().tile;
-    if (tile == 0) {
-        const long rows_total = (long)a.M * a.nb1 * a.nb2;
-        if (rows_total >= 1024 && a.K <= 128) {
-            tile = 4;
-        } else if (rows_total >= 1024) {
-            struct Form { int id, bm, bn; double eff; bool n256; };
-            static const Form kForms[] = {{1, 256, 256, 1.00, true}, {6, 192, 256, 0.91, true}, {2, 256, 128, 0.80, false}, {5, 128, 128, 0.55, false}};
-            double best = 0.0;
-            for (const Form& f : kForms) {
-                if (f.n256 && a.N % 256 != 0) continue;
-                if (f.id == 6 && gemm_knobs().no192) continue;
-                const double tiles = (double)((a.M + f.bm - 1) / f.bm) * ((a.N + f.bn - 1) / f.bn) * a.nb1 * a.nb2;
-                const double rounds = a.co_scheduled ? tiles / 256.0 : (double)(((long)tiles + 255) / 256);
-                const double cost = rounds * f.bm * f.bn / f.eff;
-                if (tile == 0 || cost < best) { tile = f.id; best = cost; }
-            }
-            if (tile == 2 && gemm_knobs().narrow) tile = gemm_knobs().narrow;
-        } else {
-            tile = 5;
-        }
-    }
+    const int tile = choose_tile(a);
+    if (ln_fused) *ln_fused = tile == 9;
     if (a.terms == 2) {
         switch (tile) {
             case 1: return launch_tile<4, 4, 3, 2, 0, 2>(a, s);
             case 2: return launch_tile<4, 2, 3, 3, 0, 2>(a, s);
             case 4: return launch_tile<2, 2, 2, 2, 2, 2>(a, s);
             case 6: return launch_tile<3, 4, 3, 2, 0, 2>(a, s);
+            case 9: return launch_tile<3, 4, 3, 2, 0, 2, true>(a, s);
             case 3:
             case 5: return launch_tile<2, 2, 3, 3, 0, 2>(a, s);
             default: return hipErrorInvalidValue;
@@ -889,9 +945,16 @@
         case 5: return launch_tile<2, 2, 3, 3, 0>(a, s);
         case 8: return launch_tile<2, 2, 5, 5, 0>(a, s);
         case 6: return launch_tile<3, 4, 3, 2, 0>(a, s);
+        case 9: return launch_tile<3, 4, 3, 2, 0, 3, true>(a, s);
         case 7: return launch_tile<4, 4, 2, 2, 0>(a, s);
         default: return hipErrorInvalidValue;
     }
+}
+
+int gemm_split_tile_form(const GemmSplitArgs& a) {
+    if (a.epilogue == kEpiPosConv) return 0;
+    if (a.splitk_ws && a.nb1 * a.nb2 == 1 && a.M <= kSplitKMaxM && !gemm_knobs().nosplitk) return 0;
+    return choose_tile(a);
 }
 
 __global__ void split_f16_kernel(const float* __restrict__ x, _Float16* __restrict__ hi, _Float16* __restrict__ lo, long n4, float scale) {
diff --git a/loco-asr_amd/csrc/loco_api.hip b/loco-asr_amd/csrc/loco_api.hip
--- a/loco-asr_amd/csrc/loco_api.hip
+++ b/loco-asr_amd/csrc/loco_api.hip
@@ -444,6 +444,32 @@
                           gemm_bytes(a.M, a.N, a.K, a.nb1, a.nb2, a.epilogue));
 }
 
+int dbg_check(loco_encoder* e, hipStream_t s, const char* stage, int layer, const void* p, size_t n, bool half, long row_len);
+
+int run_gemm_split_ln(loco_encoder* e, const Call& c, hipStream_t s, GemmSplitArgs a, const SplitW& w, const WB& ln, float* y,
+                      _Float16* yhi, _Float16* ylo, float* nonfinite_slot, const char* dbg_stage, int layer) {
+    a.Whi = w.hi;
+    a.Wlo = w.lo;
+    a.out_scale = w.inv_scale;
+    a.terms = c.precision == 2 ? 2 : 3;
+    a.co_scheduled = c.dual;
+    a.splitk_ws = c.splitk;
+    a.ln_gamma = ln.w; a.ln_beta = ln.b; a.ln_eps = e->cfg.ln_eps;
+    a.ln_y = y; a.ln_hi = yhi; a.ln_lo = ylo; a.ln_nonfinite = nonfinite_slot;
+    const bool fuse = gemm_split_tile_form(a) == 9;
+    if (!fuse) a.ln_gamma = nullptr;
+    bool fused = false;
+    {
+        Bracket br(e, s, K_GEMM_SPLIT, gemm_flops(a.M, a.N, a.K, 1, 1),
+                   gemm_bytes(a.M, a.N, a.K, 1, 1, a.epilogue) + (fuse ? (y && yhi ? 8.0 : 4.0) * a.M * (double)a.N : 0.0));
+        HIP_TRY(launch_gemm_split(a, s, &fused));
+    }
+    if (fused != fuse) return fail(LOCO_E_HIP, "gemm + LayerNorm: the launcher did not take the form it announced");
+    dbg_check(e, s, dbg_stage, layer, a.C, (size_t)a.M * a.N, false, a.N);
+    if (fused) return LOCO_OK;
+    return run_ln(e, s, a.C, ln.w, ln.b, y, a.M, a.N, yhi, ylo, nonfinite_slot);
+}
+
 int absmax_host(loco_encoder* e, const float* src, size_t n, hipStream_t s, float& out) {
     HIP_TRY(hipMemsetAsync(e->absmax_dev, 0, sizeof(float), s));
     HIP_TRY(launch_absmax(src, (long)n, e->absmax_dev, s));
@@ -767,9 +793,7 @@
         a = split_args(M, kHidden, kHidden, kEpiResidual);
         a.Ahi = chi; a.Alo = clo; a.bias = lw.out_proj.b;
         a.Rhi = x0hi; a.Rlo = x0lo; a.ldr = kHidden; a.C = tmp;
-        if ((rc = run_gemm_split(e, c, s, a, lw.so))) return rc;
-        dbg_check(e, s, "out_proj + residual (fp32)", l, tmp, MH, false, kHidden);
-        if ((rc = run_ln(e, s, tmp, lw.layer_norm.w, lw.layer_norm.b, nullptr, M, kHidden, x1hi, x1lo))) return rc;
+        if ((rc = run_gemm_split_ln(e, c, s, a, lw.so, lw.layer_norm, nullptr, x1hi, x1lo, nullptr, "out_proj + residual (fp32)", l))) return rc;
         dbg_planes(e, s, "layer_norm planes %s", l, x1hi, x1lo, MH, kHidden);
         a = split_args(M, F, kHidden, kEpiGelu);
         a.Ahi = x1hi; a.Alo = x1lo; a.bias = lw.ffn_in.b;
@@ -779,12 +803,10 @@
         a = split_args(M, kHidden, F, kEpiResidual);
         a.Ahi = fhi; a.Alo = flo; a.bias = lw.ffn_out.b;
         a.Rhi = x1hi; a.Rlo = x1lo; a.ldr = kHidden; a.C = tmp;
-        if ((rc = run_gemm_split(e, c, s, a, lw.s2))) return rc;
-        dbg_check(e, s, "feed_forward output + residual (fp32)", l, tmp, MH, false, kHidden);
         const bool last = l == nl - 1;
-        if ((rc = run_ln(e, s, tmp, lw.final_layer_norm.w, lw.final_layer_norm.b, last ? out : (hidden_states ? x0 : nullptr), M, kHidden,
-                         last ? nullptr : x0hi, last ? nullptr : x0lo,
-                         last && c.range_dev ? c.range_dev + (size_t)kRangeShards * kFiniteStage : nullptr)))
+        if ((rc = run_gemm_split_ln(e, c, s, a, lw.s2, lw.final_layer_norm, last ? out : (hidden_states ? x0 : nullptr), last ? nullptr : x0hi,
+                                    last ? nullptr : x0lo, last && c.range_dev ? c.range_dev + (size_t)kRangeShards * kFiniteStage : nullptr,
+                                    "feed_forward output + residual (fp32)", l)))
             return rc;
     }
     if (nl == 0 && (rc = run_copy(e, s, out, x0, MH))) return rc;
@@ -1752,6 +1774,32 @@
     return LOCO_OK;
 }
 
+int loco_op_gemm_f16x3_ln(const void* Ahi, const void* Alo, const void* Whi, const void* Wlo, const float* bias, const void* Rhi,
+                          const void* Rlo, float* C, const float* gamma, const float* beta, float eps, float* y, void* yhi, void* ylo,
+                          int32_t M, int32_t K, int32_t* fused, void* stream) {
+    if (!Ahi || !Alo || !Whi || !Wlo || !Rhi || !Rlo || !C || !gamma || !beta || (!y && !yhi) || ((yhi == nullptr) != (ylo == nullptr)))
+        return fail(LOCO_E_INVALID, "loco_op_gemm_f16x3_ln: null argument");
+    if (M <= 0 || K <= 0 || K % 32) return fail(LOCO_E_INVALID, "loco_op_gemm_f16x3_ln: M > 0, K %% 32 == 0");
+    GemmSplitArgs a = split_args(M, kHidden, K, kEpiResidual);
+    a.Ahi = (const _Float16*)Ahi; a.Alo = (const _Float16*)Alo; a.Whi = (const _Float16*)Whi; a.Wlo = (const _Float16*)Wlo;
+    a.bias = bias; a.Rhi = (const _Float16*)Rhi; a.Rlo = (const _Float16*)Rlo; a.ldr = kHidden; a.C = C;
+    a.ln_gamma = gamma; a.ln_beta = beta; a.ln_eps = eps; a.ln_y = y; a.ln_hi = (_Float16*)yhi; a.ln_lo = (_Float16*)ylo;
+    bool f = false;
+    HIP_TRY(launch_gemm_split(a, (hipStream_t)stream, &f));
+    if (!f) HIP_TRY(launch_layernorm(C, gamma, beta, y, M, kHidden, eps, (hipStream_t)stream, yhi, ylo));
+    if (fused) *fused = f ? 1 : 0;
+    return LOCO_OK;
+}
+
+int loco_debug_gemm_tile_form(int32_t M, int32_t N, int32_t K, int32_t epilogue, int32_t with_layernorm, int32_t co_scheduled) {
+    static const float dummy = 0.f;
+    GemmSplitArgs a = split_args(M, N, K, epilogue);
+    a.C = const_cast<float*>(&dummy);
+    a.co_scheduled = co_scheduled != 0;
+    if (with_layernorm) { a.ln_gamma = &dummy; a.ln_beta = &dummy; a.ln_y = const_cast<float*>(&dummy); }
+    return gemm_split_tile_form(a);
+}
+
 size_t loco_gemm_splitk_bytes(void) { return kSplitKBytes; }
 
 void loco_debug_reload_gemm_knobs(void) {
diff --git a/loco-asr_amd/csrc/loco_kernels.h b/loco-asr_amd/csrc/loco_kernels.h
--- a/loco-asr_amd/csrc/loco_kernels.h
+++ b/loco-asr_amd/csrc/loco_kernels.h
@@ -70,6 +70,13 @@
     long sBias2 = 0;
     const float* sin_table = nullptr;
     const int32_t* frames = nullptr;
+    const float* ln_gamma = nullptr;
+    const float* ln_beta = nullptr;
+    float* ln_y = nullptr;
+    _Float16* ln_hi = nullptr;
+    _Float16* ln_lo = nullptr;
+    float* ln_nonfinite = nullptr;
+    float ln_eps = 0.f;
 };
 hipError_t launch_group_major_split(const float* x, void* hi, void* lo, int B, int T, hipStream_t s, float* range_slot = nullptr,
                                     const int32_t* rows_clip = nullptr);
@@ -78,7 +85,8 @@
                                   const _Float16* vhi, const _Float16* vlo, const float* qp, const int32_t* frames,
                                   _Float16* ctx_hi, _Float16* ctx_lo, float* ctx, int B, int T, hipStream_t s,
                                   const _Float16* pe_hi = nullptr, const _Float16* pe_lo = nullptr, float pe_scale = 1.0f);
-hipError_t launch_gemm_split(const GemmSplitArgs& a, hipStream_t s);
+hipError_t launch_gemm_split(const GemmSplitArgs& a, hipStream_t s, bool* ln_fused = nullptr);
+int gemm_split_tile_form(const GemmSplitArgs& a);
 void reload_gemm_knobs();
 void reload_attention_knobs();
 hipError_t launch_split_f16(const float* x, void* hi, void* lo, long n, hipStream_t s, float scale = 1.0f);
@@ -185,6 +193,54 @@
     return r;
 }
 
+__device__ __forceinline__ float ln_wave_sum(float v) {
+#pragma unroll
+    for (int o = 32; o > 0; o >>= 1) v += __shfl_xor(v, o, 64);
+    return v;
+}
+
+template <int NV4, bool SPLIT>
+__device__ __forceinline__ void layernorm_row(const float* __restrict__ x, const float* __restrict__ g, const float* __restrict__ b,
+                                              float* __restrict__ y, _Float16* __restrict__ yhi, _Float16* __restrict__ ylo, long row,
+                                              int lane, float eps, float* __restrict__ nonfinite_slot) {
+    constexpr int D = NV4 * 256;
+    const float4* xr = reinterpret_cast<const float4*>(x + row * D);
+    float4 v[NV4];
+    float s = 0.f;
+#pragma unroll
+    for (int i = 0; i < NV4; ++i) {
+        v[i] = xr[lane + 64 * i];
+        s += (v[i].x + v[i].y) + (v[i].z + v[i].w);
+    }
+    const float mean = ln_wave_sum(s) * (1.0f / D);
+    float q = 0.f;
+#pragma unroll
+    for (int i = 0; i < NV4; ++i) {
+        v[i].x -= mean; v[i].y -= mean; v[i].z -= mean; v[i].w -= mean;
+        q += (v[i].x * v[i].x + v[i].y * v[i].y) + (v[i].z * v[i].z + v[i].w * v[i].w);
+    }
+    const float rstd = 1.0f / sqrtf(ln_wave_sum(q) * (1.0f / D) + eps);
+    if (nonfinite_slot && lane == 0 && !(rstd > 0.f)) atomicMax(reinterpret_cast<unsigned*>(nonfinite_slot) + (blockIdx.x & 7), 0x7f800000u);
+#pragma unroll
+    for (int i = 0; i < NV4; ++i) {
+        const float4 gg = reinterpret_cast<const float4*>(g)[lane + 64 * i];
+        const float4 bb = reinterpret_cast<const float4*>(b)[lane + 64 * i];
+        float o[4];
+        o[0] = v[i].x * rstd * gg.x + bb.x;
+        o[1] = v[i].y * rstd * gg.y + bb.y;
+        o[2] = v[i].z * rstd * gg.z + bb.z;
+        o[3] = v[i].w * rstd * gg.w + bb.w;
+        if (y) reinterpret_cast<float4*>(y + row * D)[lane + 64 * i] = make_float4(o[0], o[1], o[2], o[3]);
+        if (SPLIT) {
+            typedef unsigned u32x2_t __attribute__((ext_vector_type(2)));
+            unsigned h0, l0, h1, l1;
+            split_f16_2pairs(o[0], o[1], o[2], o[3], h0, l0, h1, l1);
+            reinterpret_cast<u32x2_t*>(yhi + row * D)[lane + 64 * i] = u32x2_t{h0, h1};
+            reinterpret_cast<u32x2_t*>(ylo + row * D)[lane + 64 * i] = u32x2_t{l0, l1};
+        }
+    }
+}
+
 hipError_t launch_gemm(const GemmArgs& a, hipStream_t s);
 hipError_t launch_layernorm(const float* x, const float* g, const float* b, float* y, long rows, int dim, float eps,
                             hipStream_t s, void* yhi = nullptr, void* ylo = nullptr, float* nonfinite_slot = nullptr);
diff --git a/loco-asr_amd/csrc/norm_misc.hip b/loco-asr_amd/csrc/norm_misc.hip
--- a/loco-asr_amd/csrc/norm_misc.hip
+++ b/loco-asr_amd/csrc/norm_misc.hip
@@ -1,59 +1,16 @@
 #include "loco_kernels.h"
 
 namespace loco {
-
-__device__ __forceinline__ float wave_sum(float v) {
-#pragma unroll
-    for (int o = 32; o > 0; o >>= 1) v += __shfl_xor(v, o, 64);
-    return v;
-}
-
-typedef _Float16 h4_t __attribute__((ext_vector_type(4)));
 
 template <int NV4, bool SPLIT>
 __global__ __launch_bounds__(256) void layernorm_kernel(const float* __restrict__ x, const float* __restrict__ g,
                                                         const float* __restrict__ b, float* __restrict__ y,
                                                         _Float16* __restrict__ yhi, _Float16* __restrict__ ylo, long rows,
                                                         float eps, float* __restrict__ nonfinite_slot) {
-    constexpr int D = NV4 * 256;
     const int lane = threadIdx.x & 63;
     const long row = (long)blockIdx.x * 4 + (threadIdx.x >> 6);
     if (row >= rows) return;
-    const float4* xr = reinterpret_cast<const float4*>(x + row * D);
-    float4 v[NV4];
-    float s = 0.f;
-#pragma unroll
-    for (int i = 0; i < NV4; ++i) {
-        v[i] = xr[lane + 64 * i];
-        s += (v[i].x + v[i].y) + (v[i].z + v[i].w);
-    }
-    const float mean = wave_sum(s) * (1.0f / D);
-    float q = 0.f;
-#pragma unroll
-    for (int i = 0; i < NV4; ++i) {
-        v[i].x -= mean; v[i].y -= mean; v[i].z -= mean; v[i].w -= mean;
-        q += (v[i].x * v[i].x + v[i].y * v[i].y) + (v[i].z * v[i].z + v[i].w * v[i].w);
-    }
-    const float rstd = 1.0f / sqrtf(wave_sum(q) * (1.0f / D) + eps);
-    if (nonfinite_slot && lane == 0 && !(rstd > 0.f)) atomicMax(reinterpret_cast<unsigned*>(nonfinite_slot) + (blockIdx.x & 7), 0x7f800000u);
-#pragma unroll
-    for (int i = 0; i < NV4; ++i) {
-        const float4 gg = reinterpret_cast<const float4*>(g)[lane + 64 * i];
-        const float4 bb = reinterpret_cast<const float4*>(b)[lane + 64 * i];
-        float o[4];
-        o[0] = v[i].x * rstd * gg.x + bb.x;
-        o[1] = v[i].y * rstd * gg.y + bb.y;
-        o[2] = v[i].z * rstd * gg.z + bb.z;
-        o[3] = v[i].w * rstd * gg.w + bb.w;
-        if (y) reinterpret_cast<float4*>(y + row * D)[lane + 64 * i] = make_float4(o[0], o[1], o[2], o[3]);
-        if (SPLIT) {
-            typedef unsigned u32x2_t __attribute__((ext_vector_type(2)));
-            unsigned h0, l0, h1, l1;
-            split_f16_2pairs(o[0], o[1], o[2], o[3], h0, l0, h1, l1);
-            reinterpret_cast<u32x2_t*>(yhi + row * D)[lane + 64 * i] = u32x2_t{h0, h1};
-            reinterpret_cast<u32x2_t*>(ylo + row * D)[lane + 64 * i] = u32x2_t{l0, l1};
-        }
-    }
+    layernorm_row<NV4, SPLIT>(x, g, b, y, yhi, ylo, row, lane, eps, nonfinite_slot);
 }
 
 hipError_t launch_layernorm(const float* x, const float* g, const float* b, float* y, long rows, int dim, float eps,
```

New measurement: 943,100 frames/s. 3.3% lower.
